# ewrfcas/LeftRefill

Measured on AMD Instinct MI355X. Metric: 512x1024 stitched images/sec @ 50 DDIM steps, cfg=2.5; per-UNet-step ms, higher is better.
Workload: dtype f16; 1 GPU; configs[1]: 1-ref inpainting, 512x1024 canvas (latent 64x128), B=4 per GPU (UNet batch 8 under CFG), 50 DDIM steps, cfg=2.5, eta=1.0, fp16; global_batch=4, per_gpu_batch=4, ddim_steps=50, parallelism=dp1 (sample-sharded, no data-path collective), ranks=1

## Files before the change

### include/leftrefill_hip.h

```cpp
#ifndef LEFTREFILL_HIP_H
#define LEFTREFILL_HIP_H

#include <stdint.h>

#ifdef __cplusplus
extern "C" {
#endif

#define LR_E_ARG (-1)
#define LR_E_ALIGN (-2)
#define LR_E_UNSUPPORTED (-3)

typedef void* lr_stream_t;
typedef uint16_t lr_half;
#define LR_DTYPE_F16 0
#define LR_DTYPE_BF16 1
#define LR_PIPE_DEFAULT 0
#define LR_PIPE_W8_DEEP 4
#define LR_PIPE_HALO 8

int lr_abi_version(void);

int lr_nchw_f32_to_nhwc_f16(const float* x1, int C1, const float* x2, int C2, lr_half* y, int Cpad, int N, int H,
                            int W, lr_stream_t s);
int lr_nhwc_f16_to_nchw(const lr_half* y, int Cstride, int C, void* out_nchw, int out_is_f32, int N, int H, int W,
                        lr_stream_t s);

#define LR_GN_CHUNKS 256
int lr_groupnorm_stats(const lr_half* x1, int C1, const lr_half* x2, int C2, int N, int HW, float* partials,
                       lr_stream_t s);
int lr_groupnorm_apply(const lr_half* x1, int C1, const lr_half* x2, int C2, int N, int HW, const float* partials,
                       const float* gamma, const float* beta, float eps, int silu, lr_half* y, lr_stream_t s);
int lr_groupnorm_finalize(const float* p1, int C1, int R1, const float* p2, int C2, int R2, int N, int HW, float* partials,
                          lr_stream_t s);

int lr_gn_conv_out_f16(const lr_half* x, int B, int H, int W, int C, const float* gpart, int chunks, const float* gamma, const float* beta,
                       float eps, const lr_half* w, int ldw, const float* bias, int Cout, lr_half* y, lr_stream_t s);
int lr_groupnorm_apply_n(const lr_half* x1, int C1, const lr_half* x2, int C2, int N, int HW, const float* partials,
                         int nchunks, const float* gamma, const float* beta, float eps, int silu, lr_half* y, lr_stream_t s);

int lr_layernorm(const lr_half* x, const float* gamma, const float* beta, float eps, lr_half* y, int M, int C,
                 lr_stream_t s);

int lr_timestep_embedding(const int64_t* t, int N, int dim, lr_half* out, lr_stream_t s);
int lr_timestep_embedding_f32(const float* t, int N, int dim, lr_half* out, lr_stream_t s);
int lr_linear_small_m(const lr_half* a, int lda, const lr_half* w, const float* bias, lr_half* out, int ldo, int M,
                      int N, int K, int act_in, int act_out, lr_stream_t s);

typedef struct lr_gemm_args {
  const lr_half* p1; int32_t C1;
  const lr_half* p2; int32_t C2;
  int32_t B, H, W;
  int32_t Hs, Ws;
  int32_t taps, stride, up;
  int32_t asym;
  const lr_half* wt; int32_t N;
  const float* bias;
  const lr_half* rowvec; int32_t ld_rowvec;
  const lr_half* resid; int32_t ld_resid;
  lr_half* out; int32_t ld_out;
  int32_t geglu;
  int32_t tile_n;
  int32_t tile_m;
  int32_t splits;
  float* workspace; int64_t workspace_bytes;
  const float* ln_stats; int32_t ln_parts; float ln_eps;
  const float* ln_colsum;
  float* stats_out;
  float* gn_stats_out;
  int32_t dtype;
  int32_t pipe;
  float* gn_group_out; int32_t gn_hw;
  int32_t wt_bstride, bias_bstride;
  int32_t wt_pm;
  const lr_half* skip1; const lr_half* skip2; int32_t Cs1, Cs2;
  int32_t splitk_mode;
} lr_gemm_args;
int lr_gemm_gn_group_chunks(const lr_gemm_args* args);
int lr_gemm_gn_rows(const lr_gemm_args* args);
int lr_gemm_plan(const lr_gemm_args* args, int32_t* plan);
int lr_gemm_stats_parts(const lr_gemm_args* args);
int64_t lr_gemm_workspace_bytes(const lr_gemm_args* args);
int lr_gemm_conv_f16(const lr_gemm_args* args, lr_stream_t s);
int lr_gemm_splitk_timeouts(void);

int lr_attention_f16(const lr_half* q, int ldq, const lr_half* k, int ldk, const lr_half* v, int ldv, lr_half* o,
                     int ldo, int B, int heads, int Nq, int Nkv, float scale, lr_stream_t s);

int lr_attention_causal_f16(const lr_half* q, int ldq, const lr_half* k, int ldk, const lr_half* v, int ldv, lr_half* o,
                            int ldo, int B, int heads, int N, float scale, lr_stream_t s);
int lr_attention_vt_f16(const lr_half* q, int ldq, const lr_half* k, int ldk, const lr_half* vt, int ld_vt, lr_half* o,
                        int ldo, int B, int heads, int Nq, int Nkv, float scale, lr_stream_t s);
int lr_transpose_v_f16(const lr_half* v, int ldv, lr_half* vt, int ld_vt, int B, int heads, int Nkv, lr_stream_t s);

typedef struct lr_xattn_args {
  const lr_half* x; lr_half* out;
  const lr_half* wq; const float* bq;
  const lr_half* k; int32_t ldk;
  const lr_half* vt;
  const lr_half* wo; const float* bo;
  float* stats_out;
  int32_t M, HW, C, heads, Lc;
  float ln_eps, scale;
  const lr_half* pre_a; const lr_half* pre_w; const float* pre_b;
} lr_xattn_args;
int lr_xattn_block_f16(const lr_xattn_args* args, lr_stream_t s);
int lr_xattn_pack_vt_f16(const lr_half* v, int ldv, lr_half* vt, int B, int heads, int Lc, lr_stream_t s);

typedef struct lr_stin_args {
  const lr_half* x; const lr_half* wp; const float* bp; const lr_half* wqkv; const float* bqkv;
  lr_half* x1; lr_half* qkv;
  int32_t M, C, NQ, ld_qkv;
  float ln_eps;
  const float* gn_part; const float* gn_gamma; const float* gn_beta;
  int32_t gn_chunks, gn_hw;
  float gn_eps;
} lr_stin_args;
int lr_stin_block_f16(const lr_stin_args* args, lr_stream_t s);

typedef struct lr_rowlin_args {
  const lr_half* x; const lr_half* w; const float* bias; lr_half* out;
  int32_t M, C, N, ld_out, geglu;
  float ln_eps;
  int32_t ln;
  const float* gn_part; const float* gn_gamma; const float* gn_beta;
  int32_t gn_chunks, gn_hw;
  float gn_eps;
} lr_rowlin_args;
int lr_rowlin_f16(const lr_rowlin_args* args, lr_stream_t s);

typedef struct lr_ffn_args {
  const lr_half* x; lr_half* out;
  const lr_half* w1; const float* b1;
  const lr_half* w2; const float* b2;
  float* stats_out;
  int32_t M, C, H;
  float ln_eps;
  const lr_half* post_w; const float* post_b; const lr_half* post_resid; float* gn_stats_out;
  float* gn_group_out; int32_t gn_hw;
} lr_ffn_args;
int lr_ffn_block_f16(const lr_ffn_args* args, lr_stream_t s);

int lr_softmax_rows_f16(const lr_half* s, lr_half* p, int M, int N, float scale, lr_stream_t st);

int lr_mv_gather(const lr_half* x, lr_half* seq, int b, int v, int s, int C, lr_stream_t st);
typedef struct lr_row_copy_job {
  const void* src; int64_t src_pitch, src_off;
  void* dst; int64_t dst_pitch, dst_off;
  int32_t row_bytes, n_rows;
  const int32_t* src_idx; const int32_t* dst_idx;
} lr_row_copy_job;
int lr_row_copy(const lr_row_copy_job* jobs, int n_jobs, lr_stream_t s);
int lr_mv_scatter(const lr_half* seq, lr_half* x, int b, int v, int s, int C, lr_stream_t st);

int lr_ddim_cfg_step(const float* x, const void* eps, int eps_is_f32, const float* noise, float* x_prev,
                     float* pred_x0, int64_t numel, float cfg_scale, float a_t, float a_prev, float sigma_t,
                     float sqrt_one_minus_at, lr_stream_t s);

int lr_plms_cfg_step(const float* x, const void* eps, int eps_is_f32, const float* const* hist, int n_hist, const float* weights,
                     float divisor, float* e_out, float* x_prev, float* pred_x0, int64_t numel, float cfg_scale, float a_t,
                     float a_prev, float sqrt_one_minus_at, lr_stream_t s);

int lr_dpmpp_cfg_step(const float* x, const void* eps, int eps_is_f32, const float* x0_prev, float* x0_out, float* x_next,
                      int64_t numel, float cfg_scale, float sigma_s, float alpha_s, float ratio, float c, float c_half,
                      float inv_r0, lr_stream_t s);

int lr_ddim_inv_cfg_step(const float* x, const void* eps, int eps_is_f32, float* x_next, int64_t numel, float cfg_scale,
                         float c1, float c2, lr_stream_t s);

int lr_ddim_cfg3_step(const float* x, const void* eps, int eps_is_f32, const float* noise, float* x_prev, float* pred_x0,
                      int64_t numel, float cfg_scale, float cond_weight, float one_minus_cond_weight, float a_t, float a_prev,
                      float sigma_t, float sqrt_one_minus_at, lr_stream_t s);

#define LR_Q_SAMPLE_MAX_B 32
int lr_ddim_q_sample(const float* x0, const float* noise, float* out, int B, int64_t per_sample, const float* sa,
                     const float* s1ma, lr_stream_t s);


int lr_layernorm_bwd(const lr_half* x, const lr_half* dy, const float* gamma, float eps, lr_half* dx, int M, int C,
                     lr_stream_t s);
int lr_groupnorm_bwd(const lr_half* x1, int C1, const lr_half* x2, int C2, const lr_half* dy, int N, int HW,
                     const float* fwd_partials, const float* gamma, const float* beta, float eps, int silu,
                     float* bwd_partials, lr_half* dx1, lr_half* dx2, lr_stream_t s);
int lr_layernorm_bwd_res(const lr_half* x, const lr_half* dy, const lr_half* dres, const float* gamma, float eps, lr_half* dx,
                         int M, int C, lr_stream_t s);
int lr_groupnorm_bwd_res(const lr_half* x1, int C1, const lr_half* x2, int C2, const lr_half* dy, const lr_half* dres1,
                         const lr_half* dres2, int N, int HW, const float* fwd_partials, int fwd_chunks, const float* gamma,
                         const float* beta, float eps, int silu, float* bwd_partials, lr_half* dx1, lr_half* dx2, lr_stream_t s);
int lr_geglu_bwd(const lr_half* pre, const lr_half* dy, lr_half* dpre, int M, int H, lr_stream_t s);
int lr_geglu_fwd(const lr_half* pre, lr_half* out, int M, int H, lr_stream_t s);
int lr_attention_lse_f16(const lr_half* q, int ldq, const lr_half* k, int ldk, const lr_half* v, int ldv, lr_half* o,
                         int ldo, float* lse, int B, int heads, int Nq, int Nkv, float scale, lr_stream_t s);
typedef struct lr_attn_bwd_args {
  const lr_half* q; const lr_half* k; const lr_half* v; const lr_half* o; const lr_half* dout;
  const lr_half* qt; const lr_half* kt; const lr_half* dot;
  const float* lse; float* dsum;
  lr_half* dq; lr_half* dk; lr_half* dv;
  int32_t ldq, ldk, ldv, ldo, lddo, ld_qt, ld_kt, lddq, lddk, lddv;
  int32_t B, heads, Nq, Nkv;
  float scale;
} lr_attn_bwd_args;
int lr_attention_bwd_f16(const lr_attn_bwd_args* args, lr_stream_t s);
int lr_attention_causal_lse_f16(const lr_half* q, int ldq, const lr_half* k, int ldk, const lr_half* v, int ldv, lr_half* o,
                                int ldo, float* lse, int B, int heads, int N, float scale, lr_stream_t s);
int lr_attention_causal_bwd_f16(const lr_attn_bwd_args* args, lr_stream_t s);
int lr_gelu_fwd_f16(const lr_half* pre, lr_half* y, int64_t n, lr_stream_t s);
int lr_gelu_bwd_f16(const lr_half* pre, const lr_half* dy, lr_half* dpre, int64_t n, lr_stream_t s);

int lr_mv_gather_bwd(const lr_half* dseq, lr_half* dx, int b, int v, int s, int C, lr_stream_t st);
int lr_mv_scatter_bwd(const lr_half* dx, lr_half* dseq, int b, int v, int s, int C, lr_stream_t st);
int lr_sumpool2x2(const lr_half* x, lr_half* y, int N, int H, int W, int C, lr_stream_t s);

int lr_groupnorm_stats_bf16(const lr_half* x1, int C1, const lr_half* x2, int C2, int N, int HW, float* partials,
    lr_stream_t s);
int lr_groupnorm_apply_bf16(const lr_half* x1, int C1, const lr_half* x2, int C2, int N, int HW, const float*
    partials, const float* gamma, const float* beta, float eps, int silu, lr_half* y, lr_stream_t s);
int lr_groupnorm_apply_n_bf16(const lr_half* x1, int C1, const lr_half* x2, int C2, int N, int HW, const float*
    partials, int nchunks, const float* gamma, const float* beta, float eps, int silu, lr_half* y, lr_stream_t s);
int lr_layernorm_bf16(const lr_half* x, const float* gamma, const float* beta, float eps, lr_half* y, int M, int C,
    lr_stream_t s);
int lr_layernorm_bwd_bf16(const lr_half* x, const lr_half* dy, const float* gamma, float eps, lr_half* dx, int M, int
    C, lr_stream_t s);
int lr_groupnorm_bwd_bf16(const lr_half* x1, int C1, const lr_half* x2, int C2, const lr_half* dy, int N, int HW,
    const float* fwd_partials, const float* gamma, const float* beta, float eps, int silu, float* bwd_partials,
    lr_half* dx1, lr_half* dx2, lr_stream_t s);
int lr_layernorm_bwd_res_bf16(const lr_half* x, const lr_half* dy, const lr_half* dres, const float* gamma, float eps, lr_half*
    dx, int M, int C, lr_stream_t s);
int lr_groupnorm_bwd_res_bf16(const lr_half* x1, int C1, const lr_half* x2, int C2, const lr_half* dy, const lr_half* dres1,
    const lr_half* dres2, int N, int HW, const float* fwd_partials, int fwd_chunks, const float* gamma, const float* beta,
// ... 66 lines not shown
```

### leftrefill_amd/_lib.py

```python
import ctypes
import os

HERE = os.path.dirname(os.path.abspath(__file__))
LIB_PATH = os.environ.get("LEFTREFILL_LIB_PATH") or os.path.join(HERE, "lib", "libleftrefill_hip.so")
ABI_VERSION = 29

c_void_p, c_int, c_float, c_int64 = ctypes.c_void_p, ctypes.c_int, ctypes.c_float, ctypes.c_int64


class GemmArgs(ctypes.Structure):
    _fields_ = [
        ("p1", c_void_p), ("C1", ctypes.c_int32),
        ("p2", c_void_p), ("C2", ctypes.c_int32),
        ("B", ctypes.c_int32), ("H", ctypes.c_int32), ("W", ctypes.c_int32),
        ("Hs", ctypes.c_int32), ("Ws", ctypes.c_int32),
        ("taps", ctypes.c_int32), ("stride", ctypes.c_int32), ("up", ctypes.c_int32),
        ("asym", ctypes.c_int32),
        ("wt", c_void_p), ("N", ctypes.c_int32),
        ("bias", c_void_p),
        ("rowvec", c_void_p), ("ld_rowvec", ctypes.c_int32),
        ("resid", c_void_p), ("ld_resid", ctypes.c_int32),
        ("out", c_void_p), ("ld_out", ctypes.c_int32),
        ("geglu", ctypes.c_int32),
        ("tile_n", ctypes.c_int32),
        ("tile_m", ctypes.c_int32),
        ("splits", ctypes.c_int32),
        ("workspace", c_void_p), ("workspace_bytes", ctypes.c_int64),
        ("ln_stats", c_void_p), ("ln_parts", ctypes.c_int32), ("ln_eps", ctypes.c_float),
        ("ln_colsum", c_void_p),
        ("stats_out", c_void_p),
        ("gn_stats_out", c_void_p),
        ("dtype", ctypes.c_int32),
        ("pipe", ctypes.c_int32),
        ("gn_group_out", c_void_p), ("gn_hw", ctypes.c_int32),
        ("wt_bstride", ctypes.c_int32), ("bias_bstride", ctypes.c_int32),
        ("wt_pm", ctypes.c_int32),
        ("skip1", c_void_p), ("skip2", c_void_p), ("Cs1", ctypes.c_int32), ("Cs2", ctypes.c_int32),
        ("splitk_mode", ctypes.c_int32),
    ]


class AttnBwdArgs(ctypes.Structure):
    _fields_ = ([(n, c_void_p) for n in ("q", "k", "v", "o", "dout", "qt", "kt", "dot", "lse", "dsum", "dq", "dk", "dv")] +
                [(n, ctypes.c_int32) for n in ("ldq", "ldk", "ldv", "ldo", "lddo", "ld_qt", "ld_kt", "lddq", "lddk", "lddv",
                                               "B", "heads", "Nq", "Nkv")] + [("scale", ctypes.c_float)])


class XattnArgs(ctypes.Structure):
    _fields_ = [("x", c_void_p), ("out", c_void_p), ("wq", c_void_p), ("bq", c_void_p), ("k", c_void_p), ("ldk", ctypes.c_int32),
                ("vt", c_void_p), ("wo", c_void_p), ("bo", c_void_p), ("stats_out", c_void_p),
                ("M", ctypes.c_int32), ("HW", ctypes.c_int32), ("C", ctypes.c_int32), ("heads", ctypes.c_int32),
                ("Lc", ctypes.c_int32), ("ln_eps", ctypes.c_float), ("scale", ctypes.c_float),
                ("pre_a", c_void_p), ("pre_w", c_void_p), ("pre_b", c_void_p)]


class RowCopyJob(ctypes.Structure):
    _fields_ = [("src", c_void_p), ("src_pitch", ctypes.c_int64), ("src_off", ctypes.c_int64),
                ("dst", c_void_p), ("dst_pitch", ctypes.c_int64), ("dst_off", ctypes.c_int64),
                ("row_bytes", ctypes.c_int32), ("n_rows", ctypes.c_int32), ("src_idx", c_void_p), ("dst_idx", c_void_p)]


class StinArgs(ctypes.Structure):
    _fields_ = [("x", c_void_p), ("wp", c_void_p), ("bp", c_void_p), ("wqkv", c_void_p), ("bqkv", c_void_p), ("x1", c_void_p),
                ("qkv", c_void_p), ("M", ctypes.c_int32), ("C", ctypes.c_int32), ("NQ", ctypes.c_int32), ("ld_qkv", ctypes.c_int32),
                ("ln_eps", ctypes.c_float), ("gn_part", c_void_p), ("gn_gamma", c_void_p), ("gn_beta", c_void_p),
                ("gn_chunks", ctypes.c_int32), ("gn_hw", ctypes.c_int32), ("gn_eps", ctypes.c_float)]


class RowlinArgs(ctypes.Structure):
    _fields_ = [("x", c_void_p), ("w", c_void_p), ("bias", c_void_p), ("out", c_void_p), ("M", ctypes.c_int32), ("C", ctypes.c_int32),
                ("N", ctypes.c_int32), ("ld_out", ctypes.c_int32), ("geglu", ctypes.c_int32), ("ln_eps", ctypes.c_float), ("ln", ctypes.c_int32),
                ("gn_part", c_void_p), ("gn_gamma", c_void_p), ("gn_beta", c_void_p), ("gn_chunks", ctypes.c_int32), ("gn_hw", ctypes.c_int32),
                ("gn_eps", ctypes.c_float)]


class FfnArgs(ctypes.Structure):
    _fields_ = [("x", c_void_p), ("out", c_void_p), ("w1", c_void_p), ("b1", c_void_p), ("w2", c_void_p), ("b2", c_void_p),
                ("stats_out", c_void_p), ("M", ctypes.c_int32), ("C", ctypes.c_int32), ("H", ctypes.c_int32), ("ln_eps", ctypes.c_float),
                ("post_w", c_void_p), ("post_b", c_void_p), ("post_resid", c_void_p), ("gn_stats_out", c_void_p),
                ("gn_group_out", c_void_p), ("gn_hw", ctypes.c_int32)]


SIGNATURES = {
    "lr_abi_version": [],
    "lr_nchw_f32_to_nhwc_f16": [c_void_p, c_int, c_void_p, c_int, c_void_p, c_int, c_int, c_int, c_int, c_void_p],
    "lr_nhwc_f16_to_nchw": [c_void_p, c_int, c_int, c_void_p, c_int, c_int, c_int, c_int, c_void_p],
    "lr_groupnorm_stats": [c_void_p, c_int, c_void_p, c_int, c_int, c_int, c_void_p, c_void_p],
    "lr_groupnorm_apply": [c_void_p, c_int, c_void_p, c_int, c_int, c_int, c_void_p, c_void_p, c_void_p, c_float,
                           c_int, c_void_p, c_void_p],
    "lr_layernorm_bwd": [c_void_p, c_void_p, c_void_p, c_float, c_void_p, c_int, c_int, c_void_p],
    "lr_groupnorm_bwd": [c_void_p, c_int, c_void_p, c_int, c_void_p, c_int, c_int, c_void_p, c_void_p, c_void_p, c_float,
                         c_int, c_void_p, c_void_p, c_void_p, c_void_p],
    "lr_layernorm_bwd_res": [c_void_p, c_void_p, c_void_p, c_void_p, c_float, c_void_p, c_int, c_int, c_void_p],
    "lr_groupnorm_bwd_res": [c_void_p, c_int, c_void_p, c_int, c_void_p, c_void_p, c_void_p, c_int, c_int, c_void_p, c_int, c_void_p,
                             c_void_p, c_float, c_int, c_void_p, c_void_p, c_void_p, c_void_p],
    "lr_mv_gather_bwd": [c_void_p, c_void_p, c_int, c_int, c_int, c_int, c_void_p],
    "lr_mv_scatter_bwd": [c_void_p, c_void_p, c_int, c_int, c_int, c_int, c_void_p],
    "lr_geglu_fwd": [c_void_p, c_void_p, c_int, c_int, c_void_p],
    "lr_geglu_bwd": [c_void_p, c_void_p, c_void_p, c_int, c_int, c_void_p],
    "lr_sumpool2x2": [c_void_p, c_void_p, c_int, c_int, c_int, c_int, c_void_p],
    "lr_softmax_rows_f16": [c_void_p, c_void_p, c_int, c_int, c_float, c_void_p],
    "lr_layernorm": [c_void_p, c_void_p, c_void_p, c_float, c_void_p, c_int, c_int, c_void_p],
    "lr_timestep_embedding": [c_void_p, c_int, c_int, c_void_p, c_void_p],
    "lr_linear_small_m": [c_void_p, c_int, c_void_p, c_void_p, c_void_p, c_int, c_int, c_int, c_int, c_int, c_int,
                          c_void_p],
    "lr_gemm_workspace_bytes": [ctypes.POINTER(GemmArgs)],
    "lr_gemm_stats_parts": [ctypes.POINTER(GemmArgs)],
    "lr_gemm_gn_rows": [ctypes.POINTER(GemmArgs)],
    "lr_gemm_gn_group_chunks": [ctypes.POINTER(GemmArgs)],
    "lr_gn_conv_out_f16": [c_void_p, c_int, c_int, c_int, c_int, c_void_p, c_int, c_void_p, c_void_p, c_float, c_void_p, c_int, c_void_p,
                           c_int, c_void_p, c_void_p],
    "lr_groupnorm_finalize": [c_void_p, c_int, c_int, c_void_p, c_int, c_int, c_int, c_int, c_void_p, c_void_p],
    "lr_groupnorm_apply_n": [c_void_p, c_int, c_void_p, c_int, c_int, c_int, c_void_p, c_int, c_void_p, c_void_p, c_float,
                             c_int, c_void_p, c_void_p],
    "lr_gemm_plan": [ctypes.POINTER(GemmArgs), ctypes.POINTER(ctypes.c_int32)],
    "lr_gemm_conv_f16": [ctypes.POINTER(GemmArgs), c_void_p],
    "lr_attention_f16": [c_void_p, c_int, c_void_p, c_int, c_void_p, c_int, c_void_p, c_int, c_int, c_int, c_int,
                         c_int, c_float, c_void_p],
    "lr_attention_vt_f16": [c_void_p, c_int, c_void_p, c_int, c_void_p, c_int, c_void_p, c_int, c_int, c_int, c_int,
                         c_int, c_float, c_void_p],
    "lr_attention_causal_f16": [c_void_p, c_int, c_void_p, c_int, c_void_p, c_int, c_void_p, c_int, c_int, c_int, c_int, c_float,
                                c_void_p],
    "lr_attention_lse_f16": [c_void_p, c_int, c_void_p, c_int, c_void_p, c_int, c_void_p, c_int, c_void_p, c_int, c_int, c_int,
                             c_int, c_float, c_void_p],
    "lr_attention_bwd_f16": [ctypes.POINTER(AttnBwdArgs), c_void_p],
    "lr_attention_causal_lse_f16": [c_void_p, c_int, c_void_p, c_int, c_void_p, c_int, c_void_p, c_int, c_void_p, c_int, c_int, c_int,
                                    c_float, c_void_p],
    "lr_attention_causal_bwd_f16": [ctypes.POINTER(AttnBwdArgs), c_void_p],
    "lr_gelu_fwd_f16": [c_void_p, c_void_p, c_int64, c_void_p],
    "lr_gelu_bwd_f16": [c_void_p, c_void_p, c_void_p, c_int64, c_void_p],
    "lr_transpose_v_f16": [c_void_p, c_int, c_void_p, c_int, c_int, c_int, c_int, c_void_p],
    "lr_xattn_block_f16": [ctypes.POINTER(XattnArgs), c_void_p],
    "lr_xattn_pack_vt_f16": [c_void_p, c_int, c_void_p, c_int, c_int, c_int, c_void_p],
    "lr_ffn_block_f16": [ctypes.POINTER(FfnArgs), c_void_p],
    "lr_stin_block_f16": [ctypes.POINTER(StinArgs), c_void_p],
    "lr_rowlin_f16": [ctypes.POINTER(RowlinArgs), c_void_p],
    "lr_mv_gather": [c_void_p, c_void_p, c_int, c_int, c_int, c_int, c_void_p],
    "lr_row_copy": [c_void_p, c_int, c_void_p],
    "lr_gemm_splitk_timeouts": [],
    "lr_mv_scatter": [c_void_p, c_void_p, c_int, c_int, c_int, c_int, c_void_p],
    "lr_ddim_cfg_step": [c_void_p, c_void_p, c_int, c_void_p, c_void_p, c_void_p, c_int64, c_float, c_float, c_float,
                         c_float, c_float, c_void_p],
    "lr_timestep_embedding_f32": [c_void_p, c_int, c_int, c_void_p, c_void_p],
    "lr_plms_cfg_step": [c_void_p, c_void_p, c_int, c_void_p, c_int, c_void_p, c_float, c_void_p, c_void_p, c_void_p, c_int64,
                         c_float, c_float, c_float, c_float, c_void_p],
    "lr_dpmpp_cfg_step": [c_void_p, c_void_p, c_int, c_void_p, c_void_p, c_void_p, c_int64, c_float, c_float, c_float, c_float,
                          c_float, c_float, c_float, c_void_p],
    "lr_ddim_inv_cfg_step": [c_void_p, c_void_p, c_int, c_void_p, c_int64, c_float, c_float, c_float, c_void_p],
    "lr_ddim_cfg3_step": [c_void_p, c_void_p, c_int, c_void_p, c_void_p, c_void_p, c_int64, c_float, c_float, c_float, c_float,
                          c_float, c_float, c_float, c_void_p],
    "lr_ddim_q_sample": [c_void_p, c_void_p, c_void_p, c_int, c_int64, c_void_p, c_void_p, c_void_p],
}

BF16_TWINS = ["lr_groupnorm_stats", "lr_groupnorm_apply", "lr_groupnorm_apply_n", "lr_layernorm", "lr_layernorm_bwd",
              "lr_groupnorm_bwd", "lr_layernorm_bwd_res", "lr_groupnorm_bwd_res", "lr_nchw_f32_to_nhwc_f16", "lr_nhwc_f16_to_nchw", "lr_timestep_embedding", "lr_linear_small_m",
              "lr_mv_gather", "lr_mv_scatter", "lr_ddim_cfg_step", "lr_timestep_embedding_f32", "lr_plms_cfg_step",
              "lr_dpmpp_cfg_step", "lr_ddim_inv_cfg_step", "lr_ddim_cfg3_step", "lr_geglu_fwd", "lr_geglu_bwd", "lr_sumpool2x2",
              "lr_mv_gather_bwd", "lr_mv_scatter_bwd", "lr_attention_f16", "lr_attention_causal_f16", "lr_attention_lse_f16",
              "lr_attention_vt_f16", "lr_transpose_v_f16", "lr_attention_bwd_f16", "lr_xattn_block_f16",
              "lr_xattn_pack_vt_f16", "lr_ffn_block_f16", "lr_stin_block_f16", "lr_rowlin_f16", "lr_gn_conv_out_f16",
              "lr_attention_causal_lse_f16", "lr_attention_causal_bwd_f16", "lr_gelu_fwd_f16", "lr_gelu_bwd_f16"]


def twin(name):
    return (name[:-4] if name.endswith("_f16") else name) + "_bf16"


for _n in BF16_TWINS:
    SIGNATURES[twin(_n)] = SIGNATURES[_n]

_FOLD_SIG = [c_void_p, c_int, c_int, c_int, c_int, c_void_p, c_void_p, c_float, c_void_p, c_void_p, c_int, c_void_p, c_void_p, c_void_p]
DEV_SIGNATURES = {"lr_dev_set": [ctypes.c_char_p, c_int], "lr_dev_unset": [ctypes.c_char_p],
                  "lr_gn_fold_weights_f16": _FOLD_SIG, "lr_gn_fold_weights_bf16": _FOLD_SIG}

_lib = None


def fn(lib, name, dtype):
    import torch
    if dtype == torch.bfloat16:
        return getattr(lib, twin(name))
    assert dtype == torch.float16, dtype
    return getattr(lib, name)


def load():
    global _lib
    if _lib is not None:
        return _lib
    import torch
    if not os.path.exists(LIB_PATH):
# ... 42 lines not shown
```

### leftrefill_amd/build.py

```python
import os
import shutil
import subprocess
import sys
from concurrent.futures import ThreadPoolExecutor

HERE = os.path.dirname(os.path.abspath(__file__))
CSRC = os.path.join(HERE, "csrc")
LIBDIR = os.path.join(HERE, "lib")
LIB = os.path.join(LIBDIR, "libleftrefill_hip.so")
SOURCES = ["norm.hip", "elementwise.hip", "gemm_conv.hip", "conv_halo.hip", "attention.hip", "attention_bwd.hip", "xattn_block.hip", "xattn_block640.hip", "stin_block.hip", "rowlin.hip", "ffn_block.hip", "conv_out.hip"]
FLAGS = ["--offload-arch=gfx950", "-O3", "-std=c++17", "-fPIC", "-Wno-unused-value"]
EXTRA = {"attention.hip": ["-mllvm", "-amdgpu-mfma-vgpr-form"], "xattn_block.hip": ["-mllvm", "-amdgpu-mfma-vgpr-form"], "ffn_block.hip": ["-mllvm", "-amdgpu-mfma-vgpr-form"], "stin_block.hip": ["-mllvm", "-amdgpu-mfma-vgpr-form"], "rowlin.hip": ["-mllvm", "-amdgpu-mfma-vgpr-form"], "attention_bwd.hip": ["-mllvm", "-amdgpu-mfma-vgpr-form"]}


def hipcc():
    for c in (os.environ.get("HIPCC"), shutil.which("hipcc"), "/opt/rocm/bin/hipcc"):
        if c and os.path.exists(c):
            return c
    raise RuntimeError("hipcc not found")


def _stale(out, deps):
    if not os.path.exists(out):
        return True
    t = os.path.getmtime(out)
    return any(os.path.getmtime(d) > t for d in deps)


def build(force=False, verbose=True):
    os.makedirs(LIBDIR, exist_ok=True)
    objdir = os.path.join(HERE, "build")
    os.makedirs(objdir, exist_ok=True)
    cc = hipcc()
    headers = [os.path.join(CSRC, "common.h"), os.path.join(CSRC, "chain_common.h"), os.path.join(CSRC, "gemm_common.h"), os.path.join(HERE, "..", "include", "leftrefill_hip.h")]
    jobs = []
    for s in SOURCES:
        src = os.path.join(CSRC, s)
        obj = os.path.join(objdir, s.replace(".hip", ".o"))
        if force or _stale(obj, [src] + headers):
            jobs.append([cc] + FLAGS + EXTRA.get(s, []) + ["-c", src, "-o", obj])
    if jobs:
        def run(cmd):
            if verbose:
                print(" ".join(cmd), flush=True)
            subprocess.run(cmd, check=True)
        with ThreadPoolExecutor(max_workers=4) as ex:
            list(ex.map(run, jobs))
    objs = [os.path.join(objdir, s.replace(".hip", ".o")) for s in SOURCES]
    if force or jobs or _stale(LIB, objs):
        cmd = [cc, "--offload-arch=gfx950", "-shared", "-fPIC", "-o", LIB] + objs
        if verbose:
            print(" ".join(cmd), flush=True)
        subprocess.run(cmd, check=True)
    return LIB


if __name__ == "__main__":
    print(build(force="--force" in sys.argv))
```

### leftrefill_amd/csrc/chain_common.h

```cpp
#pragma once
#include "common.h"

typedef __attribute__((address_space(3))) void* lptr_t;

template <int N> __device__ __forceinline__ void xa_wait_vmcnt() { asm volatile("s_waitcnt vmcnt(%0)" ::"n"(N) : "memory"); }

__device__ __forceinline__ float xa_row4_sum(float v) {
#if defined(__HIP_DEVICE_COMPILE__)
  const unsigned u = __builtin_bit_cast(unsigned, v);
  const auto a = __builtin_amdgcn_permlane16_swap(u, u, false, false);
  v = __builtin_bit_cast(float, (unsigned)a[0]) + __builtin_bit_cast(float, (unsigned)a[1]);
  const unsigned u2 = __builtin_bit_cast(unsigned, v);
  const auto b = __builtin_amdgcn_permlane32_swap(u2, u2, false, false);
  v = __builtin_bit_cast(float, (unsigned)b[0]) + __builtin_bit_cast(float, (unsigned)b[1]);
#endif
  return v;
}
__device__ __forceinline__ float xa_row4_max(float v) {
#if defined(__HIP_DEVICE_COMPILE__)
  const unsigned u = __builtin_bit_cast(unsigned, v);
  const auto a = __builtin_amdgcn_permlane16_swap(u, u, false, false);
  v = fmaxf(__builtin_bit_cast(float, (unsigned)a[0]), __builtin_bit_cast(float, (unsigned)a[1]));
  const unsigned u2 = __builtin_bit_cast(unsigned, v);
  const auto b = __builtin_amdgcn_permlane32_swap(u2, u2, false, false);
  v = fmaxf(__builtin_bit_cast(float, (unsigned)b[0]), __builtin_bit_cast(float, (unsigned)b[1]));
#endif
  return v;
}

template <typename T>
__device__ __forceinline__ vec8<T> xa_pack(const f32x4& a, const f32x4& b) {
  vec8<T> r;
#pragma unroll
  for (int i = 0; i < 4; ++i) { r[i] = (T)a[i]; r[4 + i] = (T)b[i]; }
  return r;
}
int lr_xattn640_launch(const lr_xattn_args* a, int bf16_, lr_stream_t s);

__device__ __forceinline__ void xa_swap_rows16(f32x4& a, f32x4& b) {
#if defined(__HIP_DEVICE_COMPILE__)
#pragma unroll
  for (int r = 0; r < 4; ++r) {
    const float ar = a[r], br = b[r];
    const auto s = __builtin_amdgcn_permlane16_swap(__builtin_bit_cast(unsigned, ar), __builtin_bit_cast(unsigned, br), false, false);
    a[r] = __builtin_bit_cast(float, (unsigned)s[0]);
    b[r] = __builtin_bit_cast(float, (unsigned)s[1]);
  }
#endif
}

__device__ __forceinline__ void xa_gn_tables(const float* gp, int nchunks, int n, int HW, int C, const float* gamma, const float* beta,
                                             float eps, float* tabA, float* tabB, float* s_mr , int t, int nthreads) {
#if defined(__HIP_DEVICE_COMPILE__)
  const int Cg = C / 32;
  if (t < 128) {
    const int g = t >> 2, sub = t & 3;
    double s = 0.0, q = 0.0;
    const float* ps = gp + ((size_t)n * nchunks * 32 + g) * 2;
#pragma unroll 4
    for (int c = sub; c < nchunks; c += 4) { s += (double)ps[c * 64]; q += (double)ps[c * 64 + 1]; }
#pragma unroll
    for (int sh = 2; sh > 0; sh >>= 1) { s += __shfl_xor(s, sh, 64); q += __shfl_xor(q, sh, 64); }
    if (sub == 0) {
      const double cnt = (double)HW * (double)Cg;
      const double mean = s / cnt;
      double var = q / cnt - mean * mean;
      if (var < 0.0) var = 0.0;
      s_mr[g] = (float)mean;
      s_mr[32 + g] = (float)(1.0 / sqrt(var + (double)eps));
    }
  }
  __syncthreads();
  for (int c = t; c < C; c += nthreads) {
    const int g = c / Cg;
    const float a = s_mr[32 + g] * gamma[c];
    tabA[c] = a;
    tabB[c] = beta[c] - s_mr[g] * a;
  }
  __syncthreads();
#endif
}
```

### leftrefill_amd/csrc/conv_halo.hip

```cpp
#include "gemm_common.h"

#ifndef HALO_EXP
#define HALO_EXP 0
#endif
#define HALO_PW 18
#define HALO_NQ 45

template <int BN, int WMW, int NSTAGE, typename T>
__global__ __launch_bounds__(512) void conv_halo_kernel(const GemmParams P) {
#if defined(__HIP_DEVICE_COMPILE__)
  constexpr int NW = 8, WNW = NW / WMW, TM = 16 / WMW, TN = BN / WNW / 16;
  constexpr int PATCH_BYTES = HALO_NQ * 1024;
  constexpr int B_BYTES = BN * 128;
  constexpr int NB_FULL = BN / (NW * 8);
  constexpr bool B_TAIL = (BN % (NW * 8)) != 0;
  constexpr int TAIL_WAVES = (BN % (NW * 8)) / 8;
  constexpr int PAR_LD = ((BN + 63) / 64) * 64;
  static_assert(NSTAGE == 2 || NSTAGE == 3, "weight ring depth");
  extern __shared__ __attribute__((aligned(16))) char smem[];
  char* const patch = smem;
  char* const wring = smem + PATCH_BYTES;
  float* const par = reinterpret_cast<float*>(wring + NSTAGE * B_BYTES);

  const int t = threadIdx.x;
  const int lane = t & 63;
  const int w = __builtin_amdgcn_readfirstlane(t >> 6);
  const int wm = w / WNW, wn = w % WNW;
  const int fr = lane & 15, fq = lane >> 4;
  const unsigned OOB = 0x80000000u;

  const int xcd = blockIdx.x & 7;
  const int q8 = P.nblocks >> 3, r8 = P.nblocks & 7;
  const int bid = (xcd < r8 ? xcd * (q8 + 1) : r8 * (q8 + 1) + (xcd - r8) * q8) + (blockIdx.x >> 3);
  [[maybe_unused]] const int lr_trace_tile = bid;
  int tile_n, tile;
  tile_order(P, bid, tile, tile_n);
  const bool seg = P.H == 8;
  const int Hv = seg ? 16 : P.H;
  const int npx = seg ? 2 * 10 * HALO_PW : HALO_PW * HALO_PW, nq = (npx + 7) >> 3;
  const int tiles_x = P.W >> 4, tps = (Hv >> 4) * tiles_x;
  const int smp = tile / tps, trem = tile - smp * tps;
  const int tyi = trem / tiles_x, txi = trem - tyi * tiles_x;
  const int y0 = tyi * 16, x0 = txi * 16;
  const int n0 = tile_n * BN;
  const int m_org = (smp * Hv + y0) * P.W + x0;

  int pix[6];
#pragma unroll
  for (int k = 0; k < 6; ++k) {
    const int px = (w + 8 * k) * 8 + (lane >> 3);
    const int pl = (px * 3641) >> 16, pc = px - pl * HALO_PW;
    const int sg = seg ? (pl * 26) >> 8 : 0;
    const int y = (seg ? pl - 10 * sg : y0 + pl) - 1, x = x0 - 1 + pc;
    const bool ok = px < npx && (unsigned)y < (unsigned)P.H && (unsigned)x < (unsigned)P.W;
    const int c = (lane & 7) ^ (pc & 6);
    pix[k] = ok ? (((((seg ? 2 * smp + sg : smp) * P.H + y) * P.W + x)) | (c << 28)) : -1;
  }
  const int Ctot = P.C1 + P.C2;
  const int cpt1 = P.C1 >> 6, ncm = Ctot >> 6, cpt3 = P.C3 >> 6;
  const int nch_all = ncm + ((P.C3 + P.C4) >> 6);
  const int c_per = (nch_all + P.splits - 1) / P.splits;
  const int c_begin = min((int)blockIdx.y * c_per, nch_all);
  const int nch = min(nch_all, c_begin + c_per);
  const int nsteps = (min(nch, ncm) - min(c_begin, ncm)) * 9 + (max(nch, ncm) - max(c_begin, ncm));
  auto issue_patch = [&](const int ci) __attribute__((always_inline)) {
    const f16* src; int cs, ch;
    if (ci < cpt1) { src = P.p1; cs = P.C1; ch = ci; }
    else if (ci < ncm) { src = P.p2; cs = P.C2; ch = ci - cpt1; }
    else if (ci < ncm + cpt3) { src = P.p3; cs = P.C3; ch = ci - ncm; }
    else { src = P.p4; cs = P.C4; ch = ci - ncm - cpt3; }
    const __amdgpu_buffer_rsrc_t rsA = uniform_rsrc((const void*)src, (size_t)P.M * cs * 2);
    const unsigned coff = (unsigned)ch * 128u;
#pragma unroll
    for (int k = 0; k < 6; ++k) {
      const int q = w + 8 * k;
      if (q < nq) {
        const unsigned vo = pix[k] >= 0 ? (unsigned)((pix[k] & 0x0FFFFFFF) * cs + (pix[k] >> 28) * 8) * 2u : OOB;
        __builtin_amdgcn_raw_ptr_buffer_load_lds(rsA, (lptr_t)(patch + q * 1024), 16, vo, coff, 0, 0);
      }
    }
  };

  const __amdgpu_buffer_rsrc_t rsB = uniform_rsrc((const void*)P.wt, (size_t)P.N * P.K * 2);
  const __amdgpu_buffer_rsrc_t rsZ = uniform_rsrc((const void*)P.wt, 0);
  __amdgpu_buffer_rsrc_t rsW = rsB;
  unsigned wvo[NB_FULL + 1];
#pragma unroll
  for (int i = 0; i < NB_FULL + 1; ++i) {
    const int row = (i * NW + w) * 8 + (lane >> 3);
    const int n = n0 + row;
    const int chunk = (lane & 7) ^ ((row >> 1) & 7);
    wvo[i] = (row < BN && n < P.N) ? (unsigned)(((size_t)n * (P.wt_pm ? 64 : P.K) + chunk * 8) * 2) : OOB;
  }
  auto wkoff = [&](const int ci, const int tap) -> unsigned {
    if (P.wt_pm) return (unsigned)(ci < ncm ? tap * ncm + ci : 9 * ncm + (ci - ncm)) * (unsigned)P.N * 128u;
    return (unsigned)((ci < ncm ? tap * Ctot + ci * 64 : 9 * Ctot + (ci - ncm) * 64) * 2);
  };
  auto issue_weights = [&](const int slot, const unsigned koff) __attribute__((always_inline)) {
    char* Bs = wring + slot * B_BYTES;
    if (B_TAIL && w < TAIL_WAVES)
      __builtin_amdgcn_raw_ptr_buffer_load_lds(rsW, (lptr_t)(Bs + ((NB_FULL * NW + w) * 8) * 128), 16, wvo[NB_FULL], koff, 0, 0);
#pragma unroll
    for (int i = 0; i < NB_FULL; ++i)
      __builtin_amdgcn_raw_ptr_buffer_load_lds(rsW, (lptr_t)(Bs + ((i * NW + w) * 8) * 128), 16, wvo[i], koff, 0, 0);
  };
  auto advance = [&](int& ci, int& tap) __attribute__((always_inline)) {
    const int nt = ci < ncm ? 9 : 1;
    if (++tap == nt) { tap = 0; ++ci; }
  };

  const int pb0 = (wm * TM + (seg ? 2 * ((wm * TM) >> 3) : 0)) * HALO_PW + fr;
  auto read_frags = [&](vec8<T> (&xf)[TM], vec8<T> (&wf)[TN], const int slot, const int ks, const int ky, const int kx) {
    const char* Bs = wring + slot * B_BYTES;
    const int kc = ks * 4 + fq;
    const int col = fr + kx;
    const char* xs = patch + (pb0 + kx) * 128 + ((kc ^ (col & 6)) << 4) + ky * (HALO_PW * 128);
#pragma unroll
    for (int i = 0; i < TM; ++i) xf[i] = *reinterpret_cast<const vec8<T>*>(xs + i * (HALO_PW * 128));
#pragma unroll
    for (int j = 0; j < TN; ++j) {
      const int row = weight_tile<TN, WNW, false>(wn, j) * 16 + fr;
      wf[j] = *reinterpret_cast<const vec8<T>*>(Bs + row * 128 + ((kc ^ ((row >> 1) & 7)) << 4));
    }
  };
  f32x4 acc[TN][TM];
  auto mma = [&](const vec8<T> (&xf)[TM], const vec8<T> (&wf)[TN]) {
#pragma unroll
    for (int j = 0; j < TN; ++j)
#pragma unroll
      for (int i = 0; i < TM; ++i)
        acc[j][i] = lr_mfma16(wf[j], xf[i], acc[j][i]);
  };
  auto spread = [&](auto ndma) __attribute__((always_inline)) {
    constexpr int ND = decltype(ndma)::value;
    constexpr int PER = (TM * TN) / ND > 0 ? (TM * TN) / ND : 1;
#pragma unroll
    for (int g = 0; g < ND; ++g) {
      __builtin_amdgcn_sched_group_barrier(0x8, PER, 0);
      __builtin_amdgcn_sched_group_barrier(0x10, 1, 0);
    }
  };
  using std::integral_constant;

  LR_STAMP(0);
  stage_params<BN, PAR_LD>(P, par, n0, w, lane, 0);
  if (nsteps > 0) issue_patch(c_begin);
  int wci = c_begin, wtap = 0;
#pragma unroll
  for (int sidx = 0; sidx < NSTAGE - 1; ++sidx) {
    if (sidx < nsteps) { issue_weights(sidx, wkoff(wci, wtap)); advance(wci, wtap); }
  }
  LR_STAMP(1);
#pragma unroll
  for (int j = 0; j < TN; ++j)
#pragma unroll
    for (int i = 0; i < TM; ++i) acc[j][i] = (f32x4){0.f, 0.f, 0.f, 0.f};
  if (NSTAGE == 3 && nsteps > 1) {
    if (B_TAIL && w < TAIL_WAVES) wait_vmcnt<NB_FULL + 1>(); else wait_vmcnt<NB_FULL>();
  } else {
    wait_vmcnt<0>();
  }
  __builtin_amdgcn_s_barrier();
  LR_STAMP(2);

  int ci = c_begin, tap = 0, cur = 0;
  vec8<T> xa[TM], wa[TN];
  for (int s = 0; s < nsteps; ++s) {
    const bool main_part = ci < ncm;
    const int ky = main_part ? (tap * 11) >> 5 : 1, kx = main_part ? tap - 3 * ky : 1;
    const bool last_tap = !main_part || tap == 8;
    const bool pf_w = s + NSTAGE - 1 < nsteps;
    const bool pf_p = last_tap && ci + 1 < nch;
    int wslot = cur + NSTAGE - 1; if (wslot >= NSTAGE) wslot -= NSTAGE;
    read_frags(xa, wa, cur, 0, ky, kx);
    __builtin_amdgcn_sched_barrier(0);
    rsW = (pf_w && HALO_EXP != 3) ? rsB : rsZ;
    issue_weights(wslot, wkoff(wci, wtap));
    advance(wci, wtap);
    mma(xa, wa);
    spread(integral_constant<int, NB_FULL>{});
    __builtin_amdgcn_sched_barrier(0);
    read_frags(xa, wa, cur, 1, ky, kx);
    if (pf_p && HALO_EXP != 1) {
      asm volatile("s_waitcnt lgkmcnt(0)" ::: "memory");
      __builtin_amdgcn_s_barrier();
      issue_patch(ci + 1);
    }
    mma(xa, wa);
    if (NSTAGE == 3 && !pf_p) {
      if (B_TAIL && w < TAIL_WAVES) wait_vmcnt<NB_FULL + 1>(); else wait_vmcnt<NB_FULL>();
    } else {
      wait_vmcnt<0>();
    }
    __builtin_amdgcn_s_barrier();
    cur = cur + 1 == NSTAGE ? 0 : cur + 1;
    advance(ci, tap);
  }
  LR_STAMP(3);
  LR_STAMP(4);

  float* gsl = reinterpret_cast<float*>(smem);
  const bool gp = P.gp_out != nullptr && P.splits == 1;
  epilogue_units<TM, TN, 0, PAR_LD, WNW, T, true>(P, acc, m_org + wm * TM * P.W, n0, wn, lane, par, par, tile_n * WNW + wn,
                                                  gsl + wm * (BN * 2), tile * WMW + wm);
  if (gp) {
    asm volatile("s_waitcnt lgkmcnt(0)" ::: "memory");
    __builtin_amdgcn_s_barrier();
    gn_group_reduce<BN, WMW, 256>(P, gsl, tile * 256, n0, t);
  }
#ifdef LR_DEV_VARIANTS
  if (P.sk_cnt != nullptr && P.splits > 1)
    sk_fused_tail<T, BN>(P, tile * P.ntiles_n + tile_n, 8,
                         [&](const int j, const int r) { return m_org + (2 * j + (r >> 4)) * P.W + (r & 15); },
                         [&](const int j) { return tile * 8 + j; }, [&](const int j) { return tile * 256 + 32 * j; }, n0,
                         reinterpret_cast<float*>(smem), t);
#endif
  LR_STAMP(5);
#ifdef LR_GEMM_TRACE
  asm volatile("s_waitcnt vmcnt(0)" ::: "memory");
  LR_STAMP(6);
#endif
#endif
}

template <int BN, int WMW, int NSTAGE, typename T>
static int launch_halo_t(const GemmParams& P0, hipStream_t st) {
  GemmParams P = P0;
  P.ntiles_n = (P.N + BN - 1) / BN;
  P.ntiles_m = P.M / 256;
  P.m_fastest = 0;
  if (LR_DEV("LR_HALO_MFASTEST", 0) && P.splits > 1) P.m_fastest = 1;
  P.nblocks = P.ntiles_n * P.ntiles_m;
  const size_t smem = (size_t)HALO_NQ * 1024 + NSTAGE * (size_t)BN * 128 + 2 * (((BN + 63) / 64) * 64) * sizeof(float);
  static unsigned long long attr_done = 0;
  if (lr_attr_needed(&attr_done)) {
    hipFuncSetAttribute(reinterpret_cast<const void*>(conv_halo_kernel<BN, WMW, NSTAGE, T>), hipFuncAttributeMaxDynamicSharedMemorySize,
                        (int)smem);
  }
  hipLaunchKernelGGL((conv_halo_kernel<BN, WMW, NSTAGE, T>), dim3(P.nblocks, P.splits), dim3(512), smem, st, P);
  return lr_launch_status();
}

int lr_launch_conv_halo(const GemmParams& P, int tile_n, hipStream_t st) {
  if (P.taps != 9 || P.stride != 1 || P.up || P.zins || P.pad != 1 || P.c16 || P.splits < 1 || P.geglu || P.gelu || P.ln_part ||
      P.wt_bstride || P.st_out || ((P.H & 15) && !(P.H == 8 && P.M % 256 == 0)) || (P.W & 15) || P.Hs != P.H || P.Ws != P.W)
    return LR_E_UNSUPPORTED;
  if ((long long)P.M >= (1ll << 28)) return LR_E_UNSUPPORTED;
  if (tile_n == 320) return P.bf16 ? launch_halo_t<320, 2, 2, bf16>(P, st) : launch_halo_t<320, 2, 2, f16>(P, st);
  if (tile_n == 160) return P.bf16 ? launch_halo_t<160, 4, 3, bf16>(P, st) : launch_halo_t<160, 4, 3, f16>(P, st);
  return LR_E_UNSUPPORTED;
}

unsigned lr_halo_sk_timeouts() {
  unsigned v = 0;
  if (hipMemcpyFromSymbol(&v, HIP_SYMBOL(lr_sk_error), sizeof(v)) != hipSuccess) return 0xFFFFFFFFu;
  return v;
}
```

### leftrefill_amd/csrc/elementwise.hip

```cpp
#include "common.h"

template <typename T>
__global__ void nchw_to_nhwc_kernel(const float* __restrict__ x1, int C1, const float* __restrict__ x2, int C2,
                                    T* __restrict__ y, int Cpad, int HW, long long total) {
  const int nOct = Cpad >> 3;
  for (long long idx = blockIdx.x * (long long)blockDim.x + threadIdx.x; idx < total;
       idx += (long long)gridDim.x * blockDim.x) {
    const int p = (int)(idx % HW);
    const long long q = idx / HW;
    const int o = (int)(q % nOct);
    const long long n = q / nOct;
    float f[8];
#pragma unroll
    for (int i = 0; i < 8; ++i) {
      const int c = o * 8 + i;
      float v = 0.f;
      if (c < C1) v = x1[((size_t)n * C1 + c) * HW + p];
      else if (c < C1 + C2) v = x2[((size_t)n * C2 + (c - C1)) * HW + p];
      f[i] = v;
    }
    *reinterpret_cast<uint4*>(y + ((size_t)n * HW + p) * Cpad + o * 8) = lr_pack8<T>(f);
  }
}

// ... 228 lines not shown
    ld_eps<V, EpsT>(eps, i, eu);
    ld_eps<V, EpsT>(eps, numel + i, ec);
    ld_f32<V>(x, i, xv);
    if (n_hist > 0) ld_f32<V>(h1, i, a);
    if (n_hist > 1) ld_f32<V>(h2, i, b);
    if (n_hist > 2) ld_f32<V>(h3, i, c);
#pragma unroll
    for (int k = 0; k < V; ++k) {
      e[k] = cfg_combine<EpsT, T>(eu[k], ec[k], scale);
      float acc = w0 * e[k];
      if (n_hist > 0) acc = acc + w1 * a[k];
      if (n_hist > 1) acc = acc + w2 * b[k];
      if (n_hist > 2) acc = acc + w3 * c[k];
      const float ep = acc / div;
      p0[k] = (xv[k] - sqrt_1m_at * ep) / sqrt_at;
      xp[k] = sqrt_aprev * p0[k] + dir_coef * ep;
    }
    if (e_out) st_f32<V>(e_out, i, e);
    st_f32<V>(pred_x0, i, p0);
    st_f32<V>(x_prev, i, xp);
  }
}

template <int V, typename EpsT, typename T>
__global__ void dpmpp_cfg_step_kernel(const float* __restrict__ x, const EpsT* __restrict__ eps, const float* __restrict__ x0_prev,
                                      float* __restrict__ x0_out, float* __restrict__ x_next, long long numel, float scale,
                                      float sigma_s, float alpha_s, float ratio, float c, float c_half, float inv_r0) {
#pragma clang fp contract(off)
  const long long groups = numel / V;
  for (long long g = blockIdx.x * (long long)blockDim.x + threadIdx.x; g < groups; g += (long long)gridDim.x * blockDim.x) {
    const long long i = g * V;
    float eu[V], ec[V], xv[V], m1[V], m0[V], xt[V];
    ld_eps<V, EpsT>(eps, i, eu);
    ld_eps<V, EpsT>(eps, numel + i, ec);
    ld_f32<V>(x, i, xv);
    if (x0_prev) ld_f32<V>(x0_prev, i, m1);
#pragma unroll
    for (int k = 0; k < V; ++k) {
      const float e = cfg_combine<EpsT, T>(eu[k], ec[k], scale);
      m0[k] = (xv[k] - sigma_s * e) / alpha_s;
      float v = ratio * xv[k] - c * m0[k];
      if (x0_prev) {
        const float D = inv_r0 * (m0[k] - m1[k]);
        v = v - c_half * D;
      }
      xt[k] = v;
    }
    st_f32<V>(x0_out, i, m0);
    st_f32<V>(x_next, i, xt);
  }
}

template <int V, typename EpsT, typename T>
__global__ void ddim_inv_cfg_step_kernel(const float* __restrict__ x, const EpsT* __restrict__ eps, float* __restrict__ x_next,
                                         long long numel, float scale, float c1, float c2) {
#pragma clang fp contract(off)
  const long long groups = numel / V;
  for (long long g = blockIdx.x * (long long)blockDim.x + threadIdx.x; g < groups; g += (long long)gridDim.x * blockDim.x) {
    const long long i = g * V;
    float eu[V], ec[V], xv[V], xn[V];
    ld_eps<V, EpsT>(eps, i, eu);
    ld_eps<V, EpsT>(eps, numel + i, ec);
    ld_f32<V>(x, i, xv);
#pragma unroll
    for (int k = 0; k < V; ++k) {
      const float e = cfg_combine<EpsT, T>(eu[k], ec[k], scale);
      const float a = c1 * xv[k];
      float b;
      if constexpr (sizeof(EpsT) == 2) b = (float)(T)((float)(T)c2 * e);
      else b = c2 * e;
      xn[k] = a + b;
    }
    st_f32<V>(x_next, i, xn);
  }
}

__device__ __forceinline__ float f32_rounded(float v) {
  asm volatile("" : "+v"(v));
  return v;
}

template <typename EpsT, typename T>
__device__ __forceinline__ float cfg3_combine(float eu, float ec, float es, float scale, float w, float w1m) {
#pragma clang fp contract(off)
  if constexpr (sizeof(EpsT) == 2) {
    const T a = (T)f32_rounded(w * ec);
    const T b = (T)f32_rounded(w1m * es);
    const T m = (T)((float)a + (float)b);
    const T d = (T)((float)m - eu);
    const T sd = (T)f32_rounded(scale * (float)d);
    return (float)(T)(eu + (float)sd);
  } else {
    return eu + scale * ((w * ec + w1m * es) - eu);
  }
}

template <int V, typename EpsT, typename T>
__global__ void ddim_cfg3_step_kernel(const float* __restrict__ x, const EpsT* __restrict__ eps, const float* __restrict__ noise,
                                      float* __restrict__ x_prev, float* __restrict__ pred_x0, long long numel, float scale,
                                      float w, float w1m, float sqrt_at, float sqrt_1m_at, float sqrt_aprev, float dir_coef,
                                      float sigma) {
#pragma clang fp contract(off)
  const long long groups = numel / V;
  for (long long g = blockIdx.x * (long long)blockDim.x + threadIdx.x; g < groups; g += (long long)gridDim.x * blockDim.x) {
    const long long i = g * V;
    float eu[V], ec[V], es[V], xv[V], nz[V], p0[V], xp[V];
    ld_eps<V, EpsT>(eps, i, eu);
    ld_eps<V, EpsT>(eps, numel + i, ec);
    ld_eps<V, EpsT>(eps, 2 * numel + i, es);
    ld_f32<V>(x, i, xv);
    if (noise) ld_f32<V>(noise, i, nz);
#pragma unroll
    for (int k = 0; k < V; ++k) {
      const float e = cfg3_combine<EpsT, T>(eu[k], ec[k], es[k], scale, w, w1m);
      p0[k] = (xv[k] - sqrt_1m_at * e) / sqrt_at;
      float v = sqrt_aprev * p0[k] + dir_coef * e;
      if (noise) v = v + sigma * nz[k];
      xp[k] = v;
    }
    st_f32<V>(pred_x0, i, p0);
    st_f32<V>(x_prev, i, xp);
  }
}

struct QSampleCoefs { float sa[LR_Q_SAMPLE_MAX_B]; float s1ma[LR_Q_SAMPLE_MAX_B]; };

template <int V>
__global__ void ddim_q_sample_kernel(const float* __restrict__ x0, const float* __restrict__ noise, float* __restrict__ out,
                                     long long per_sample, const QSampleCoefs C) {
#pragma clang fp contract(off)
  const long long base = (long long)blockIdx.y * per_sample;
  const float sa = C.sa[blockIdx.y], s1ma = C.s1ma[blockIdx.y];
  const long long groups = per_sample / V;
  for (long long g = blockIdx.x * (long long)blockDim.x + threadIdx.x; g < groups; g += (long long)gridDim.x * blockDim.x) {
    const long long i = base + g * V;
    float xv[V], nv[V], o[V];
    ld_f32<V>(x0, i, xv);
    ld_f32<V>(noise, i, nv);
#pragma unroll
    for (int k = 0; k < V; ++k) o[k] = sa * xv[k] + s1ma * nv[k];
    st_f32<V>(out, i, o);
  }
}

static inline bool aligned16(const void* p) { return p == nullptr || ((uintptr_t)p & 15) == 0; }

static inline int grid_for(long long total, int block, int cap = 4096) {
  long long g = (total + block - 1) / block;
  if (g > cap) g = cap;
  if (g < 1) g = 1;
  return (int)g;
}

extern "C" int lr_abi_version(void) { return 29; }

#ifdef LR_DEV_VARIANTS
#include <map>
#include <mutex>
#include <string>
static std::map<std::string, int>& lr_dev_table() { static std::map<std::string, int> t; return t; }
static std::mutex lr_dev_mutex;
extern "C" int lr_dev_set(const char* name, int value) {
  if (!name) return LR_E_ARG;
  std::lock_guard<std::mutex> g(lr_dev_mutex);
  lr_dev_table()[name] = value;
  return 0;
}
extern "C" int lr_dev_unset(const char* name) {
  if (!name) return LR_E_ARG;
  std::lock_guard<std::mutex> g(lr_dev_mutex);
  lr_dev_table().erase(name);
  return 0;
}
int lr_dev_get(const char* name, int dflt) {
  std::lock_guard<std::mutex> g(lr_dev_mutex);
  const auto it = lr_dev_table().find(name);
  return it == lr_dev_table().end() ? dflt : it->second;
}
#endif

template <typename T>
static int lr_nchw_f32_to_nhwc_t(const float* x1, int C1, const float* x2, int C2, lr_half* y, int Cpad, int N,
                                       int H, int W, lr_stream_t s) {
  if (!x1 || !y || N <= 0 || H <= 0 || W <= 0 || C1 <= 0) return LR_E_ARG;
  if (!x2) C2 = 0;
  if (Cpad % 8 || Cpad < C1 + C2) return LR_E_ALIGN;
  const long long total = (long long)N * (Cpad / 8) * H * W;
  hipLaunchKernelGGL(nchw_to_nhwc_kernel<T>, dim3(grid_for(total, 256)), dim3(256), 0, (hipStream_t)s, x1, C1, x2, C2,
                     (T*)y, Cpad, H * W, total);
  return lr_launch_status();
}

template <typename T>
static int lr_nhwc_f16_to_nchw_t(const lr_half* y, int Cstride, int C, void* out, int out_is_f32, int N, int H, int W,
                                   lr_stream_t s) {
  if (!y || !out || N <= 0 || C <= 0 || C > Cstride) return LR_E_ARG;
  const long long total = (long long)N * C * H * W;
  if (out_is_f32)
    hipLaunchKernelGGL((nhwc_to_nchw_kernel<float, T>), dim3(grid_for(total, 256)), dim3(256), 0, (hipStream_t)s,
                       (const T*)y, Cstride, C, (float*)out, H * W, total);
  else
    hipLaunchKernelGGL((nhwc_to_nchw_kernel<T, T>), dim3(grid_for(total, 256)), dim3(256), 0, (hipStream_t)s,
                       (const T*)y, Cstride, C, (T*)out, H * W, total);
  return lr_launch_status();
}

template <typename TT, typename T>
static int lr_timestep_embedding_t(const TT* t, int N, int dim, lr_half* out, lr_stream_t s) {
  if (!t || !out || N <= 0 || dim < 2) return LR_E_ARG;
  const int total = N * (dim / 2);
  hipLaunchKernelGGL((timestep_embedding_kernel<TT, T>), dim3((total + 255) / 256), dim3(256), 0, (hipStream_t)s, t, N, dim,
                     (T*)out);
  return lr_launch_status();
}

template <typename T>
static int lr_linear_small_m_t(const lr_half* a, int lda, const lr_half* w, const float* bias, lr_half* out, int ldo,
                                 int M, int N, int K, int act_in, int act_out, lr_stream_t s) {
  if (!a || !w || !out || M <= 0 || N <= 0 || K <= 0) return LR_E_ARG;
  if (M > 16) return LR_E_UNSUPPORTED;
  if (K % 8) return LR_E_ALIGN;
  const int waves = 4;
  int cpw = (N + waves * 512 - 1) / (waves * 512);
  if (cpw < 4) cpw = 4;
  if (cpw > 32) cpw = 32;
  dim3 grid((N + cpw * waves - 1) / (cpw * waves)), block(64 * waves);
  hipStream_t st = (hipStream_t)s;
  if (M <= 4)
    hipLaunchKernelGGL((linear_small_m_kernel<4, T>), grid, block, 4 * K * sizeof(T), st, (const T*)a, lda,
                       (const T*)w, bias, (T*)out, ldo, M, N, K, act_in, act_out, cpw);
  else if (M <= 8)
    hipLaunchKernelGGL((linear_small_m_kernel<8, T>), grid, block, 8 * K * sizeof(T), st, (const T*)a, lda,
                       (const T*)w, bias, (T*)out, ldo, M, N, K, act_in, act_out, cpw);
  else
    hipLaunchKernelGGL((linear_small_m_kernel<16, T>), grid, block, 16 * K * sizeof(T), st, (const T*)a, lda,
                       (const T*)w, bias, (T*)out, ldo, M, N, K, act_in, act_out, cpw);
  return lr_launch_status();
}

template <typename T>
static int lr_mv_gather_t(const lr_half* x, lr_half* seq, int b, int v, int s, int C, lr_stream_t st) {
  if (!x || !seq || b <= 0 || v <= 0 || s <= 0) return LR_E_ARG;
  if (C % 8) return LR_E_ALIGN;
  const long long total = (long long)b * (v + 1) * s * s * (C / 8);
  hipLaunchKernelGGL((mv_gather_kernel<false, T>), dim3(grid_for(total, 256)), dim3(256), 0, (hipStream_t)st, (const uint4*)x,
                     (uint4*)seq, b, v, s, C / 8, total);
  return lr_launch_status();
}

template <typename T>
static int lr_mv_scatter_t(const lr_half* seq, lr_half* x, int b, int v, int s, int C, lr_stream_t st) {
  if (!x || !seq || b <= 0 || v <= 0 || s <= 0) return LR_E_ARG;
  if (C % 8) return LR_E_ALIGN;
  const long long total = (long long)b * v * s * 2 * s * (C / 8);
  hipLaunchKernelGGL(mv_scatter_kernel<false>, dim3(grid_for(total, 256)), dim3(256), 0, (hipStream_t)st, (const uint4*)seq,
                     (uint4*)x, b, v, s, C / 8, total);
  return lr_launch_status();
}

template <typename T>
static int lr_ddim_cfg_step_t(const float* x, const void* eps, int eps_is_f32, const float* noise, float* x_prev,
                                float* pred_x0, int64_t numel, float cfg_scale, float a_t, float a_prev, float sigma_t,
                                float sqrt_one_minus_at, lr_stream_t s) {
  if (!x || !eps || !x_prev || !pred_x0 || numel <= 0) return LR_E_ARG;
  const float sqrt_at = sqrtf(a_t);
  const float sqrt_aprev = sqrtf(a_prev);
  const float dir_coef = sqrtf(1.0f - a_prev - sigma_t * sigma_t);
  dim3 grid(grid_for(numel, 256)), block(256);
  if (eps_is_f32)
    hipLaunchKernelGGL((ddim_cfg_step_kernel<float, T>), grid, block, 0, (hipStream_t)s, x, (const float*)eps, noise, x_prev,
                       pred_x0, (long long)numel, cfg_scale, sqrt_at, sqrt_one_minus_at, sqrt_aprev, dir_coef,
                       sigma_t);
  else
    hipLaunchKernelGGL((ddim_cfg_step_kernel<T, T>), grid, block, 0, (hipStream_t)s, x, (const T*)eps, noise, x_prev,
                       pred_x0, (long long)numel, cfg_scale, sqrt_at, sqrt_one_minus_at, sqrt_aprev, dir_coef,
                       sigma_t);
  return lr_launch_status();
}

template <int V, typename EpsT, typename T>
static void launch_plms(const float* x, const void* eps, const float* h1, const float* h2, const float* h3, float* e_out,
                        float* x_prev, float* pred_x0, long long numel, int n_hist, float scale, const float* w, float div,
                        float sqrt_at, float sqrt_1m_at, float sqrt_aprev, float dir_coef, hipStream_t s) {
  hipLaunchKernelGGL((plms_cfg_step_kernel<V, EpsT, T>), dim3(grid_for(numel / V, 256)), dim3(256), 0, s, x, (const EpsT*)eps,
                     h1, h2, h3, e_out, x_prev, pred_x0, numel, n_hist, scale, w[0], w[1], w[2], w[3], div, sqrt_at, sqrt_1m_at,
                     sqrt_aprev, dir_coef);
}

template <typename T>
static int lr_plms_cfg_step_t(const float* x, const void* eps, int eps_is_f32, const float* const* hist, int n_hist,
                              const float* weights, float divisor, float* e_out, float* x_prev, float* pred_x0, int64_t numel,
                              float cfg_scale, float a_t, float a_prev, float sqrt_one_minus_at, lr_stream_t s) {
  if (!x || !eps || !x_prev || !pred_x0 || !weights || numel <= 0 || n_hist < 0 || n_hist > 3 || divisor == 0.f) return LR_E_ARG;
  if (n_hist > 0 && !hist) return LR_E_ARG;
  const float* h[3] = {nullptr, nullptr, nullptr};
  for (int k = 0; k < n_hist; ++k) {
    if (!hist[k]) return LR_E_ARG;
    h[k] = hist[k];
  }
  float w[4] = {weights[0], 0.f, 0.f, 0.f};
  for (int k = 0; k < n_hist; ++k) w[k + 1] = weights[k + 1];
  const float sqrt_at = sqrtf(a_t);
  const float sqrt_aprev = sqrtf(a_prev);
  const float dir_coef = sqrtf(1.0f - a_prev - 0.0f);
  const bool vec = numel % 4 == 0 && aligned16(x) && aligned16(h[0]) && aligned16(h[1]) && aligned16(h[2]) && aligned16(e_out) &&
                   aligned16(x_prev) && aligned16(pred_x0) && ((uintptr_t)eps & (eps_is_f32 ? 15 : 7)) == 0;
  hipStream_t st = (hipStream_t)s;
// ... 326 lines not shown
```

### leftrefill_amd/csrc/gemm_common.h

```cpp
#pragma once
#include "common.h"
#include <type_traits>

#define BK 64
#define GEMM_THREADS 256
#define BM 128

struct GemmParams {
  const f16* p1; const f16* p2; const f16* wt; const float* bias; const f16* rowvec; const f16* resid; f16* out;
  int C1, C2, H, W, Hs, Ws, taps, stride, up, pad, zins, N, M, K, ld_rowvec, ld_resid, ld_out, geglu, gelu, rows_per_batch;
  int ntiles_n, nblocks;
  int splits; float* ws;
  int ntiles_m, m_fastest;
  unsigned hw_mul, hw_sh, w_mul, w_sh;
  const float* ln_part; const float* ln_cs; int ln_parts; float ln_eps, ln_invc;
  float* st_out; int st_parts;
  float* gs_out;
  float* gp_out; int gp_cg, gp_chunks, gp_hw;
  int gs_store;
  int wt_bstride, bias_bstride;
  int wt_pm;
  int c16;
  const f16* p3; const f16* p4; int C3, C4;
  int bf16;
  unsigned* sk_cnt;
#ifdef LR_GEMM_STAGGER
  int stagger;
#endif
#ifdef LR_GEMM_TRACE
  unsigned long long* trace;
#endif
};

#ifdef LR_GEMM_TRACE
#define LR_STAMP(k) do { if (P.trace && threadIdx.x == 0) P.trace[(size_t)(blockIdx.y * P.nblocks + lr_trace_tile) * 8 + (k)] = __builtin_readcyclecounter(); } while (0)
#else
#define LR_STAMP(k) do { } while (0)
#endif

__device__ __forceinline__ void tile_order(const GemmParams& P, int bid, int& tile_m, int& tile_n) {
  if (P.m_fastest > 1) {
    const int G = P.m_fastest, per = G * P.ntiles_n;
    const int grp = bid / per, first = grp * G;
    const int gsz = min(G, P.ntiles_m - first), r = bid - grp * per;
    tile_m = first + r % gsz; tile_n = r / gsz;
  } else if (P.m_fastest) { tile_m = bid % P.ntiles_m; tile_n = bid / P.ntiles_m; }
  else { tile_n = bid % P.ntiles_n; tile_m = bid / P.ntiles_n; }
}

typedef __attribute__((address_space(3))) void* lptr_t;


__device__ __forceinline__ void swap_rows16(f32x4& a, f32x4& b) {
#if defined(__HIP_DEVICE_COMPILE__)
#pragma unroll
  for (int r = 0; r < 4; ++r) {
    const float ar = a[r], br = b[r];
    const auto s = __builtin_amdgcn_permlane16_swap(__builtin_bit_cast(unsigned, ar), __builtin_bit_cast(unsigned, br),
                                                    false, false);
    a[r] = __builtin_bit_cast(float, (unsigned)s[0]);
    b[r] = __builtin_bit_cast(float, (unsigned)s[1]);
  }
#endif
}

typedef unsigned u32x4 __attribute__((ext_vector_type(4)));
#ifndef LR_OUT_AUX
#define LR_OUT_AUX 16
#endif

template <int TE, int WNW>
__device__ __forceinline__ constexpr int emit_tile(const int wn, const int je) {
  return TE == 5 ? (je < 4 ? 4 * wn + je : 4 * WNW + wn) : wn * TE + je;
}
template <int TN, int WNW, bool GEGLU>
__device__ __forceinline__ constexpr int weight_tile(const int wn, const int j) {
  return GEGLU ? 2 * emit_tile<TN / 2, WNW>(wn, j >> 1) + (j & 1) : emit_tile<TN, WNW>(wn, j);
}

template <int TM, int TN, int MODE, int PAR_LD, int WNW, typename T, bool HALO = false>
__device__ __forceinline__ void epilogue_units(const GemmParams& P, f32x4 (&acc)[TN][TM], const int m_w0, const int n0,
                                               const int wn, const int lane, const float* rs, const float* par,
                                               const int part, float* gsl = nullptr, const int rb_halo = 0) {
#if defined(__HIP_DEVICE_COMPILE__)
  constexpr bool GEGLU = MODE == 1;
  constexpr int TE = GEGLU ? TN / 2 : TN;
  constexpr int NPJ = TE / 2;
  constexpr int NUJ = TM * NPJ;
  constexpr int NU = NUJ + (TE & 1) * (TM / 2);
  constexpr int G = TM * TN >= 40 ? 8 : (NU < 16 ? NU : 16);
  const int fr = lane & 15, fq = lane >> 4;
  const int odd = fq & 1, ch8 = (fq >> 1) * 8;
  const int N_out = GEGLU ? P.N >> 1 : P.N;
  const int no0 = GEGLU ? n0 >> 1 : n0;
  const bool ln = P.ln_part != nullptr;
  const bool fin = P.splits == 1;
  const unsigned OOB = 0x80000000u;
  const int mstep = HALO ? P.W : 16;
  const __amdgpu_buffer_rsrc_t rsR = uniform_rsrc(P.resid ? (const void*)P.resid : (const void*)P.out,
                                                  (P.resid && fin) ? ((size_t)(P.M - 1) * P.ld_resid + N_out) * 2 : 0);
  const __amdgpu_buffer_rsrc_t rsV = uniform_rsrc(P.rowvec ? (const void*)P.rowvec : (const void*)P.out,
                                                  (P.rowvec && fin) ? ((size_t)((P.M - 1) / P.rows_per_batch) * P.ld_rowvec + N_out) * 2 : 0);
  const __amdgpu_buffer_rsrc_t rsO = uniform_rsrc(P.out, fin ? ((size_t)(P.M - 1) * P.ld_out + N_out) * 2 : 0);
  const __amdgpu_buffer_rsrc_t rsWS = uniform_rsrc(P.sk_cnt ? (const void*)P.ws : (const void*)P.out,
                                                   P.sk_cnt ? (size_t)P.splits * P.M * P.N * 4 : 0);
  constexpr int SGH = TM > 8 ? TM : 8;
  float sg[2 * SGH];
#pragma unroll
  for (int i = 0; i < 2 * SGH; ++i) sg[i] = 0.f;
#define s1(i) sg[(i)]
#define s2(i) sg[SGH + (i)]
#define g1(q) sg[(q)]
#define g2(q) sg[SGH + (q)]
  const bool gstat = !GEGLU && fin && (P.gs_out != nullptr || P.gp_out != nullptr) && P.st_out == nullptr;
  auto row16_sum = [&](float v) -> float {
    v += __builtin_bit_cast(float, __builtin_amdgcn_mov_dpp(__builtin_bit_cast(int, v), 0xB1, 0xF, 0xF, true));
    v += __builtin_bit_cast(float, __builtin_amdgcn_mov_dpp(__builtin_bit_cast(int, v), 0x4E, 0xF, 0xF, true));
    v += __builtin_bit_cast(float, __builtin_amdgcn_mov_dpp(__builtin_bit_cast(int, v), 0x141, 0xF, 0xF, true));
    v += __builtin_bit_cast(float, __builtin_amdgcn_mov_dpp(__builtin_bit_cast(int, v), 0x140, 0xF, 0xF, true));
    return v;
  };
  auto flush_group = [&](const int n_lane, const bool pair_fq) {
    const int rb = HALO ? rb_halo : m_w0 / (TM * 16);
#pragma unroll
    for (int q = 0; q < 8; ++q) {
      float a = row16_sum(g1(q)), b = row16_sum(g2(q));
      if (pair_fq) {
        const auto sa = __builtin_amdgcn_permlane16_swap(__builtin_bit_cast(unsigned, a), __builtin_bit_cast(unsigned, a), false, false);
        a = __builtin_bit_cast(float, (unsigned)sa[0]) + __builtin_bit_cast(float, (unsigned)sa[1]);
        const auto sb = __builtin_amdgcn_permlane16_swap(__builtin_bit_cast(unsigned, b), __builtin_bit_cast(unsigned, b), false, false);
        b = __builtin_bit_cast(float, (unsigned)sb[0]) + __builtin_bit_cast(float, (unsigned)sb[1]);
      }
      g1(q) = a; g2(q) = b;
    }
    if (fr == 0 && (!pair_fq || !odd) && n_lane < N_out) {
      if (P.gs_out != nullptr && m_w0 < P.M) {
        float* dst = P.gs_out + ((size_t)rb * N_out + n_lane) * 2;
#pragma unroll
        for (int q = 0; q < 8; q += 2) {
          const f32x4 o = {g1(q), g2(q), g1(q + 1), g2(q + 1)};
          *reinterpret_cast<f32x4*>(dst + 2 * q) = o;
        }
      }
      if (P.gp_out != nullptr) {
        float* dst = gsl + (n_lane - no0) * 2;
#pragma unroll
        for (int q = 0; q < 8; q += 2) {
          const f32x4 o = {g1(q), g2(q), g1(q + 1), g2(q + 1)};
          *reinterpret_cast<f32x4*>(dst + 2 * q) = o;
        }
      }
    }
#pragma unroll
    for (int q = 0; q < 8; ++q) { g1(q) = 0.f; g2(q) = 0.f; }
  };
  auto rowstat = [&](const int i) -> float2 { return *reinterpret_cast<const float2*>(rs + 2 * (i * 16 + fr)); };
  auto par4 = [&](const int which, const int col) -> f32x4 { return *reinterpret_cast<const f32x4*>(par + which * PAR_LD + col); };
  auto tile = [&](const int i, const int je) -> f32x4 {
    if constexpr (!GEGLU) {
      const int c = weight_tile<TN, WNW, false>(wn, je) * 16 + fq * 4;
      f32x4 r = acc[je][i];
      if (ln) { const float2 mr = rowstat(i); r = (r - par4(1, c) * mr.x) * mr.y; }
      if (fin) r += par4(0, c);
      return r;
    } else {
      const int c = weight_tile<TN, WNW, true>(wn, 2 * je) * 16 + fq * 4;
      f32x4 u = acc[2 * je][i], g = acc[2 * je + 1][i];
      if (ln) {
        const float2 mr = rowstat(i);
        u = (u - par4(1, c) * mr.x) * mr.y;
        g = (g - par4(1, c + 16) * mr.x) * mr.y;
      }
      u += par4(0, c); g += par4(0, c + 16);
      const f32x2_t g01 = lr_gelu_erf2((f32x2_t){g[0], g[1]}), g23 = lr_gelu_erf2((f32x2_t){g[2], g[3]});
      const f32x4 o = {u[0] * g01[0], u[1] * g01[1], u[2] * g23[0], u[3] * g23[1]};
      return o;
    }
  };
// ... 338 lines not shown
```

### leftrefill_amd/csrc/gemm_conv.hip

```cpp
#include "gemm_common.h"
#include <atomic>

#ifdef LR_GEMM_TRACE
static unsigned long long* g_trace = nullptr;
extern "C" void lr_gemm_set_trace(void* p) { g_trace = (unsigned long long*)p; }
#endif


template <int BN, int MODE, typename T>
__global__ __launch_bounds__(GEMM_THREADS, BN == 64 ? 4 : BN == 128 ? 3 : 2) void gemm_conv_kernel(const GemmParams P) {
#if defined(__HIP_DEVICE_COMPILE__)
  constexpr int TM = 4;
  constexpr int TN = BN / 32;
  constexpr int A_BYTES = BM * 128;
  constexpr int B_BYTES = BN * 128;
  constexpr int STAGE = A_BYTES + B_BYTES;
  extern __shared__ __attribute__((aligned(16))) char smem[];

  const int t = threadIdx.x;
  const int lane = t & 63;
  const int w = __builtin_amdgcn_readfirstlane(t >> 6);
  const int wm = w >> 1, wn = w & 1;
#ifdef LR_GEMM_STAGGER
  if (P.stagger) {
// ... 771 lines not shown
  const int splits = a->splits ? a->splits : choose_splits(M, a->N, K, tm, tn, a->geglu == 1, a->pipe);
  return gn_group_chunks(a, tm, tn, splits);
}

extern "C" int lr_gemm_stats_parts(const lr_gemm_args* a) {
  if (!a) return 0;
  int tn = a->tile_n, tm = a->tile_m;
  choose_tile(a->B * a->H * a->W, a->N, a->geglu != 0, &tm, &tn);
  return ((a->N + tn - 1) / tn) * tile_wnw(tm, tn, a->geglu == 1);
}

extern "C" int64_t lr_gemm_workspace_bytes(const lr_gemm_args* a) {
  if (!a) return 0;
  const int M = a->B * a->H * a->W;
  const int K = a->taps * (a->C1 + (a->p2 ? a->C2 : 0)) + (a->skip1 ? a->Cs1 + (a->skip2 ? a->Cs2 : 0) : 0);
  int tn = a->tile_n, tm = a->tile_m;
  choose_tile(M, a->N, a->geglu != 0, &tm, &tn);
  int splits = a->splits ? a->splits : choose_splits(M, a->N, K, tm, tn, a->geglu == 1, a->pipe);
  return splits > 1 ? (int64_t)splits * M * a->N * (int64_t)sizeof(float) : 0;
}

static __device__ unsigned lr_sk_counters[16][2048];
static unsigned* sk_counter_slot() {
  static unsigned* base[64] = {nullptr};
  static std::atomic<unsigned> next{0};
  int dev = 0;
  if (hipGetDevice(&dev) != hipSuccess) return nullptr;
  dev &= 63;
  if (!base[dev]) {
    void* p = nullptr;
    if (hipGetSymbolAddress(&p, HIP_SYMBOL(lr_sk_counters)) != hipSuccess) return nullptr;
    base[dev] = (unsigned*)p;
  }
  return base[dev] + (size_t)(next.fetch_add(1, std::memory_order_relaxed) & 15) * 2048;
}

extern "C" int lr_gemm_splitk_timeouts(void) {
  unsigned v = 0;
  if (hipMemcpyFromSymbol(&v, HIP_SYMBOL(lr_sk_error), sizeof(v)) != hipSuccess) return -1;
  const unsigned h = lr_halo_sk_timeouts();
  return h == 0xFFFFFFFFu ? -1 : (int)(v + h);
}

extern "C" int lr_gemm_conv_f16(const lr_gemm_args* a, lr_stream_t s) {
  if (!a || !a->p1 || !a->wt || !a->out) return LR_E_ARG;
  GemmParams P;
  P.p1 = (const f16*)a->p1; P.C1 = a->C1;
  P.p2 = (const f16*)a->p2; P.C2 = a->p2 ? a->C2 : 0;
  P.c16 = (P.C1 == 16 && P.C2 == 0 && a->taps == 9 && a->stride == 1 && a->up == 0 && !a->asym) ? 1 : 0;
  if (P.C1 <= 0 || (!P.c16 && P.C1 % 64) || P.C2 % 64) return LR_E_ALIGN;
  if (a->taps != 1 && a->taps != 9) return LR_E_UNSUPPORTED;
  if (a->stride != 1 && a->stride != 2) return LR_E_UNSUPPORTED;
  if (a->up < 0 || a->up > 2) return LR_E_UNSUPPORTED;
  if (a->B <= 0 || a->H <= 0 || a->W <= 0 || a->Hs <= 0 || a->Ws <= 0 || a->N <= 0) return LR_E_ARG;
  P.H = a->H; P.W = a->W; P.Hs = a->Hs; P.Ws = a->Ws;
  P.taps = a->taps; P.stride = a->stride; P.up = a->up;
  P.zins = (a->up == 2) ? 1 : 0;
  if (P.zins) P.up = 1;
  P.pad = a->asym ? 0 : 1;
  P.wt = (const f16*)a->wt; P.N = a->N; P.bias = a->bias;
  P.M = a->B * a->H * a->W;
  P.p3 = (const f16*)a->skip1; P.C3 = a->skip1 ? a->Cs1 : 0;
  P.p4 = a->skip1 ? (const f16*)a->skip2 : nullptr; P.C4 = P.p4 ? a->Cs2 : 0;
  if (P.p3) {
    if (P.c16 || a->stride != 1 || a->up != 0 || a->asym || a->geglu || a->ln_stats || a->wt_bstride ||
        a->Hs != a->H || a->Ws != a->W)
      return LR_E_UNSUPPORTED;
    if (P.C3 <= 0 || P.C3 % 64 || P.C4 % 64 || (((uintptr_t)P.p3 | (uintptr_t)P.p4) & 15)) return LR_E_ALIGN;
  }
  P.K = P.c16 ? 192 : a->taps * (P.C1 + P.C2) + P.C3 + P.C4;
  const int64_t lim = (int64_t)1 << 31;
  const int64_t src_rows = (int64_t)a->B * a->Hs * a->Ws;
  if (src_rows * P.C1 * 2 >= lim || src_rows * P.C2 * 2 >= lim || src_rows * P.C3 * 2 >= lim || src_rows * P.C4 * 2 >= lim ||
      (int64_t)P.N * P.K * 2 >= lim ||
      (int64_t)a->B * a->H * a->W >= lim / 2)
    return LR_E_UNSUPPORTED;
  P.rowvec = (const f16*)a->rowvec; P.ld_rowvec = a->ld_rowvec;
  P.resid = (const f16*)a->resid; P.ld_resid = a->ld_resid;
  P.out = (f16*)a->out; P.ld_out = a->ld_out;
  if ((int64_t)P.M * a->ld_out * 2 >= lim || (a->resid && (int64_t)P.M * a->ld_resid * 2 >= lim) ||
      (a->rowvec && (int64_t)a->B * a->ld_rowvec * 2 >= lim))
    return LR_E_UNSUPPORTED;
  if (a->geglu < 0 || a->geglu > 2) return LR_E_ARG;
  P.geglu = a->geglu == 1 ? 1 : 0;
  P.gelu = a->geglu == 2 ? 1 : 0;
  P.rows_per_batch = a->H * a->W;
  lr_udiv_magic((unsigned)(a->H * a->W), &P.hw_mul, &P.hw_sh);
  lr_udiv_magic((unsigned)a->W, &P.w_mul, &P.w_sh);
  const int N_out = P.geglu ? P.N / 2 : P.N;
  if (P.N % 8 || N_out % 8 || P.ld_out % 8 || (P.resid && P.ld_resid % 8) || (P.rowvec && P.ld_rowvec % 8))
    return LR_E_ALIGN;
  if (P.geglu && P.N % 32) return LR_E_ALIGN;
  if (((uintptr_t)P.p1 | (uintptr_t)P.p2 | (uintptr_t)P.wt | (uintptr_t)P.out | (uintptr_t)P.resid |
       (uintptr_t)P.rowvec | (uintptr_t)P.bias) & 15)
    return LR_E_ALIGN;
  int tn = a->tile_n, tm = a->tile_m;
  choose_tile(P.M, P.N, P.geglu || P.gelu, &tm, &tn);
  int splits = a->splits;
  if (P.c16) {
    if (tm != 256 || (a->splits > 1) || P.geglu || P.gelu || a->wt_bstride) return LR_E_UNSUPPORTED;
    splits = 1;
  }
  if (splits == 0) splits = choose_splits(P.M, P.N, P.K, tm, tn, P.geglu, a->pipe);
  if (splits > 1 && P.geglu) return LR_E_UNSUPPORTED;
  if (splits > 1) {
    const int64_t need = (int64_t)splits * P.M * P.N * (int64_t)sizeof(float);
    if (!a->workspace || a->workspace_bytes < need) {
      if (a->splits > 1) return LR_E_ARG;
      splits = 1;
    }
  }
  P.splits = splits;
  P.ws = a->workspace;
  P.sk_cnt = nullptr;
  if (a->splitk_mode != 0 && a->splitk_mode != 1) return LR_E_ARG;
#ifndef LR_DEV_VARIANTS
  if (a->splitk_mode == 1) return LR_E_UNSUPPORTED;
#endif
  P.ln_part = a->ln_stats; P.ln_cs = a->ln_colsum; P.ln_parts = a->ln_parts; P.ln_eps = a->ln_eps;
  P.ln_invc = 1.0f / (float)P.K;
  if (P.ln_part) {
    if (!P.ln_cs || P.ln_parts <= 0 || P.taps != 1 || P.C2 || splits > 1) return LR_E_ARG;
    if (((uintptr_t)P.ln_part & 7) || ((uintptr_t)P.ln_cs & 15)) return LR_E_ALIGN;
  }
#ifdef LR_GEMM_TRACE
  P.trace = g_trace;
#endif
  if (a->dtype != LR_DTYPE_F16 && a->dtype != LR_DTYPE_BF16) return LR_E_ARG;
  P.bf16 = a->dtype == LR_DTYPE_BF16;
#ifdef LR_GEMM_STAGGER
  P.stagger = LR_DEV("LR_GEMM_STAGGER", 0);
#endif
  if (P.bf16 && P.gelu) return LR_E_UNSUPPORTED;
  P.gs_out = a->gn_stats_out;
  if (P.gs_out && (P.geglu || ((uintptr_t)P.gs_out & 15))) return LR_E_ARG;
  P.gs_store = P.gs_out != nullptr;
  P.gp_out = a->gn_group_out; P.gp_cg = 1; P.gp_chunks = 0; P.gp_hw = 1;
  if (P.gp_out) {
    P.gp_chunks = gn_group_chunks(a, tm, tn, splits);
    if (P.gp_chunks <= 0 || ((uintptr_t)P.gp_out & 7) || a->stats_out) return LR_E_ARG;
    P.gp_cg = P.N / 32;
    P.gp_hw = a->gn_hw > 0 ? a->gn_hw : a->H * a->W;
  }
  P.wt_pm = a->wt_pm ? 1 : 0;
  if (P.wt_pm && (a->wt_bstride || P.K % 64)) return LR_E_ARG;
  P.wt_bstride = a->wt_bstride; P.bias_bstride = a->bias_bstride;
  if (P.wt_bstride) {
    if (a->taps != 1 || splits > 1 || P.rows_per_batch % tm || P.wt_bstride < 0 || P.bias_bstride < 0 || (P.wt_bstride & 7)) return LR_E_ARG;
    if ((int64_t)a->B * P.wt_bstride * 2 >= lim) return LR_E_UNSUPPORTED;
  }
  P.st_out = a->stats_out;
  P.st_parts = ((P.N + tn - 1) / tn) * tile_wnw(tm, tn, P.geglu);
  if (P.st_out && (splits > 1 || ((uintptr_t)P.st_out & 7))) return LR_E_ARG;
  hipStream_t st = (hipStream_t)s;
  int rc;
  const int mode = P.geglu ? 1 : P.gelu ? 2 : 0;
  if (a->pipe != 0 && a->pipe != choose_stages(tm, tn, a->pipe)) return LR_E_UNSUPPORTED;
  const bool deep = tm == 128 && choose_stages(tm, tn, a->pipe) == 4;
#ifdef LR_DEV_VARIANTS
  if (P.splits > 1 && a->splitk_mode == 1 && mode != 1 && (tn == 160 || tn == 320) && (tm == 256 || deep || a->pipe == LR_PIPE_HALO)) {
    const int64_t tiles = (int64_t)((P.M + tm - 1) / tm) * ((P.N + tn - 1) / tn);
    if (tiles * P.splits <= 256 && tiles <= 2048 && (int64_t)P.splits * P.M * P.N * 4 < lim && P.N % 8 == 0)
      P.sk_cnt = sk_counter_slot();
  }
#endif
  if (a->pipe == LR_PIPE_HALO) {
    if (mode != 0 || a->asym) return LR_E_UNSUPPORTED;
    rc = lr_launch_conv_halo(P, tn, st);
    if (rc || P.splits == 1 || P.sk_cnt) return rc;
    return launch_reduce(P, st);
  }
  if (mode == 0) {
    if (deep && tn == 128) rc = launch_pipe<128, 8, 128, 4, 4, 0>(P, st);
    else if (deep && tn == 160) rc = launch_pipe<128, 8, 160, 4, 4, 0>(P, st);

    else if (tm == 128 && tn == 128) rc = launch_gemm<128, 0>(P, st);
    else if (tm == 128 && tn == 64) rc = launch_gemm<64, 0>(P, st);
    else if (tm == 128 && tn == 160) rc = launch_gemm<160, 0>(P, st);
    else if (tm == 256 && tn == 128) rc = launch_gemm256<128, 4, 3, 0>(P, st);
    else if (tm == 256 && tn == 160) rc = launch_gemm256<160, 4, 3, 0>(P, st);
    else if (tm == 256 && tn == 256) rc = launch_gemm256<256, 2, 2, 0>(P, st);
    else if (tm == 256 && tn == 320) rc = launch_gemm256<320, 2, 2, 0>(P, st);
    else return LR_E_UNSUPPORTED;
  } else if (mode == 1) {
    if (deep && tn == 128) rc = launch_pipe<128, 8, 128, 4, 4, 1>(P, st);
    else if (deep) return LR_E_UNSUPPORTED;
    else if (tm == 128 && tn == 128) rc = launch_gemm<128, 1>(P, st);
    else if (tm == 128 && tn == 64) rc = launch_gemm<64, 1>(P, st);
    else if (tm == 256 && tn == 128) rc = launch_gemm256<128, 4, 3, 1>(P, st);
    else if (tm == 256 && tn == 256) rc = launch_gemm256<256, 2, 2, 1>(P, st);
    else if (tm == 256 && tn == 320) rc = launch_gemm256<320, 4, 2, 1>(P, st);
    else return LR_E_UNSUPPORTED;
  } else {
    if (deep) return LR_E_UNSUPPORTED;
    if (tm == 128 && tn == 128) rc = launch_gemm<128, 2>(P, st);
    else if (tm == 128 && tn == 64) rc = launch_gemm<64, 2>(P, st);
    else if (tm == 256 && tn == 128) rc = launch_gemm256<128, 4, 3, 2>(P, st);
    else return LR_E_UNSUPPORTED;
  }
  if (rc || P.splits == 1 || P.sk_cnt) return rc;
  return launch_reduce(P, st);
}
```

### leftrefill_amd/csrc/norm.hip

```cpp
#include "common.h"

#include <stdlib.h>

template <typename T>
__global__ void gn_stats_kernel(const T* __restrict__ x1, int C1, const T* __restrict__ x2, int C2, int HW,
                                float* __restrict__ partials, int nOct, int R, int nchunks) {
  extern __shared__ float s_part[];
  const int C = C1 + C2;
  const int Cg = C / 32;
  const int n = blockIdx.y, chunk = blockIdx.x;
  const int t = threadIdx.x;
  const int o = t % nOct, r = t / nOct;
  const int per = (HW + nchunks - 1) / nchunks;
  const int p0 = chunk * per, p1 = min(HW, p0 + per);
  const int c0 = o * 8;
  const T* src;
  int cs, coff;
  if (c0 < C1) { src = x1; cs = C1; coff = c0; } else { src = x2; cs = C2; coff = c0 - C1; }
  float sm[8], sq[8];
#pragma unroll
  for (int i = 0; i < 8; ++i) { sm[i] = 0.f; sq[i] = 0.f; }
  const T* base = src + ((size_t)n * HW) * cs + coff;
  int p = p0 + r;
  for (; p + 3 * R < p1; p += 4 * R) {
    uint4 u[4];
#pragma unroll
    for (int k = 0; k < 4; ++k) u[k] = *reinterpret_cast<const uint4*>(base + (size_t)(p + k * R) * cs);
#pragma unroll
    for (int k = 0; k < 4; ++k) {
      float f[8];
      lr_unpack8<T>(u[k], f);
#pragma unroll
      for (int i = 0; i < 8; ++i) { sm[i] += f[i]; sq[i] = fmaf(f[i], f[i], sq[i]); }
    }
  }
  for (; p < p1; p += R) {
    const uint4 u0 = *reinterpret_cast<const uint4*>(base + (size_t)p * cs);
    float f[8];
    lr_unpack8<T>(u0, f);
#pragma unroll
    for (int i = 0; i < 8; ++i) { sm[i] += f[i]; sq[i] = fmaf(f[i], f[i], sq[i]); }
  }
#pragma unroll
  for (int i = 0; i < 8; ++i) {
    s_part[((size_t)r * C + c0 + i) * 2 + 0] = sm[i];
    s_part[((size_t)r * C + c0 + i) * 2 + 1] = sq[i];
  }
  __syncthreads();
  if (t < 32) {
    float s = 0.f, q = 0.f;
    for (int c = t * Cg; c < (t + 1) * Cg; ++c)
      for (int rr = 0; rr < R; ++rr) { s += s_part[((size_t)rr * C + c) * 2]; q += s_part[((size_t)rr * C + c) * 2 + 1]; }
    float* dst = partials + (((size_t)n * nchunks + chunk) * 32 + t) * 2;
    dst[0] = s;
    dst[1] = q;
  }
}

template <typename T>
__global__ void gn_apply_kernel(const T* __restrict__ x1, int C1, const T* __restrict__ x2, int C2, int HW,
                                const float* __restrict__ partials, const float* __restrict__ gamma,
                                const float* __restrict__ beta, float eps, int silu, T* __restrict__ y,
                                int pix_per_block, int nOct, int R, int nchunks) {
  __shared__ float s_mean[32], s_rstd[32];
  const int C = C1 + C2;
  const int Cg = C / 32;
  const int n = blockIdx.y;
  const int t = threadIdx.x;
  const int o = t % nOct, r = t / nOct;
  const int c0 = o * 8;
  const int p0 = blockIdx.x * pix_per_block;
  const int p1 = min(HW, p0 + pix_per_block);
  const T* src;
  int cs;
  if (c0 < C1) { src = x1 + ((size_t)n * HW) * C1 + c0; cs = C1; }
  else { src = x2 + ((size_t)n * HW) * C2 + (c0 - C1); cs = C2; }
  T* dst = y + ((size_t)n * HW) * C + c0;

  int p = p0 + r;
  uint4 u[4];
  const bool first = p + 3 * R < p1;
  if (first) {
#pragma unroll
    for (int k = 0; k < 4; ++k) u[k] = *reinterpret_cast<const uint4*>(src + (size_t)(p + k * R) * cs);
  }
  float ga[8], be[8];
#pragma unroll
  for (int i = 0; i < 8; ++i) { ga[i] = gamma[c0 + i]; be[i] = beta[c0 + i]; }
  if (t < 128) {
    const int g = t >> 2, sub = t & 3;
    double s = 0.0, q = 0.0;
    const float* ps = partials + ((size_t)n * nchunks * 32 + g) * 2;
#pragma unroll 4
    for (int c = sub; c < nchunks; c += 4) { s += (double)ps[c * 64]; q += (double)ps[c * 64 + 1]; }
#pragma unroll
    for (int sh = 2; sh > 0; sh >>= 1) { s += __shfl_xor(s, sh, 64); q += __shfl_xor(q, sh, 64); }
    if (sub == 0) {
      const double cnt = (double)HW * (double)Cg;
      const double mean = s / cnt;
      double var = q / cnt - mean * mean;
      if (var < 0.0) var = 0.0;
      s_mean[g] = (float)mean;
      s_rstd[g] = (float)(1.0 / sqrt(var + (double)eps));
    }
  }
  __syncthreads();
  float a[8], b[8];
#pragma unroll
  for (int i = 0; i < 8; ++i) {
    const int g = (c0 + i) / Cg;
    a[i] = s_rstd[g] * ga[i];
    b[i] = be[i] - s_mean[g] * a[i];
  }
  auto emit = [&](int pp, const uint4& v) {
    float f[8];
    lr_unpack8<T>(v, f);
#pragma unroll
    for (int i = 0; i < 8; ++i) {
      const float z = fmaf(f[i], a[i], b[i]);
      f[i] = silu ? z * __builtin_amdgcn_rcpf(1.0f + __expf(-z)) : z;
    }
    *reinterpret_cast<uint4*>(dst + (size_t)pp * C) = lr_pack8<T>(f);
  };
  if (r >= R) return;
  bool have = first;
  while (have) {
    const int np = p + 4 * R;
    const bool more = np + 3 * R < p1;
    uint4 w[4];
    if (more) {
#pragma unroll
      for (int k = 0; k < 4; ++k) w[k] = *reinterpret_cast<const uint4*>(src + (size_t)(np + k * R) * cs);
    }
#pragma unroll
    for (int k = 0; k < 4; ++k) emit(p + k * R, u[k]);
    if (more) {
#pragma unroll
      for (int k = 0; k < 4; ++k) u[k] = w[k];
    }
    p = np;
    have = more;
  }
  for (; p < p1; p += R) emit(p, *reinterpret_cast<const uint4*>(src + (size_t)p * cs));
}

template <int NV, typename T>
__global__ void layernorm_kernel(const T* __restrict__ x, const float* __restrict__ gamma,
                                 const float* __restrict__ beta, float eps, T* __restrict__ y, int M, int C) {
  const int lane = threadIdx.x & 63;
  const int row = blockIdx.x * (blockDim.x >> 6) + (threadIdx.x >> 6);
  if (row >= M) return;
  const int nOct = C >> 3;
  float v[NV][8];
  float sum = 0.f;
#pragma unroll
  for (int j = 0; j < NV; ++j) {
    const int o = lane + j * 64;
    if (o < nOct) {
      const uint4 u = *reinterpret_cast<const uint4*>(x + (size_t)row * C + o * 8);
      lr_unpack8<T>(u, v[j]);
#pragma unroll
      for (int i = 0; i < 8; ++i) sum += v[j][i];
    } else {
#pragma unroll
      for (int i = 0; i < 8; ++i) v[j][i] = 0.f;
    }
  }
  const float mean = lr_wave_sum(sum) / (float)C;
  float sq = 0.f;
#pragma unroll
  for (int j = 0; j < NV; ++j) {
    const int o = lane + j * 64;
    if (o < nOct) {
#pragma unroll
      for (int i = 0; i < 8; ++i) { const float d = v[j][i] - mean; sq = fmaf(d, d, sq); }
    }
  }
  const float rstd = rsqrtf(lr_wave_sum(sq) / (float)C + eps);
#pragma unroll
  for (int j = 0; j < NV; ++j) {
    const int o = lane + j * 64;
    if (o < nOct) {
      const float4 g0 = *reinterpret_cast<const float4*>(gamma + o * 8);
      const float4 g1 = *reinterpret_cast<const float4*>(gamma + o * 8 + 4);
      const float4 b0 = *reinterpret_cast<const float4*>(beta + o * 8);
      const float4 b1 = *reinterpret_cast<const float4*>(beta + o * 8 + 4);
      const float g[8] = {g0.x, g0.y, g0.z, g0.w, g1.x, g1.y, g1.z, g1.w};
      const float b[8] = {b0.x, b0.y, b0.z, b0.w, b1.x, b1.y, b1.z, b1.w};
      float f[8];
#pragma unroll
      for (int i = 0; i < 8; ++i) f[i] = fmaf((v[j][i] - mean) * rstd, g[i], b[i]);
      *reinterpret_cast<uint4*>(y + (size_t)row * C + o * 8) = lr_pack8<T>(f);
    }
  }
}


template <int NV, typename T>
__global__ void softmax_rows_kernel(const T* __restrict__ s, T* __restrict__ p, int N, float scale) {
  __shared__ float red[8];
  const size_t row = blockIdx.x;
  const int t = threadIdx.x, lane = t & 63, w = t >> 6;
  const T* src = s + row * (size_t)N;
  T* dst = p + row * (size_t)N;
  float f[NV][8];
  float mx = -INFINITY;
#pragma unroll
  for (int v = 0; v < NV; ++v) {
    const int c = (v * 256 + t) * 8;
    if (c < N) {
      const uint4 u = *reinterpret_cast<const uint4*>(src + c);
      lr_unpack8<T>(u, f[v]);
#pragma unroll
      for (int i = 0; i < 8; ++i) { f[v][i] *= scale; mx = fmaxf(mx, f[v][i]); }
    }
  }
  mx = lr_wave_max(mx);
  if (lane == 0) red[w] = mx;
  __syncthreads();
  mx = fmaxf(fmaxf(red[0], red[1]), fmaxf(red[2], red[3]));
  float sum = 0.f;
#pragma unroll
  for (int v = 0; v < NV; ++v) {
    const int c = (v * 256 + t) * 8;
    if (c < N) {
#pragma unroll
      for (int i = 0; i < 8; ++i) { f[v][i] = __expf(f[v][i] - mx); sum += f[v][i]; }
    }
  }
  sum = lr_wave_sum(sum);
  if (lane == 0) red[4 + w] = sum;
  __syncthreads();
  const float inv = 1.f / ((red[4] + red[5]) + (red[6] + red[7]));
#pragma unroll
  for (int v = 0; v < NV; ++v) {
    const int c = (v * 256 + t) * 8;
    if (c < N) {
#pragma unroll
      for (int i = 0; i < 8; ++i) f[v][i] *= inv;
      *reinterpret_cast<uint4*>(dst + c) = lr_pack8<T>(f[v]);
    }
  }
}

static int gn_nchunks(int N, int HW, int C) {
  const int base_blocks = LR_DEV("LR_GN_STAT_BLOCKS", 256);
  const long long want = ((long long)N * HW * C * 2) >> 19;
  const int target_blocks = want > base_blocks ? (int)want : base_blocks;
  int c = (target_blocks + N - 1) / N;
  if (c > LR_GN_CHUNKS) c = LR_GN_CHUNKS;
  if (c > HW / 8) c = HW / 8;
  if (c < 1) c = 1;
  return c;
}

template <typename T>
static int lr_groupnorm_stats_t(const lr_half* x1, int C1, const lr_half* x2, int C2, int N, int HW, float* partials,
                                  lr_stream_t s) {
  if (!x1 || !partials || N <= 0 || HW <= 0) return LR_E_ARG;
  if (!x2) C2 = 0;
  const int C = C1 + C2;
  if (C % 32 || C1 % 8 || C2 % 8) return LR_E_ALIGN;
  const int nOct = C / 8;
  int R = 256 / nOct;
  if (R < 1) R = 1;
  const int threads = nOct * R;
  if (threads > 1024) return LR_E_UNSUPPORTED;
  const int nchunks = gn_nchunks(N, HW, C);
  dim3 grid(nchunks, N);
  hipLaunchKernelGGL(gn_stats_kernel<T>, grid, dim3(threads), (size_t)R * C * 2 * sizeof(float), (hipStream_t)s,
                     (const T*)x1, C1, (const T*)x2, C2, HW, partials, nOct, R, nchunks);
  return lr_launch_status();
}

__global__ __launch_bounds__(256) void gn_finalize_kernel(const float* __restrict__ p1, int C1, int R1,
                                                          const float* __restrict__ p2, int C2, int R2, int HW,
// ... 130 lines not shown
  if (nchunks <= 0) return LR_E_ARG;
  return groupnorm_apply_impl<T>(x1, C1, x2, C2, N, HW, partials, nchunks, gamma, beta, eps, silu, y, s);
}

template <typename T>
static int groupnorm_apply_impl(const lr_half* x1, int C1, const lr_half* x2, int C2, int N, int HW, const float* partials,
                                int nchunks_in, const float* gamma, const float* beta, float eps, int silu, lr_half* y,
                                lr_stream_t s) {
  if (!x1 || !partials || !gamma || !beta || !y || N <= 0 || HW <= 0) return LR_E_ARG;
  if (!x2) C2 = 0;
  const int C = C1 + C2;
  if (C % 32 || C1 % 8 || C2 % 8) return LR_E_ALIGN;
  int ppb = (int)(((long long)N * HW + 1023) / 1024);
  if (ppb < 16) ppb = 16;
  if (ppb > HW) ppb = HW;
  const int nOct = C / 8;
  int R = 256 / nOct;
  if (R < 1) R = 1;
  const int threads = nOct * R;
  const int base_apply_blocks = LR_DEV("LR_GN_APPLY_BLOCKS", 2048);
  const long long want_blocks = ((long long)N * HW * C * 2) >> 18;
  const long long apply_blocks = want_blocks > base_apply_blocks ? want_blocks : base_apply_blocks;
  ppb = (int)(((long long)N * HW + apply_blocks - 1) / apply_blocks);
  if (ppb < 16) ppb = 16;
  if (ppb > HW) ppb = HW;
  ppb = ((ppb + 4 * R - 1) / (4 * R)) * (4 * R);
  dim3 grid((HW + ppb - 1) / ppb, N);
  if (threads > 1024 || threads < 128) return LR_E_UNSUPPORTED;
  hipLaunchKernelGGL(gn_apply_kernel<T>, grid, dim3(threads), 0, (hipStream_t)s, (const T*)x1, C1, (const T*)x2, C2,
                     HW, partials, gamma, beta, eps, silu, (T*)y, ppb, nOct, R, nchunks_in > 0 ? nchunks_in : gn_nchunks(N, HW, C));
  return lr_launch_status();
}

template <typename T>
static int lr_layernorm_t(const lr_half* x, const float* gamma, const float* beta, float eps, lr_half* y, int M, int C,
                            lr_stream_t s) {
  if (!x || !gamma || !beta || !y || M <= 0) return LR_E_ARG;
  if (C % 8 || C > 2048) return LR_E_ALIGN;
  const int nv = (C / 8 + 63) / 64;
  dim3 grid((M + 3) / 4), block(256);
  hipStream_t st = (hipStream_t)s;
  switch (nv) {
    case 1: hipLaunchKernelGGL((layernorm_kernel<1, T>), grid, block, 0, st, (const T*)x, gamma, beta, eps, (T*)y, M, C); break;
    case 2: hipLaunchKernelGGL((layernorm_kernel<2, T>), grid, block, 0, st, (const T*)x, gamma, beta, eps, (T*)y, M, C); break;
    case 3: hipLaunchKernelGGL((layernorm_kernel<3, T>), grid, block, 0, st, (const T*)x, gamma, beta, eps, (T*)y, M, C); break;
    default: hipLaunchKernelGGL((layernorm_kernel<4, T>), grid, block, 0, st, (const T*)x, gamma, beta, eps, (T*)y, M, C); break;
  }
  return lr_launch_status();
}

extern "C" int lr_softmax_rows_f16(const lr_half* s, lr_half* p, int M, int N, float scale, lr_stream_t st) {
  if (!s || !p || M <= 0 || N <= 0) return LR_E_ARG;
  if (N % 8) return LR_E_ALIGN;
  if (N > 8 * 2048) return LR_E_UNSUPPORTED;
  const int nv = (N + 2047) / 2048;
  dim3 grid(M), block(256);
  hipStream_t hs = (hipStream_t)st;
  if (nv <= 1) hipLaunchKernelGGL((softmax_rows_kernel<1, f16>), grid, block, 0, hs, (const f16*)s, (f16*)p, N, scale);
  else if (nv <= 2) hipLaunchKernelGGL((softmax_rows_kernel<2, f16>), grid, block, 0, hs, (const f16*)s, (f16*)p, N, scale);
  else if (nv <= 4) hipLaunchKernelGGL((softmax_rows_kernel<4, f16>), grid, block, 0, hs, (const f16*)s, (f16*)p, N, scale);
  else hipLaunchKernelGGL((softmax_rows_kernel<8, f16>), grid, block, 0, hs, (const f16*)s, (f16*)p, N, scale);
  return lr_launch_status();
}


template <int NV, typename T>
__global__ void layernorm_bwd_kernel(const T* __restrict__ x, const T* __restrict__ dy, const float* __restrict__ gamma,
                                     float eps, T* __restrict__ dx, int M, int C, const T* __restrict__ dres) {
  const int lane = threadIdx.x & 63;
  const int row = blockIdx.x * (blockDim.x >> 6) + (threadIdx.x >> 6);
  if (row >= M) return;
  const int nOct = C >> 3;
  float v[NV][8], g[NV][8];
  float sum = 0.f;
#pragma unroll
  for (int j = 0; j < NV; ++j) {
    const int o = lane + j * 64;
    if (o < nOct) {
      lr_unpack8<T>(*reinterpret_cast<const uint4*>(x + (size_t)row * C + o * 8), v[j]);
      lr_unpack8<T>(*reinterpret_cast<const uint4*>(dy + (size_t)row * C + o * 8), g[j]);
      const float4 g0 = *reinterpret_cast<const float4*>(gamma + o * 8);
      const float4 g1 = *reinterpret_cast<const float4*>(gamma + o * 8 + 4);
      const float gm[8] = {g0.x, g0.y, g0.z, g0.w, g1.x, g1.y, g1.z, g1.w};
#pragma unroll
      for (int i = 0; i < 8; ++i) { sum += v[j][i]; g[j][i] *= gm[i]; }
    } else {
#pragma unroll
      for (int i = 0; i < 8; ++i) { v[j][i] = 0.f; g[j][i] = 0.f; }
    }
  }
  const float mean = lr_wave_sum(sum) / (float)C;
  float sq = 0.f;
#pragma unroll
  for (int j = 0; j < NV; ++j) {
    const int o = lane + j * 64;
    if (o < nOct) {
#pragma unroll
      for (int i = 0; i < 8; ++i) { const float d = v[j][i] - mean; sq = fmaf(d, d, sq); }
    }
  }
  const float rstd = rsqrtf(lr_wave_sum(sq) / (float)C + eps);
  float s1 = 0.f, s2 = 0.f;
#pragma unroll
  for (int j = 0; j < NV; ++j) {
    const int o = lane + j * 64;
    if (o < nOct) {
#pragma unroll
      for (int i = 0; i < 8; ++i) {
        v[j][i] = (v[j][i] - mean) * rstd;
        s1 += g[j][i];
        s2 = fmaf(g[j][i], v[j][i], s2);
      }
    }
  }
  s1 = lr_wave_sum(s1) / (float)C;
  s2 = lr_wave_sum(s2) / (float)C;
#pragma unroll
  for (int j = 0; j < NV; ++j) {
    const int o = lane + j * 64;
    if (o < nOct) {
      float f[8];
#pragma unroll
      for (int i = 0; i < 8; ++i) f[i] = rstd * (g[j][i] - s1 - v[j][i] * s2);
      if (dres) {
        float e[8];
        lr_unpack8<T>(*reinterpret_cast<const uint4*>(dres + (size_t)row * C + o * 8), e);
#pragma unroll
        for (int i = 0; i < 8; ++i) f[i] += e[i];
      }
      *reinterpret_cast<uint4*>(dx + (size_t)row * C + o * 8) = lr_pack8<T>(f);
    }
  }
}

template <typename T>
static int lr_layernorm_bwd_t(const lr_half* x, const lr_half* dy, const float* gamma, float eps, lr_half* dx, int M,
                                int C, lr_stream_t s, const lr_half* dres = nullptr) {
  if (!x || !dy || !gamma || !dx || M <= 0) return LR_E_ARG;
  if (C % 8 || C > 2048) return LR_E_ALIGN;
  const int nv = (C / 8 + 63) / 64;
  dim3 grid((M + 3) / 4), block(256);
  hipStream_t st = (hipStream_t)s;
  switch (nv) {
    case 1: hipLaunchKernelGGL((layernorm_bwd_kernel<1, T>), grid, block, 0, st, (const T*)x, (const T*)dy, gamma, eps, (T*)dx, M, C, (const T*)dres); break;
    case 2: hipLaunchKernelGGL((layernorm_bwd_kernel<2, T>), grid, block, 0, st, (const T*)x, (const T*)dy, gamma, eps, (T*)dx, M, C, (const T*)dres); break;
    case 3: hipLaunchKernelGGL((layernorm_bwd_kernel<3, T>), grid, block, 0, st, (const T*)x, (const T*)dy, gamma, eps, (T*)dx, M, C, (const T*)dres); break;
    default: hipLaunchKernelGGL((layernorm_bwd_kernel<4, T>), grid, block, 0, st, (const T*)x, (const T*)dy, gamma, eps, (T*)dx, M, C, (const T*)dres); break;
  }
  return lr_launch_status();
}

__device__ __forceinline__ void gn_finalize_stats(const float* __restrict__ partials, int n, int nchunks, int HW, int Cg,
                                                  float eps, float* s_mean, float* s_rstd) {
  const int t = threadIdx.x;
  if (t < 128) {
    const int g = t >> 2, sub = t & 3;
    double s = 0.0, q = 0.0;
    const float* ps = partials + ((size_t)n * nchunks * 32 + g) * 2;
    for (int c = sub; c < nchunks; c += 4) { s += (double)ps[c * 64]; q += (double)ps[c * 64 + 1]; }
#pragma unroll
    for (int sh = 2; sh > 0; sh >>= 1) { s += __shfl_xor(s, sh, 64); q += __shfl_xor(q, sh, 64); }
    if (sub == 0) {
      const double cnt = (double)HW * (double)Cg;
      const double mean = s / cnt;
      double var = q / cnt - mean * mean;
      if (var < 0.0) var = 0.0;
      s_mean[g] = (float)mean;
      s_rstd[g] = (float)(1.0 / sqrt(var + (double)eps));
    }
  }
}

__device__ __forceinline__ float gn_act_grad(float z, int silu) {
  if (!silu) return 1.0f;
  const float sg = __builtin_amdgcn_rcpf(1.0f + __expf(-z));
  return sg * fmaf(z, 1.0f - sg, 1.0f);
}

template <typename T>
__global__ void gn_bwd_stats_kernel(const T* __restrict__ x1, int C1, const T* __restrict__ x2, int C2, int HW,
                                    const T* __restrict__ dy, const float* __restrict__ fwd, const float* __restrict__ gamma,
                                    const float* __restrict__ beta, float eps, int silu, float* __restrict__ out, int nOct,
                                    int R, int nchunks, int fwd_chunks) {
  extern __shared__ float s_part[];
  __shared__ float s_mean[32], s_rstd[32];
  const int C = C1 + C2, Cg = C / 32;
  const int n = blockIdx.y, chunk = blockIdx.x, t = threadIdx.x;
  const int o = t % nOct, r = t / nOct;
  const int per = (HW + nchunks - 1) / nchunks;
  const int p0 = chunk * per, p1 = min(HW, p0 + per);
  const int c0 = o * 8;
  gn_finalize_stats(fwd, n, fwd_chunks, HW, Cg, eps, s_mean, s_rstd);
  __syncthreads();
  const T* src;
  int cs;
  if (c0 < C1) { src = x1 + ((size_t)n * HW) * C1 + c0; cs = C1; } else { src = x2 + ((size_t)n * HW) * C2 + (c0 - C1); cs = C2; }
  const T* gsrc = dy + ((size_t)n * HW) * C + c0;
  float mu[8], rs[8], ga[8], be[8], s1[8], s2[8];
#pragma unroll
  for (int i = 0; i < 8; ++i) {
    const int g = (c0 + i) / Cg;
    mu[i] = s_mean[g]; rs[i] = s_rstd[g]; ga[i] = gamma[c0 + i]; be[i] = beta[c0 + i];
    s1[i] = 0.f; s2[i] = 0.f;
  }
  auto accum = [&](const uint4& ux, const uint4& ug) {
    float xv[8], gv[8];
    lr_unpack8<T>(ux, xv);
    lr_unpack8<T>(ug, gv);
#pragma unroll
    for (int i = 0; i < 8; ++i) {
      const float xh = (xv[i] - mu[i]) * rs[i];
      const float z = fmaf(xh, ga[i], be[i]);
      const float g = gv[i] * gn_act_grad(z, silu) * ga[i];
      s1[i] += g;
      s2[i] = fmaf(g, xh, s2[i]);
    }
  };
  int p = p0 + r;
  for (; p + 3 * R < p1; p += 4 * R) {
    uint4 ux[4], ug[4];
#pragma unroll
    for (int k = 0; k < 4; ++k) {
      ux[k] = *reinterpret_cast<const uint4*>(src + (size_t)(p + k * R) * cs);
      ug[k] = *reinterpret_cast<const uint4*>(gsrc + (size_t)(p + k * R) * C);
    }
#pragma unroll
    for (int k = 0; k < 4; ++k) accum(ux[k], ug[k]);
  }
  for (; p < p1; p += R)
    accum(*reinterpret_cast<const uint4*>(src + (size_t)p * cs), *reinterpret_cast<const uint4*>(gsrc + (size_t)p * C));
#pragma unroll
  for (int i = 0; i < 8; ++i) {
    s_part[((size_t)r * C + c0 + i) * 2 + 0] = s1[i];
    s_part[((size_t)r * C + c0 + i) * 2 + 1] = s2[i];
  }
  __syncthreads();
  if (t < 32) {
    float a = 0.f, b = 0.f;
    for (int c = t * Cg; c < (t + 1) * Cg; ++c)
      for (int rr = 0; rr < R; ++rr) { a += s_part[((size_t)rr * C + c) * 2]; b += s_part[((size_t)rr * C + c) * 2 + 1]; }
    float* dst = out + (((size_t)n * nchunks + chunk) * 32 + t) * 2;
    dst[0] = a;
    dst[1] = b;
  }
}

template <typename T>
__global__ void gn_bwd_apply_kernel(const T* __restrict__ x1, int C1, const T* __restrict__ x2, int C2, int HW,
                                    const T* __restrict__ dy, const float* __restrict__ fwd, const float* __restrict__ bwd,
                                    const float* __restrict__ gamma, const float* __restrict__ beta, float eps, int silu,
                                    T* __restrict__ dx1, T* __restrict__ dx2, int pix_per_block, int nOct, int R,
                                    int nchunks, int fwd_chunks, const T* __restrict__ dres1, const T* __restrict__ dres2) {
  __shared__ float s_mean[32], s_rstd[32], s_c1[32], s_c2[32];
  const int C = C1 + C2, Cg = C / 32;
  const int n = blockIdx.y, t = threadIdx.x;
  const int o = t % nOct, r = t / nOct;
  const int c0 = o * 8;
  const int p0 = blockIdx.x * pix_per_block, p1 = min(HW, p0 + pix_per_block);
  gn_finalize_stats(fwd, n, fwd_chunks, HW, Cg, eps, s_mean, s_rstd);
  __syncthreads();
  if (t < 128) {
    const int g = t >> 2, sub = t & 3;
    double a = 0.0, b = 0.0;
    const float* ps = bwd + ((size_t)n * nchunks * 32 + g) * 2;
    for (int c = sub; c < nchunks; c += 4) { a += (double)ps[c * 64]; b += (double)ps[c * 64 + 1]; }
#pragma unroll
    for (int sh = 2; sh > 0; sh >>= 1) { a += __shfl_xor(a, sh, 64); b += __shfl_xor(b, sh, 64); }
    if (sub == 0) {
      const double m = (double)HW * (double)Cg;
      s_c1[g] = (float)(a / m);
      s_c2[g] = (float)(b / m);
    }
  }
  __syncthreads();
  if (r >= R) return;
  const T* src;
  const T* rsrc;
  T* dst;
  int cs;
  if (c0 < C1) { src = x1 + ((size_t)n * HW) * C1 + c0; dst = dx1 + ((size_t)n * HW) * C1 + c0; cs = C1; rsrc = dres1 ? dres1 + ((size_t)n * HW) * C1 + c0 : nullptr; }
  else { src = x2 + ((size_t)n * HW) * C2 + (c0 - C1); dst = dx2 + ((size_t)n * HW) * C2 + (c0 - C1); cs = C2; rsrc = dres2 ? dres2 + ((size_t)n * HW) * C2 + (c0 - C1) : nullptr; }
  const T* gsrc = dy + ((size_t)n * HW) * C + c0;
  float mu[8], rs[8], ga[8], be[8], k1[8], k2[8];
#pragma unroll
  for (int i = 0; i < 8; ++i) {
    const int g = (c0 + i) / Cg;
    mu[i] = s_mean[g]; rs[i] = s_rstd[g]; ga[i] = gamma[c0 + i]; be[i] = beta[c0 + i];
    k1[i] = s_c1[g]; k2[i] = s_c2[g];
  }
  auto emit = [&](int pp, const uint4& ux, const uint4& ug) {
    float xv[8], gv[8], f[8];
    lr_unpack8<T>(ux, xv);
    lr_unpack8<T>(ug, gv);
#pragma unroll
    for (int i = 0; i < 8; ++i) {
      const float xh = (xv[i] - mu[i]) * rs[i];
      const float z = fmaf(xh, ga[i], be[i]);
      const float g = gv[i] * gn_act_grad(z, silu) * ga[i];
      f[i] = rs[i] * (g - k1[i] - xh * k2[i]);
    }
    if (rsrc) {
      float e[8];
      lr_unpack8<T>(*reinterpret_cast<const uint4*>(rsrc + (size_t)pp * cs), e);
#pragma unroll
      for (int i = 0; i < 8; ++i) f[i] += e[i];
    }
    *reinterpret_cast<uint4*>(dst + (size_t)pp * cs) = lr_pack8<T>(f);
  };
  int p = p0 + r;
  for (; p + 3 * R < p1; p += 4 * R) {
    uint4 ux[4], ug[4];
#pragma unroll
    for (int k = 0; k < 4; ++k) {
      ux[k] = *reinterpret_cast<const uint4*>(src + (size_t)(p + k * R) * cs);
      ug[k] = *reinterpret_cast<const uint4*>(gsrc + (size_t)(p + k * R) * C);
    }
#pragma unroll
    for (int k = 0; k < 4; ++k) emit(p + k * R, ux[k], ug[k]);
  }
  for (; p < p1; p += R)
    emit(p, *reinterpret_cast<const uint4*>(src + (size_t)p * cs), *reinterpret_cast<const uint4*>(gsrc + (size_t)p * C));
}

// ... 58 lines not shown
```

### leftrefill_amd/engine.py

```python
import math
from dataclasses import dataclass
from typing import Optional

import torch

from . import packing
from . import train_ops as ops
from .ops import plan_batch_scale

_COMPUTE = [torch.float16]


def compute_dtype():
    return _COMPUTE[0]


class compute:

    def __init__(self, dtype):
        if dtype not in (torch.float16, torch.bfloat16):
            raise ValueError(f"compute dtype must be float16 or bfloat16, got {dtype}")
        self.dtype = dtype

    def __enter__(self):
        self.prev = _COMPUTE[0]
        _COMPUTE[0] = self.dtype

    def __exit__(self, *exc):
        _COMPUTE[0] = self.prev


@dataclass
class Act:
    tok: torch.Tensor
    N: int
    H: int
    W: int
    tok2: Optional[torch.Tensor] = None
    gs: Optional[tuple] = None
    gs2: Optional[tuple] = None

    @property
    def HW(self):
        return self.H * self.W

    def materialize(self):
        if self.tok2 is None:
            return self.tok
        return torch.cat([self.tok, self.tok2], dim=1).contiguous()


def f32(p):
    return p.detach().float().contiguous()


class PackedConv:
    def __init__(self, conv, cin_pad=None):
        w = conv.weight.detach()
        self.cout = w.shape[0]
        self.taps = w.shape[2] * w.shape[3]
        self.w = packing.pack_conv(w, cin_pad=cin_pad, dtype=compute_dtype())
        if cin_pad == 16 and self.taps == 9:
            self.w = torch.cat([self.w, self.w.new_zeros(self.w.shape[0], 192 - self.w.shape[1])], dim=1).contiguous()
        self.b = packing.pack_bias(conv.bias.detach(), self.w.shape[0]) if conv.bias is not None else None
        self.stride = conv.stride[0]


class PackedLinear:

    def __init__(self, lin=None, weight=None, bias=None, norm=None):
        if lin is not None:
            weight, bias = lin.weight, lin.bias
        w = weight.detach()
        if w.dim() == 4:
            w = w.reshape(w.shape[0], w.shape[1])
        self.w = packing.pack_linear(w, compute_dtype())
        self.b = f32(bias) if bias is not None else None
        self.wf = None
        if norm is not None:
            self.wf, self.bf, self.cs = packing.fold_layernorm(w, None if bias is None else bias.detach(),
                                                               norm.weight.detach(), norm.bias.detach(), compute_dtype())
            self.eps = float(norm.eps)


class PackedNorm:
    def __init__(self, norm):
        self.g = f32(norm.weight)
        self.b = f32(norm.bias)
        self.eps = float(norm.eps)


class PackedRes:
    def __init__(self, blk):
        self.n1 = PackedNorm(blk.in_layers[0])
        self.c1 = PackedConv(blk.in_layers[2])
        self.emb = PackedLinear(blk.emb_layers[1])
        self.n2 = PackedNorm(blk.out_layers[0])
        self.c2 = PackedConv(blk.out_layers[3])
        self.skip = None
        self._c2s = None
        self._c2s_ok = False
        sk = blk.skip_connection
        if isinstance(sk, torch.nn.Conv2d):
            self.skip = PackedConv(sk)
            self._c2s_ok = (sk.kernel_size == (1, 1) and self.c2.taps == 9 and self.c2.stride == 1
                            and self.skip.w.shape[0] == self.c2.w.shape[0])
        self.cout = self.c1.cout

    @property
    def c2s(self):
        if self._c2s is None and self._c2s_ok:
            self._c2s = FusedSkipConv(self.c2, self.skip)
        return self._c2s


class FusedSkipConv:

    def __init__(self, c2, skip):
        self.w = torch.cat([c2.w, skip.w], dim=1).contiguous()
        b2 = c2.b if c2.b is not None else torch.zeros(c2.w.shape[0], device=c2.w.device)
        self.b = (b2 + skip.b) if skip.b is not None else c2.b
        self.cout, self.taps, self.stride = c2.cout, 9, 1


class PackedAttn:

    def __init__(self, attn, is_self, norm=None):
        self.heads = attn.heads
        self.is_self = is_self
        if is_self:
            self.qkv = PackedLinear(weight=torch.cat([attn.to_q.weight, attn.to_k.weight, attn.to_v.weight], 0), norm=norm)
        else:
            self.q = PackedLinear(weight=attn.to_q.weight, norm=norm)
            self.kv = PackedLinear(weight=torch.cat([attn.to_k.weight, attn.to_v.weight], 0))
        self.out = PackedLinear(attn.to_out[0])
        self.xk = None
        if not is_self and norm is not None and attn.to_q.weight.shape[0] in ops.XATTN_WIDTHS:
            self.xk, self.xwo = packing.pack_xattn(attn.to_k.weight.detach(), attn.to_out[0].weight.detach(), compute_dtype())
            self.xq_pi = self.q.wf[:, packing.xattn_perm(self.q.wf.shape[1], self.q.wf.device)].contiguous()
        self.dim_head = attn.to_q.weight.shape[0] // attn.heads
        if self.dim_head != 64:
            raise RuntimeError(f"attention kernel is specialised for d_head=64 (got {self.dim_head})")


class PackedTBlock:
    def __init__(self, blk):
        if getattr(blk, "disable_self_attn", False):
            raise RuntimeError("disable_self_attn=True is not used by LeftRefill configs and is unsupported")
        self.attn1 = PackedAttn(blk.attn1, True, blk.norm1)
        self.attn2 = PackedAttn(blk.attn2, False, blk.norm2)
        self.n1, self.n2, self.n3 = PackedNorm(blk.norm1), PackedNorm(blk.norm2), PackedNorm(blk.norm3)
        proj = blk.ff.net[0].proj
        self.geglu_w, self.geglu_b = packing.pack_geglu(proj.weight.detach(), proj.bias.detach(), compute_dtype())
        wf, bf, cs = packing.fold_layernorm(proj.weight.detach(), proj.bias.detach(), blk.norm3.weight.detach(),
                                            blk.norm3.bias.detach(), compute_dtype())
        perm = packing.geglu_perm(proj.weight.shape[0] // 2, proj.weight.device)
        self.geglu_wf, self.geglu_bf, self.geglu_cs = wf[perm].contiguous(), bf[perm].contiguous(), cs[perm].contiguous()
        self.ff2 = PackedLinear(blk.ff.net[2])
        self.ff2_x = None
        if self.ff2.w.shape[0] == ops.FFN_C and self.ff2.w.shape[1] % 64 == 0:
            self.ff2_x = packing.pack_pieces(blk.ff.net[2].weight.detach(), compute_dtype())
        self.kv_slot = None
        self.view_num = getattr(blk, "view_num", None)
        self.concat_target = getattr(blk, "concat_target", False)
        self.no_rearrange = getattr(blk, "no_rearrange_selfattn", False)
        if self.concat_target and self.no_rearrange:
            raise NotImplementedError("no_rearrange_selfattn=True with concat_target=True is unusable in the reference and not implemented")


class PackedST:
    def __init__(self, st):
        self.norm = PackedNorm(st.norm)
        self.proj_in = PackedLinear(st.proj_in)
        self.blocks = [PackedTBlock(b) for b in st.transformer_blocks]
        self.proj_out = PackedLinear(st.proj_out)
        self.proj_out_x = None
        if self.proj_out.w.shape == (ops.FFN_C, ops.FFN_C) and self.proj_out.b is not None:
            w_ = st.proj_out.weight.detach()
            self.proj_out_x = packing.pack_pieces(w_.reshape(w_.shape[0], w_.shape[1]), compute_dtype())
        self._ff_proj = None
        self._ff_src = None
        ff2 = st.transformer_blocks[-1].ff.net[2]
        wp = st.proj_out.weight
        if wp.shape[0] == wp.shape[1] == ff2.weight.shape[0] and wp.shape[1] % 64 == 0:
            self._ff_src = (st.proj_out, ff2, compute_dtype())

    def _build_ff_proj(self):
        if self._ff_proj is None and self._ff_src is not None:
            assert not (torch.cuda.is_available() and torch.cuda.is_current_stream_capturing()), "PackedST.ff_proj_w built inside a graph capture: call UNetModel.finalize_inference() first"
            proj_out, ff2, dt = self._ff_src
            wp = proj_out.weight.detach().float()
            wp = wp.reshape(wp.shape[0], wp.shape[1])
            dev_ = wp.device
            wp64, w2_64 = wp.double().cpu(), ff2.weight.detach().double().cpu()
            w = torch.cat([(wp64 @ w2_64).float(), wp64.float()], dim=1).to(device=dev_, dtype=dt).contiguous()
            b2 = ff2.bias.detach().double().cpu() if ff2.bias is not None else torch.zeros(w2_64.shape[0], dtype=torch.float64)
            bp = proj_out.bias.detach().double().cpu() if proj_out.bias is not None else torch.zeros(wp64.shape[0], dtype=torch.float64)
            self._ff_proj = (w, (wp64 @ b2 + bp).float().to(dev_).contiguous())
        return self._ff_proj

    @property
    def ff_proj_w(self):
        p_ = self._build_ff_proj()
        return None if p_ is None else p_[0]

    @property
    def ff_proj_b(self):
        p_ = self._build_ff_proj()
        return None if p_ is None else p_[1]


def linear(x, pl: PackedLinear, resid=None, M=None, want_stats=False):
    M = x.shape[0] if M is None else M
    return ops.gemm_conv(x, pl.w, B=1, H=1, W=M, taps=1, bias=pl.b, resid=resid, want_stats=want_stats)


def fold_ok(x):
    return LN_FOLD and not (torch.is_grad_enabled() and x.requires_grad)


def ln_linear(x, st, pn: PackedNorm, pl: PackedLinear, wide=None):
    if wide and pl.wf is not None and fold_ok(x) and ops.rowlin_ok(x.shape[0], x.shape[1], pl.wf.shape[0], wide):
        return ops.rowlin(x, pl.wf, pl.bf, eps=pl.eps)
    if st is not None and pl.wf is not None and fold_ok(x):
        return ops.gemm_conv(x, pl.wf, B=1, H=1, W=x.shape[0], taps=1, bias=pl.bf, ln=(st, pl.eps, pl.cs))
    return linear(ops.layer_norm(x, pn.g, pn.b, pn.eps), pl)


GN_FUSE = __import__("os").environ.get("LEFTREFILL_GN_FUSE", "1") != "0"
SKIP_FUSED = __import__("os").environ.get("LEFTREFILL_SKIP_FUSED", "1") != "0"
FF_PROJ = __import__("os").environ.get("LEFTREFILL_FF_PROJ", "1") != "0"


def gn_fuse_ok(x):
    return GN_FUSE and not (torch.is_grad_enabled() and x.requires_grad)


TRAIN_GN_STATS = __import__("os").environ.get("LEFTREFILL_TRAIN_GN_STATS", "1") != "0"
TRAIN_FORK = __import__("os").environ.get("LEFTREFILL_TRAIN_FORK", "1") != "0"


TRAIN_SKIP_FUSED = __import__("os").environ.get("LEFTREFILL_TRAIN_SKIP_FUSED", "1") != "0"


def gn_stats_ok(x):
    return GN_FUSE and (TRAIN_GN_STATS or not torch.is_grad_enabled())


def training(x):
    return torch.is_grad_enabled() and x.requires_grad


def forking(x):
    return TRAIN_FORK and training(x)


def conv(act: Act, pc: PackedConv, rowvec=None, resid=None, up=0, asym=False, gn_stats=False, skip=None, skip_parts=None):
    if pc.taps == 9:
        if up:
            H, W = act.H * 2, act.W * 2
        elif pc.stride == 2:
            H, W = act.H // 2, act.W // 2
        else:
            H, W = act.H, act.W
    else:
        H, W = act.H, act.W
    want = gn_stats and gn_stats_ok(act.tok) and pc.cout == pc.w.shape[0]
    extra = {} if skip_parts is None else {"skip_parts": skip_parts}
    y = ops.gemm_conv(act.tok, pc.w, B=act.N, H=H, W=W, Hs=act.H, Ws=act.W, taps=pc.taps, stride=pc.stride, up=up,
                      asym=asym, x2=act.tok2, bias=pc.b, rowvec=rowvec, resid=resid, want_gn_stats=want, skip=skip, **extra)
    y, gs = y if want else (y, None)
    return Act(y, act.N, H, W, gs=gs)


def _gn_train_stats(act: Act):
    HW = act.HW
    if not (act.gs is not None and HW % act.gs[1] == 0 and gn_stats_ok(act.tok)
            and (act.tok2 is None or (act.gs2 is not None and HW % act.gs2[1] == 0))):
        return None
    if act.tok2 is None and act.gs[2] is not None:
        return ("groups", act.gs[2], act.gs[3])
    return ("channels", act.gs, act.gs2)


def gn(act: Act, pn: PackedNorm, silu):
    HW = act.HW
    if training(act.tok) or (act.tok2 is not None and training(act.tok2)):
        return Act(ops.group_norm(act.tok, act.N, HW, pn.g, pn.b, pn.eps, silu, act.tok2, stats=_gn_train_stats(act)), act.N, act.H, act.W)
    fused = (act.gs is not None and HW % act.gs[1] == 0 and gn_fuse_ok(act.tok)
             and (act.tok2 is None or (act.gs2 is not None and HW % act.gs2[1] == 0)))
    if fused and act.tok2 is None and act.gs[2] is not None:
        y = ops.group_norm_groups(act.tok, act.N, HW, pn.g, pn.b, pn.eps, silu, act.gs[2], act.gs[3])
    elif fused:
        y = ops.group_norm_fused(act.tok, act.N, HW, pn.g, pn.b, pn.eps, silu, act.gs, act.tok2, act.gs2)
    else:
        y = ops.group_norm(act.tok, act.N, HW, pn.g, pn.b, pn.eps, silu, act.tok2)
    return Act(y, act.N, act.H, act.W)


def gn_fork(act: Act, pn: PackedNorm, silu):
    y, t1, t2 = ops.group_norm_fork(act.tok, act.N, act.HW, pn.g, pn.b, pn.eps, silu, act.tok2, stats=_gn_train_stats(act))
    return Act(y, act.N, act.H, act.W), Act(t1, act.N, act.H, act.W, tok2=t2)


def resblock(act: Act, pr: PackedRes, emb_out):
    if forking(act.tok) or (act.tok2 is not None and forking(act.tok2)):
        h, act = gn_fork(act, pr.n1, True)
    else:
        h = gn(act, pr.n1, True)
    h = conv(h, pr.c1, rowvec=emb_out, gn_stats=True)
    h = gn(h, pr.n2, True)
    if pr.c2s is not None and SKIP_FUSED and gn_fuse_ok(act.tok) and gn_fuse_ok(h.tok) and (act.tok2 is None or gn_fuse_ok(act.tok2)):
        return conv(h, pr.c2s, gn_stats=True, skip=(act.tok, act.tok2))
    if (pr.c2s is not None and SKIP_FUSED and TRAIN_SKIP_FUSED and (training(h.tok) or training(act.tok) or (act.tok2 is not None and training(act.tok2)))
            and h.tok2 is None):
        return conv(h, pr.c2s, gn_stats=True, skip=(act.tok, act.tok2), skip_parts=(pr.c2.w, pr.skip.w))
    if pr.skip is not None:
        resid = conv(act, pr.skip).tok
    else:
        resid = act.materialize()
    return conv(h, pr.c2, resid=resid, gn_stats=True)


def attention_plain(x, ctx, pa: PackedAttn, B, L, Lc=None):
    if pa.is_self:
        a = ops.attention_qkv(linear(x, pa.qkv), B, pa.heads, L, pa.dim_head ** -0.5)
    else:
        a = ops.attention_q_kv(linear(x, pa.q), linear(ctx, pa.kv), B, pa.heads, L, Lc, pa.dim_head ** -0.5)
    return linear(a, pa.out)


def self_attention(x, st, pn, pa: PackedAttn, B, L, want_stats=False, qkv=None, wide=None):
    if qkv is None and forking(x):
        n, x = ops.layer_norm_fork(x, pn.g, pn.b, pn.eps)
        qkv = linear(n, pa.qkv)
    qkv = ln_linear(x, st, pn, pa.qkv, wide=wide) if qkv is None else qkv
    a = ops.attention_qkv(qkv, B, pa.heads, L, pa.dim_head ** -0.5)
    return linear(a, pa.out, resid=x, want_stats=want_stats)


def dup2(t):
    return torch.cat([t, t], dim=0)


def xattn_fused(x, pa: PackedAttn, B, L, Lc, kv):
    return (XATTN and kv is not None and len(kv) > 2 and fold_ok(x) and ops.xattn_ok(B * L, L, x.shape[1], pa.heads, Lc))


def ffn_fused(x, pt, rows=None, ctx=None):
    rows = x.shape[0] if rows is None else rows
    if ctx is not None and torch.is_grad_enabled() and ctx.requires_grad:
        return False
    return FFN_FUSED and pt.ff2_x is not None and fold_ok(x) and ops.ffn_ok(rows, x.shape[1], pt.ff2_x.shape[0] * 64)


XATTN_PRE = __import__("os").environ.get("LEFTREFILL_XATTN_PRE", "1") != "0"


def self_then_cross_attention(x, st, pt, N, L, Lc, kv, want_stats, dup=False, qkv0=None):
    pa1, pa2 = pt.attn1, pt.attn2
    if dup:
        with plan_batch_scale(2):
            qkv = ln_linear(x, st, pt.n1, pa1.qkv, wide="qkv") if qkv0 is None else qkv0
        a = dup2(ops.attention_qkv(qkv, N // 2, pa1.heads, L, pa1.dim_head ** -0.5))
        x = dup2(x)
    else:
        qkv = ln_linear(x, st, pt.n1, pa1.qkv, wide="qkv") if qkv0 is None else qkv0
        a = ops.attention_qkv(qkv, N, pa1.heads, L, pa1.dim_head ** -0.5)
    return ops.xattn_block(x, pa2.xq_pi, pa2.q.bf, kv[2], kv[3], pa2.xwo, pa2.out.b, HW=L, heads=pa2.heads, Lc=Lc, eps=pa2.q.eps,
                           scale=pa2.dim_head ** -0.5, want_stats=want_stats, pre=(a, pa1.out.w, pa1.out.b))


def cross_attention(x, st, pn, ctx, pa: PackedAttn, B, L, Lc, kv=None, want_stats=False, dup=False, fused=None):
    if xattn_fused(x, pa, B, L, Lc, kv) if fused is None else fused:
        if dup:
            x = dup2(x)
        return ops.xattn_block(x, pa.q.wf, pa.q.bf, kv[2], kv[3], pa.xwo, pa.out.b, HW=L, heads=pa.heads, Lc=Lc, eps=pa.q.eps,
                               scale=pa.dim_head ** -0.5, want_stats=want_stats)
    if dup:
        with plan_batch_scale(2):
            q = ln_linear(x, st, pn, pa.q, wide="q")
        q, x = dup2(q), dup2(x)
    elif forking(x):
        n, x = ops.layer_norm_fork(x, pn.g, pn.b, pn.eps)
        q = linear(n, pa.q)
    else:
        q = ln_linear(x, st, pn, pa.q, wide="q")
    vt = None
    if kv is None:
        kv = linear(ctx, pa.kv)
    else:
        kv, vt = kv[0], kv[1]
    a = ops.attention_q_kv(q, kv, B, pa.heads, L, Lc, pa.dim_head ** -0.5, vt=vt)
    return linear(a, pa.out, resid=x, want_stats=want_stats)


def transformer_block(x, ctx, pt: PackedTBlock, N, L, Lc, kv=None, st=None, want_stats=False, dup=False, post=None, qkv0=None, ffn_split=False):
    use_xattn = xattn_fused(x, pt.attn2, N, L, Lc, kv)
    use_ffn = ffn_fused(x, pt, rows=N * L, ctx=ctx) and not ffn_split
    ws = fold_ok(x) and not use_xattn
    if pt.view_num is None and XATTN_PRE and use_xattn and pt.attn1.out.b is not None:
        ws = fold_ok(x) and not use_ffn
        x = self_then_cross_attention(x, st, pt, N, L, Lc, kv, ws, dup=dup, qkv0=qkv0)
        x, st = x if ws else (x, None)
        return _ffn(x, st, pt, want_stats, post, use_ffn)
    if pt.view_num is None and dup:
        with plan_batch_scale(2):
            x = self_attention(x, st, pt.n1, pt.attn1, N // 2, L, want_stats=ws, qkv=qkv0, wide="qkv")
    elif pt.view_num is None:
        x = self_attention(x, st, pt.n1, pt.attn1, N, L, want_stats=ws, qkv=qkv0, wide="qkv")
    elif pt.concat_target and not pt.no_rearrange and MV_SHARDED:
        x = _mv_sharded_self_attention(x, pt, N, L, st)
        ws = False
    elif pt.concat_target and not pt.no_rearrange:
        v = pt.view_num - 1
        b = N // v
        s = int(math.sqrt(L / 2))
        assert 2 * s * s == L and b * v == N, "concat_target needs square halves and batch = b*(view_num-1)"
        seq = ops.mv_gather(x, b, v, s)
        Ls = pt.view_num * s * s
        st_seq = None
        if st is not None and fold_ok(x) and MV_LN_FOLD:
            g = st.reshape(b, v, s, 2 * s, st.shape[1] * 2)
            st_seq = torch.cat((g[:, 0:1, :, s:], g[:, :, :, :s]), dim=1).reshape(b * Ls, st.shape[1], 2).contiguous()
        seq = self_attention(seq, st_seq, pt.n1, pt.attn1, b, Ls)
        x = ops.mv_scatter(seq, b, v, s)
        ws = False
    else:
        v = pt.view_num - 1 if pt.concat_target else pt.view_num
        b = N // v
        assert b * v == N
        x = self_attention(x, st, pt.n1, pt.attn1, b, v * L, want_stats=ws)
    x, st = x if ws else (x, None)
    ws = fold_ok(x) and not use_ffn
    x = cross_attention(x, st, pt.n2, ctx, pt.attn2, N, L, Lc, kv, want_stats=ws, dup=dup, fused=use_xattn)
    x, st = x if ws else (x, None)
    return _ffn(x, st, pt, want_stats, post, use_ffn)


FFN_POST = __import__("os").environ.get("LEFTREFILL_FFN_POST", "1") != "0"


def _ffn(x, st, pt: PackedTBlock, want_stats, post=None, fused=None):
    fused = ffn_fused(x, pt) if fused is None else fused
    compose = post is not None and post[0] == "compose"
    if compose and (fused or (torch.is_grad_enabled() and x.requires_grad)):
        compose, post = False, None
    if post is not None and not compose and FFN_POST and fused:
        pw, pb, x_in, want_gn, hw = post
        y = ops.ffn_block(x, pt.geglu_wf, pt.geglu_bf, pt.ff2_x, pt.ff2.b, eps=pt.n3.eps, post=(pw, pb, x_in), want_gn_stats=want_gn,
                          gn_hw=hw)
        return ("post",) + (y if want_gn else (y, None))
    if fused:
        ws = want_stats and fold_ok(x)
        y = ops.ffn_block(x, pt.geglu_wf, pt.geglu_bf, pt.ff2_x, pt.ff2.b, eps=pt.n3.eps, want_stats=ws)
        return y if ws else (y, None)
    if fold_ok(x) and ops.rowlin_ok(x.shape[0], x.shape[1], pt.geglu_wf.shape[0], "geglu"):
        g = ops.rowlin(x, pt.geglu_wf, pt.geglu_bf, eps=pt.n3.eps, geglu=True)
    elif st is not None:
        g = ops.gemm_conv(x, pt.geglu_wf, B=1, H=1, W=x.shape[0], taps=1, bias=pt.geglu_bf, geglu=True,
                          ln=(st, pt.n3.eps, pt.geglu_cs))
    else:
        n3, x = (ops.layer_norm_fork if TRAIN_FORK else (lambda *a_: (ops.layer_norm(*a_), x)))(x, pt.n3.g, pt.n3.b, pt.n3.eps)
        g = ops.gemm_conv(n3, pt.geglu_w, B=1, H=1, W=n3.shape[0], taps=1, bias=pt.geglu_b, geglu=True)
# ... 197 lines not shown
```

### leftrefill_amd/ops.py

```python
import ctypes
import os

import torch

from . import _lib
from ._lib import FfnArgs, GemmArgs, RowlinArgs, StinArgs, XattnArgs

GN_CHUNKS = 256
GN_GROUPS = os.environ.get("LEFTREFILL_GN_GROUPS", "1") != "0"

AUTOTUNE = os.environ.get("LEFTREFILL_AUTOTUNE", "0") == "1"
TILE_CANDIDATES = ((128, 64, 0), (128, 128, 0), (128, 160, 0), (128, 128, 4), (128, 160, 4), (256, 128, 0), (256, 160, 0),
                   (256, 256, 0), (256, 320, 0), (256, 160, 8), (256, 320, 8))
TILE_TABLE_PATH = os.environ.get("LEFTREFILL_TILE_TABLE_PATH",
                                 os.path.join(os.path.dirname(os.path.abspath(__file__)), "tile_table.json"))
_tile_cache = None
PLAN_LOG = os.environ.get("LEFTREFILL_PLAN_LOG", "0") == "1"
SPLITK_MODE = int(os.environ.get("LEFTREFILL_SPLITK_MODE", "0"))
_untabulated = set()
TABLE_HITS, TABLE_MISSES = set(), set()
PLAN_TRIAL = None
LAUNCH_HOOK = None


_PLAN_BATCH_SCALE = [1]


class plan_batch_scale:
    def __init__(self, scale):
        self.scale = int(scale)

    def __enter__(self):
        self.prev = _PLAN_BATCH_SCALE[0]
        _PLAN_BATCH_SCALE[0] = self.scale

    def __exit__(self, *exc):
        _PLAN_BATCH_SCALE[0] = self.prev


def tile_key(M, N, K, taps=1, stride=1, up=0, geglu=False, concat=False, asym=False, gelu=False, ln=False, stats=False):
    return "%d,%d,%d,%d,%d,%d,%d,%d,%d,%d,%d,%d" % (M, N, K, taps, stride, up, int(geglu), int(concat), int(asym),
                                                      int(gelu), int(ln), int(stats))


def tile_cache():
    global _tile_cache
    if _tile_cache is None:
        _tile_cache = {}
        if os.path.exists(TILE_TABLE_PATH) and os.environ.get("LEFTREFILL_TILE_TABLE", "1") != "0":
            import json
            with open(TILE_TABLE_PATH) as f:
                _tile_cache = {k: tuple(v) for k, v in json.load(f).items()}
    return _tile_cache


def _stream():
    return torch.cuda.current_stream().cuda_stream


def _p(t):
    return 0 if t is None else t.data_ptr()


HALF_TYPES = (torch.float16, torch.bfloat16)


def _chk16(t, name):
    assert t.is_cuda and t.dtype in HALF_TYPES and t.is_contiguous(), f"{name}: need contiguous cuda fp16 / bf16"


def _fn(lib, name, dtype):
    return _lib.fn(lib, name, dtype)


def nchw_to_nhwc(x1, x2=None, cpad=None, dtype=torch.float16):
    lib = _lib.load()
    N, C1, H, W = x1.shape
    C2 = 0 if x2 is None else x2.shape[1]
    cpad = cpad or ((C1 + C2 + 7) // 8) * 8
    x1 = x1.float().contiguous()
    x2 = None if x2 is None else x2.float().contiguous()
    y = torch.empty(N * H * W, cpad, device=x1.device, dtype=dtype)
    _lib.check(_fn(lib, "lr_nchw_f32_to_nhwc_f16", dtype)(_p(x1), C1, _p(x2), C2, _p(y), cpad, N, H, W, _stream()), "nchw_to_nhwc")
    return y


def nhwc_to_nchw(y, N, H, W, C, out_dtype=None):
    lib = _lib.load()
    _chk16(y, "y")
    out_dtype = y.dtype if out_dtype is None or out_dtype in HALF_TYPES else out_dtype
    out = torch.empty(N, C, H, W, device=y.device, dtype=out_dtype)
    _lib.check(_fn(lib, "lr_nhwc_f16_to_nchw", y.dtype)(_p(y), y.shape[-1], C, _p(out), int(out_dtype == torch.float32), N, H, W,
                                       _stream()), "nhwc_to_nchw")
    return out


def group_norm(x1, N, HW, gamma, beta, eps, silu, x2=None):
    lib = _lib.load()
    _chk16(x1, "x1")
    C1 = x1.shape[-1]
    C2 = 0
    if x2 is not None:
        _chk16(x2, "x2")
        C2 = x2.shape[-1]
    assert gamma.dtype == torch.float32 and beta.dtype == torch.float32 and gamma.numel() == C1 + C2
    partials = torch.empty(N * GN_CHUNKS * 64, device=x1.device, dtype=torch.float32)
    y = torch.empty(N * HW, C1 + C2, device=x1.device, dtype=x1.dtype)
    st = _stream()
    _lib.check(_fn(lib, "lr_groupnorm_stats", x1.dtype)(_p(x1), C1, _p(x2), C2, N, HW, _p(partials), st), "groupnorm_stats")
    _lib.check(_fn(lib, "lr_groupnorm_apply", x1.dtype)(_p(x1), C1, _p(x2), C2, N, HW, _p(partials), _p(gamma), _p(beta), float(eps),
                                      int(bool(silu)), _p(y), st), "groupnorm_apply")
    return y


def group_norm_fused(x1, N, HW, gamma, beta, eps, silu, gs1, x2=None, gs2=None):
    lib = _lib.load()
    _chk16(x1, "x1")
    C1 = x1.shape[-1]
    C2 = 0 if x2 is None else x2.shape[-1]
    p1, r1 = gs1[:2]
    p2, r2 = gs2[:2] if x2 is not None else (None, 1)
    assert p1.shape == (N * HW // r1, C1, 2) and HW % r1 == 0
    if x2 is not None:
        _chk16(x2, "x2")
        assert p2.shape == (N * HW // r2, C2, 2) and HW % r2 == 0
    assert gamma.dtype == torch.float32 and beta.dtype == torch.float32 and gamma.numel() == C1 + C2
    partials = torch.empty(N * 64, device=x1.device, dtype=torch.float32)
    y = torch.empty(N * HW, C1 + C2, device=x1.device, dtype=x1.dtype)
    st = _stream()
    _lib.check(lib.lr_groupnorm_finalize(_p(p1), C1, r1, _p(p2), C2, r2, N, HW, _p(partials), st), "groupnorm_finalize")
    _lib.check(_fn(lib, "lr_groupnorm_apply_n", x1.dtype)(_p(x1), C1, _p(x2), C2, N, HW, _p(partials), 1, _p(gamma), _p(beta), float(eps),
                                        int(bool(silu)), _p(y), st), "groupnorm_apply_n")
    return y


def group_norm_groups(x1, N, HW, gamma, beta, eps, silu, gp, chunks):
    lib = _lib.load()
    _chk16(x1, "x1")
    C1 = x1.shape[-1]
    assert gp.dtype == torch.float32 and gp.is_contiguous() and gp.shape == (N, chunks, 32, 2), (gp.shape, N, chunks)
    assert gamma.dtype == torch.float32 and beta.dtype == torch.float32 and gamma.numel() == C1
    y = torch.empty(N * HW, C1, device=x1.device, dtype=x1.dtype)
    _lib.check(_fn(lib, "lr_groupnorm_apply_n", x1.dtype)(_p(x1), C1, 0, 0, N, HW, _p(gp), chunks, _p(gamma), _p(beta), float(eps),
                                                          int(bool(silu)), _p(y), _stream()), "groupnorm_apply_n")
    return y


OUT_FUSED = os.environ.get("LEFTREFILL_OUT_FUSED", "1") != "0"


def gn_conv_out_ok(H, W, C, cout):
    return OUT_FUSED and 1 <= cout <= 4 and C % 64 == 0 and 64 <= C <= 704 and H % 8 == 0 and W % 16 == 0


def gn_conv_out(x, N, H, W, gamma, beta, eps, gp, chunks, w, bias, cout):
    lib = _lib.load()
    _chk16(x, "x")
    _chk16(w, "w")
    C = x.shape[1]
    assert x.shape[0] == N * H * W and gn_conv_out_ok(H, W, C, cout), (x.shape, N, H, W, cout)
    assert gp.dtype == torch.float32 and gp.is_contiguous() and gp.shape == (N, chunks, 32, 2), (gp.shape, N, chunks)
    assert gamma.dtype == torch.float32 and beta.dtype == torch.float32 and gamma.numel() == C and beta.numel() == C
    assert w.dtype == x.dtype and w.shape[0] >= cout and w.shape[1] == 9 * C and (bias is None or (bias.dtype == torch.float32 and bias.numel() >= cout))
    y = torch.empty(N, cout, H, W, device=x.device, dtype=x.dtype)
    _lib.check(_fn(lib, "lr_gn_conv_out_f16", x.dtype)(_p(x), N, H, W, C, _p(gp), chunks, _p(gamma), _p(beta), float(eps), _p(w), w.stride(0),
                                                       _p(bias), cout, _p(y), _stream()), "gn_conv_out")
    return y


def gn_fold_weights(gp, chunks, N, HW, gamma, beta, eps, w, bias):
    lib = _lib.load()
    if not _lib.dev_variants():
        raise RuntimeError("lr_gn_fold_weights_f16 is compiled in developer builds only (tools/build_variant.sh)")
    _chk16(w, "w")
    Nout, C = w.shape
    assert gp.dtype == torch.float32 and gp.is_contiguous() and gp.shape == (N, chunks, 32, 2)
    wb = torch.empty(N, Nout, C, device=w.device, dtype=w.dtype)
    bb = torch.empty(N, Nout, device=w.device, dtype=torch.float32)
    _lib.check(_fn(lib, "lr_gn_fold_weights_f16", w.dtype)(_p(gp), chunks, N, HW, C, _p(gamma), _p(beta), float(eps), _p(w), _p(bias), Nout,
                                                           _p(wb), _p(bb), _stream()), "gn_fold_weights")
    return wb, bb


def layer_norm(x, gamma, beta, eps=1e-5):
    lib = _lib.load()
    _chk16(x, "x")
    M, C = x.shape
    y = torch.empty_like(x)
    _lib.check(_fn(lib, "lr_layernorm", x.dtype)(_p(x), _p(gamma), _p(beta), float(eps), _p(y), M, C, _stream()), "layernorm")
    return y


def timestep_embedding(t, dim, dtype=torch.float16):
    lib = _lib.load()
    name = "lr_timestep_embedding_f32" if t.is_floating_point() else "lr_timestep_embedding"
    t = t.to(torch.float32 if t.is_floating_point() else torch.int64).contiguous()
    out = torch.empty(t.shape[0], dim, device=t.device, dtype=dtype)
    _lib.check(_fn(lib, name, dtype)(_p(t), t.shape[0], dim, _p(out), _stream()), "timestep_embedding")
    return out


def linear_small_m(a, w, bias, act_in=False, act_out=False):
    lib = _lib.load()
    _chk16(a, "a")
    _chk16(w, "w")
    M, K = a.shape
    N = w.shape[0]
    out = torch.empty(M, N, device=a.device, dtype=a.dtype)
    st = _stream()
    for m0 in range(0, M, 16):
        mc = min(16, M - m0)
        _lib.check(_fn(lib, "lr_linear_small_m", a.dtype)(a[m0:].data_ptr(), K, _p(w), _p(bias), out[m0:].data_ptr(), N, mc, N, K,
                                         int(act_in), int(act_out), st), "linear_small_m")
    return out


def gemm_conv(x1, wt, *, B, H, W, Hs=None, Ws=None, taps=1, stride=1, up=0, asym=False, x2=None, bias=None, rowvec=None,
              resid=None, geglu=False, gelu=False, out=None, tile_n=0, tile_m=0, splits=0, pipe=0, ln=None,
              want_stats=False, want_gn_stats=False, gn_hw=0, per_sample=False, wt_pm=False, skip=None):
    lib = _lib.load()
    _chk16(x1, "x1")
    _chk16(wt, "wt")
    Hs = H if Hs is None else Hs
    Ws = W if Ws is None else Ws
    C1 = x1.shape[-1]
    C2 = 0
    if x2 is not None:
        _chk16(x2, "x2")
        C2 = x2.shape[-1]
    if per_sample:
        assert wt.dim() == 3 and wt.shape[0] == B and taps == 1 and x2 is None and wt.is_contiguous() and not wt_pm
    if wt_pm:
        assert wt.dim() == 3 and wt.shape[2] == 64 and wt.is_contiguous()
        Nw, Kw = wt.shape[1], wt.shape[0] * 64
    else:
        Nw, Kw = wt.shape[-2], wt.shape[-1]
    c16 = C1 == 16 and C2 == 0 and taps == 9 and Kw == 192
    Cs1 = Cs2 = 0
    if skip is not None:
        s1, s2 = skip
        _chk16(s1, "skip1")
        Cs1 = s1.shape[-1]
        if s2 is not None:
            _chk16(s2, "skip2")
            Cs2 = s2.shape[-1]
        assert stride == 1 and not up and s1.shape[0] == B * H * W and (s2 is None or s2.shape[0] == s1.shape[0])
    assert c16 or Kw == taps * (C1 + C2) + Cs1 + Cs2, (wt.shape, taps, C1, C2, Cs1, Cs2)
    if c16 and tile_m == 0 and tile_n == 0:
        tile_m, tile_n, splits = 256, (320 if Nw % 320 == 0 else 160 if Nw % 160 == 0 else 128), 1
    assert x1.shape[0] == B * Hs * Ws, (x1.shape, B, Hs, Ws)
    M = B * H * W
    n_out = Nw // 2 if geglu else Nw
    if out is None:
        out = torch.empty(M, n_out, device=x1.device, dtype=x1.dtype)
    a = GemmArgs()
    a.p1, a.C1, a.p2, a.C2 = _p(x1), C1, _p(x2), C2
    a.B, a.H, a.W, a.Hs, a.Ws = B, H, W, Hs, Ws
    a.taps, a.stride, a.up, a.asym = taps, stride, up, int(bool(asym))
    a.wt, a.N = _p(wt), Nw
    a.bias = _p(bias)
    if bias is not None:
        assert bias.dtype == torch.float32 and bias.numel() == (Nw * B if per_sample else Nw)
    a.rowvec, a.ld_rowvec = _p(rowvec), (rowvec.stride(0) if rowvec is not None else 0)
    a.resid, a.ld_resid = _p(resid), (resid.stride(0) if resid is not None else 0)
    if resid is not None:
        assert resid.shape[0] == M and resid.dtype == x1.dtype
    a.out, a.ld_out = _p(out), out.stride(0)
    assert not (geglu and gelu)
    a.geglu = 2 if gelu else int(geglu)
    a.tile_n = tile_n
    a.tile_m = tile_m
    a.splits = splits
    a.pipe = pipe
    a.workspace, a.workspace_bytes = 0, 0
    a.ln_stats, a.ln_parts, a.ln_eps, a.ln_colsum, a.stats_out, a.gn_stats_out = 0, 0, 0.0, 0, 0, 0
    a.gn_group_out, a.gn_hw = 0, int(gn_hw)
    a.wt_bstride, a.bias_bstride = (Nw * Kw, Nw if bias is not None else 0) if per_sample else (0, 0)
    a.wt_pm = int(bool(wt_pm))
    a.skip1, a.skip2, a.Cs1, a.Cs2 = (_p(skip[0]), _p(skip[1]), Cs1, Cs2) if skip is not None else (0, 0, 0, 0)
    a.splitk_mode = SPLITK_MODE
    assert wt.dtype == x1.dtype, (wt.dtype, x1.dtype)
    a.dtype = int(x1.dtype == torch.bfloat16)
    if ln is not None:
        st_in, eps, colsum = ln
        assert st_in.dtype == torch.float32 and st_in.is_contiguous() and st_in.shape[0] == M and st_in.shape[2] == 2
        assert colsum.dtype == torch.float32 and colsum.numel() == Nw and taps == 1 and x2 is None
        a.ln_stats, a.ln_parts, a.ln_eps, a.ln_colsum = _p(st_in), st_in.shape[1], float(eps), _p(colsum)
    st = _stream()
    if tile_m == 0 and tile_n == 0 and splits == 0:
        scale = _PLAN_BATCH_SCALE[0]
        key = tile_key(M * scale, Nw, Kw - Cs1 - Cs2, taps, stride, up, geglu, C2 > 0, asym, gelu, ln is not None, want_stats)
        best = tile_cache().get(key)
        (TABLE_HITS if best is not None else TABLE_MISSES).add(key)
        if best is None and PLAN_LOG and key not in _untabulated:
            _untabulated.add(key)
            import sys
            print(f"[leftrefill] untabulated GEMM shape {key} (taps {taps}, H {H}, W {W}, skip {skip is not None})", file=sys.stderr, flush=True)
        if best is None and (scale != 1 or (HEURISTIC_REFINE and not AUTOTUNE and skip is None and not per_sample and not c16)):
            a.B = B * scale
            if ln is not None or want_stats:
                a.splits = 1
            best = _refine_plan(lib, a, geglu or gelu) if HEURISTIC_REFINE and skip is None and not per_sample and not c16 else _lib_plan(lib, a)
            a.B, a.splits, a.tile_m, a.tile_n, a.pipe = B, 0, 0, 0, 0
        if best is None and AUTOTUNE and not torch.cuda.is_current_stream_capturing():
            best = _tune_tiles(lib, a, x1.device, geglu, ln is not None or want_stats, want_stats)
            tile_cache()[key] = best
        if best is not None and PLAN_TRIAL is not None and PLAN_TRIAL.get(key) is not None:
            best = PLAN_TRIAL[key]
        if best is not None:
            a.tile_m, a.tile_n, a.splits = best[:3]
            a.pipe = best[3] if len(best) > 3 else 0
            if a.pipe == 8 and (W % 16 or (H % 16 and not (H == 8 and M % 256 == 0 and (M * scale) % 256 == 0))):
                a.pipe = 0
        if skip is not None and best is None:
            plan = (ctypes.c_int32 * 4)()
            lib.lr_gemm_plan(a, plan)
            a.tile_m, a.tile_n, a.splits, a.pipe = plan[0], plan[1], plan[2], plan[3]
    stats = None
    if want_stats:
        if a.splits == 0:
            a.splits = 1
        parts = lib.lr_gemm_stats_parts(a)
        stats = torch.empty(M, parts, 2, device=x1.device, dtype=torch.float32)
        a.stats_out = _p(stats)
    if ln is not None and a.splits == 0:
        a.splits = 1
    gstats = None
    if want_gn_stats:
        plan = (ctypes.c_int32 * 4)()
        lib.lr_gemm_plan(a, plan)
        a.splits = plan[2]
        rows = lib.lr_gemm_gn_rows(a)
        hw = gn_hw or H * W
        if hw % rows == 0:
            chunks = lib.lr_gemm_gn_group_chunks(a) if GN_GROUPS else 0
            gp = torch.empty(M // hw, chunks, 32, 2, device=x1.device, dtype=torch.float32) if chunks > 0 else None
            gstats = (torch.empty((M + rows - 1) // rows, n_out, 2, device=x1.device, dtype=torch.float32), rows, gp, chunks)
            a.gn_stats_out = _p(gstats[0])
            a.gn_group_out = _p(gp)
    ws = _workspace(lib, a, x1.device)
    if LAUNCH_HOOK is not None and tile_m == 0 and tile_n == 0 and splits == 0:
        plan = (ctypes.c_int32 * 4)()
        lib.lr_gemm_plan(a, plan)
        LAUNCH_HOOK(key, 0, tuple(plan))
        rc = lib.lr_gemm_conv_f16(a, st)
        LAUNCH_HOOK(key, 1, rc)
        if rc != 0 and PLAN_TRIAL is not None and PLAN_TRIAL.get(key) is not None:
            PLAN_TRIAL[key] = None
            return gemm_conv(x1, wt, B=B, H=H, W=W, Hs=Hs, Ws=Ws, taps=taps, stride=stride, up=up, asym=asym, x2=x2, bias=bias, rowvec=rowvec,
                             resid=resid, geglu=geglu, gelu=gelu, out=out, ln=ln, want_stats=want_stats, want_gn_stats=want_gn_stats, gn_hw=gn_hw,
                             per_sample=per_sample, wt_pm=wt_pm, skip=skip)
        _lib.check(rc, "gemm_conv")
    else:
        _lib.check(lib.lr_gemm_conv_f16(a, st), "gemm_conv")
    if want_gn_stats:
        return out, gstats
    return (out, stats) if want_stats else out


HEURISTIC_REFINE = os.environ.get("LEFTREFILL_HEURISTIC_REFINE", "1") != "0"


def _lib_plan(lib, a):
    plan = (ctypes.c_int32 * 4)()
    lib.lr_gemm_plan(a, plan)
    return tuple(plan)


def _refine_plan(lib, a, act_epilogue):
    base = _lib_plan(lib, a)
    tm, tn = base[0], base[1]
    M = a.B * a.H * a.W
    if (a.taps == 9 and a.stride == 1 and a.up == 0 and not a.asym and not act_epilogue and not a.ln_stats and not a.stats_out and a.W % 16 == 0
            and a.H % 16 == 0 and a.Hs == a.H and a.Ws == a.W and a.N % 160 == 0 and M >= 8192 and (a.C1 + a.C2) % 64 == 0 and M < (1 << 28)):
        tn = 320 if a.N % 320 == 0 and ((M + 255) // 256) * (a.N // 320) >= 200 else 160
        keep = (a.tile_m, a.tile_n, a.pipe)
        a.tile_m, a.tile_n, a.pipe = 256, tn, 8
        plan = _lib_plan(lib, a)
        a.tile_m, a.tile_n, a.pipe = keep
        return (256, tn, plan[2], 8)
    if tm != 128 or act_epilogue:
        return base
    if a.N % 160 == 0:
        tn = 160
    if tn not in (128, 160) or ((M + 127) // 128) * ((a.N + tn - 1) // tn) > 256:
        return base
    keep = (a.tile_m, a.tile_n, a.pipe)
    a.tile_m, a.tile_n, a.pipe = 128, tn, 4
    plan = _lib_plan(lib, a)
    a.tile_m, a.tile_n, a.pipe = keep
    return (128, tn, plan[2], 4)


def gemm_plan(M, N, K, **kw):
    best = tile_cache().get(tile_key(M, N, K, **kw))
    if best is not None:
        return tuple(best) if len(best) > 3 else tuple(best) + (0,)
    lib = _lib.load()
    a = GemmArgs()
    a.B, a.H, a.W, a.N, a.taps, a.C1 = 1, 1, M, N, kw.get("taps", 1), K // kw.get("taps", 1)
    a.geglu = int(kw.get("geglu", False))
    if kw.get("ln") or kw.get("stats"):
        a.splits = 1
    plan = _refine_plan(lib, a, bool(kw.get("geglu") or kw.get("gelu"))) if HEURISTIC_REFINE else _lib_plan(lib, a)
    return tuple(plan)[:3] + (plan[3] if plan[3] in (4, 8) else 0,)


def _workspace(lib, a, device):
    a.workspace, a.workspace_bytes = 0, 0
    need = lib.lr_gemm_workspace_bytes(a)
    if need <= 0:
        return None
    ws = torch.empty(need // 4, device=device, dtype=torch.float32)
    a.workspace, a.workspace_bytes = ws.data_ptr(), need
    return ws


def _time_launch(lib, a, st, reps, rounds):
    t = float("inf")
    for _ in range(rounds):
        e0, e1 = torch.cuda.Event(enable_timing=True), torch.cuda.Event(enable_timing=True)
        e0.record()
        for _ in range(reps):
            lib.lr_gemm_conv_f16(a, st)
        e1.record()
        e1.synchronize()
        t = min(t, e0.elapsed_time(e1))
    return t


def _tune_tiles(lib, a, device, geglu, no_split, want_stats, reps=4, rounds=2):
    st = _stream()
    best, best_t = None, float("inf")
    plan = (ctypes.c_int32 * 4)()
    for tm, tn, stg in TILE_CANDIDATES:
        if geglu and tn == 160:
            continue
        a.tile_m, a.tile_n, a.splits, a.pipe = tm, tn, 0, stg
        lib.lr_gemm_plan(a, plan)
        cands = {1} if no_split else {1, int(plan[2])}
        for sp in sorted(cands):
            a.splits = sp
            stats = None
            if want_stats:
                parts = lib.lr_gemm_stats_parts(a)
                stats = torch.empty(a.B * a.H * a.W, parts, 2, device=device, dtype=torch.float32)
                a.stats_out = stats.data_ptr()
            ws = _workspace(lib, a, device)
            if sp > 1 and ws is None:
                continue
            if lib.lr_gemm_conv_f16(a, st) != 0:
                continue
            t = _time_launch(lib, a, st, reps, rounds)
            del ws, stats
            if t < best_t:
                best, best_t = (tm, tn, sp, stg), t
    a.stats_out = 0
    return best


VT_MIN_KEYS = int(os.environ.get("LEFTREFILL_VT_MIN_KEYS", "1024"))
ATTN_VT = os.environ.get("LEFTREFILL_ATTN_VT", "0") != "0"


def transpose_v(v, B, heads, Nkv, out=None):
    lib = _lib.load()
    assert v.is_cuda and v.dtype in HALF_TYPES and v.stride(1) == 1
    ld = ((Nkv + 63) // 64) * 64
    vt = torch.empty(B, heads * 64, ld, device=v.device, dtype=v.dtype) if out is None else out
    assert vt.shape == (B, heads * 64, ld) and vt.is_contiguous()
    _lib.check(_fn(lib, "lr_transpose_v_f16", v.dtype)(_p(v), v.stride(0), _p(vt), ld, B, heads, Nkv, _stream()), "transpose_v")
    return vt


def attention(q, k, v, B, heads, Nq, Nkv, scale, out=None, vt=None):
    lib = _lib.load()
    for t_ in (q, k, v):
        assert t_.is_cuda and t_.dtype == q.dtype and q.dtype in HALF_TYPES and t_.stride(1) == 1
    if out is None:
        out = torch.empty(B * Nq, heads * 64, device=q.device, dtype=q.dtype)
    if vt is None and ATTN_VT and Nkv >= VT_MIN_KEYS:
        vt = transpose_v(v, B, heads, Nkv)
    if vt is not None:
        _lib.check(_fn(lib, "lr_attention_vt_f16", q.dtype)(_p(q), q.stride(0), _p(k), k.stride(0), _p(vt), vt.shape[2], _p(out),
                                           out.stride(0), B, heads, Nq, Nkv, float(scale), _stream()), "attention_vt")
        return out
    _lib.check(_fn(lib, "lr_attention_f16", q.dtype)(_p(q), q.stride(0), _p(k), k.stride(0), _p(v), v.stride(0), _p(out), out.stride(0),
                                    B, heads, Nq, Nkv, float(scale), _stream()), "attention")
    return out


def attention_causal(q, k, v, B, heads, N, scale):
    lib = _lib.load()
    for t_ in (q, k, v):
        assert t_.is_cuda and t_.dtype == q.dtype and q.dtype in HALF_TYPES and t_.stride(1) == 1
    out = torch.empty(B * N, heads * 64, device=q.device, dtype=q.dtype)
    _lib.check(_fn(lib, "lr_attention_causal_f16", q.dtype)(_p(q), q.stride(0), _p(k), k.stride(0), _p(v), v.stride(0), _p(out), out.stride(0),
                                           B, heads, N, float(scale), _stream()), "attention_causal")
    return out


def attention_qkv(qkv, B, heads, L, scale):
    C = heads * 64
    return attention(qkv[:, :C], qkv[:, C:2 * C], qkv[:, 2 * C:], B, heads, L, L, scale)
# ... 322 lines not shown
```

Measured before the change: 4.484 images/s.

## Fuse deferred GroupNorm+SiLU into halo conv prologue for ResBlock convs

ResBlock GroupNorm(+SiLU) is deferred so it no longer writes a normalized activation. Instead the halo 3x3 conv kernel computes group stats and per-channel coefficients in shared memory, then normalizes each loaded patch chunk before the MMA. This removes a full read/write pass over the activation per ResBlock norm. In exchange the conv kernel does more ALU and shared-memory work, uses more shared memory, and needs extra barriers. Shapes the halo path cannot take fall back to a separate apply kernel.

```diff
diff --git a/include/leftrefill_hip.h b/include/leftrefill_hip.h
--- a/include/leftrefill_hip.h
+++ b/include/leftrefill_hip.h
@@ -75,6 +75,8 @@
   int32_t wt_pm;
   const lr_half* skip1; const lr_half* skip2; int32_t Cs1, Cs2;
   int32_t splitk_mode;
+  const float* gn_in_part; const float* gn_in_gamma; const float* gn_in_beta;
+  int32_t gn_in_chunks; float gn_in_eps; int32_t gn_in_silu;
 } lr_gemm_args;
 int lr_gemm_gn_group_chunks(const lr_gemm_args* args);
 int lr_gemm_gn_rows(const lr_gemm_args* args);
diff --git a/leftrefill_amd/_lib.py b/leftrefill_amd/_lib.py
--- a/leftrefill_amd/_lib.py
+++ b/leftrefill_amd/_lib.py
@@ -3,7 +3,7 @@
 
 HERE = os.path.dirname(os.path.abspath(__file__))
 LIB_PATH = os.environ.get("LEFTREFILL_LIB_PATH") or os.path.join(HERE, "lib", "libleftrefill_hip.so")
-ABI_VERSION = 29
+ABI_VERSION = 30
 
 c_void_p, c_int, c_float, c_int64 = ctypes.c_void_p, ctypes.c_int, ctypes.c_float, ctypes.c_int64
 
@@ -37,6 +37,8 @@
         ("wt_pm", ctypes.c_int32),
         ("skip1", c_void_p), ("skip2", c_void_p), ("Cs1", ctypes.c_int32), ("Cs2", ctypes.c_int32),
         ("splitk_mode", ctypes.c_int32),
+        ("gn_in_part", c_void_p), ("gn_in_gamma", c_void_p), ("gn_in_beta", c_void_p),
+        ("gn_in_chunks", ctypes.c_int32), ("gn_in_eps", ctypes.c_float), ("gn_in_silu", ctypes.c_int32),
     ]
 
 
diff --git a/leftrefill_amd/build.py b/leftrefill_amd/build.py
--- a/leftrefill_amd/build.py
+++ b/leftrefill_amd/build.py
@@ -32,7 +32,7 @@
     objdir = os.path.join(HERE, "build")
     os.makedirs(objdir, exist_ok=True)
     cc = hipcc()
-    headers = [os.path.join(CSRC, "common.h"), os.path.join(CSRC, "chain_common.h"), os.path.join(CSRC, "gemm_common.h"), os.path.join(HERE, "..", "include", "leftrefill_hip.h")]
+    headers = [os.path.join(CSRC, "common.h"), os.path.join(CSRC, "chain_common.h"), os.path.join(CSRC, "gn_elem.h"), os.path.join(CSRC, "gemm_common.h"), os.path.join(HERE, "..", "include", "leftrefill_hip.h")]
     jobs = []
     for s in SOURCES:
         src = os.path.join(CSRC, s)
diff --git a/leftrefill_amd/csrc/chain_common.h b/leftrefill_amd/csrc/chain_common.h
--- a/leftrefill_amd/csrc/chain_common.h
+++ b/leftrefill_amd/csrc/chain_common.h
@@ -1,5 +1,6 @@
 #pragma once
 #include "common.h"
+#include "gn_elem.h"
 
 typedef __attribute__((address_space(3))) void* lptr_t;
 
@@ -53,29 +54,11 @@
                                              float eps, float* tabA, float* tabB, float* s_mr , int t, int nthreads) {
 #if defined(__HIP_DEVICE_COMPILE__)
   const int Cg = C / 32;
-  if (t < 128) {
-    const int g = t >> 2, sub = t & 3;
-    double s = 0.0, q = 0.0;
-    const float* ps = gp + ((size_t)n * nchunks * 32 + g) * 2;
-#pragma unroll 4
-    for (int c = sub; c < nchunks; c += 4) { s += (double)ps[c * 64]; q += (double)ps[c * 64 + 1]; }
-#pragma unroll
-    for (int sh = 2; sh > 0; sh >>= 1) { s += __shfl_xor(s, sh, 64); q += __shfl_xor(q, sh, 64); }
-    if (sub == 0) {
-      const double cnt = (double)HW * (double)Cg;
-      const double mean = s / cnt;
-      double var = q / cnt - mean * mean;
-      if (var < 0.0) var = 0.0;
-      s_mr[g] = (float)mean;
-      s_mr[32 + g] = (float)(1.0 / sqrt(var + (double)eps));
-    }
-  }
+  lr_gn_group_stats(gp, n, nchunks, HW, Cg, eps, s_mr, s_mr + 32, t);
   __syncthreads();
   for (int c = t; c < C; c += nthreads) {
     const int g = c / Cg;
-    const float a = s_mr[32 + g] * gamma[c];
-    tabA[c] = a;
-    tabB[c] = beta[c] - s_mr[g] * a;
+    lr_gn_coef(s_mr[g], s_mr[32 + g], gamma[c], beta[c], tabA[c], tabB[c]);
   }
   __syncthreads();
 #endif
diff --git a/leftrefill_amd/csrc/conv_halo.hip b/leftrefill_amd/csrc/conv_halo.hip
--- a/leftrefill_amd/csrc/conv_halo.hip
+++ b/leftrefill_amd/csrc/conv_halo.hip
@@ -1,4 +1,5 @@
 #include "gemm_common.h"
+#include "gn_elem.h"
 
 #ifndef HALO_EXP
 #define HALO_EXP 0
@@ -6,7 +7,7 @@
 #define HALO_PW 18
 #define HALO_NQ 45
 
-template <int BN, int WMW, int NSTAGE, typename T>
+template <int BN, int WMW, int NSTAGE, typename T, bool GN>
 __global__ __launch_bounds__(512) void conv_halo_kernel(const GemmParams P) {
 #if defined(__HIP_DEVICE_COMPILE__)
   constexpr int NW = 8, WNW = NW / WMW, TM = 16 / WMW, TN = BN / WNW / 16;
@@ -21,6 +22,8 @@
   char* const patch = smem;
   char* const wring = smem + PATCH_BYTES;
   float* const par = reinterpret_cast<float*>(wring + NSTAGE * B_BYTES);
+  [[maybe_unused]] float* const gn_mr = par + 2 * PAR_LD;
+  [[maybe_unused]] float* const gn_a = gn_mr + 128;
 
   const int t = threadIdx.x;
   const int lane = t & 63;
@@ -81,6 +84,34 @@
     }
   };
 
+  [[maybe_unused]] float* const gn_b = gn_a + (seg ? 2 : 1) * Ctot;
+  [[maybe_unused]] auto gn_patch = [&](const int ci, auto silu_c) __attribute__((always_inline)) {
+    constexpr int SILU = decltype(silu_c)::value;
+    int tt = t;
+    asm volatile("" : "+v"(tt));
+    char* const slot0 = patch + tt * 16;
+#pragma unroll
+    for (int k = 0; k < 6; ++k) {
+      const int q = w + 8 * k;
+      if (q < nq && pix[k] >= 0) {
+        uint4* const slot = reinterpret_cast<uint4*>(slot0 + k * 8192);
+        const int ch = ((seg && (tt >> 3) + 64 * k >= 10 * HALO_PW) ? Ctot : 0) + ci * 64 + (pix[k] >> 28) * 8;
+        float a[8], b[8];
+        *reinterpret_cast<float4*>(a) = *reinterpret_cast<const float4*>(gn_a + ch);
+        *reinterpret_cast<float4*>(a + 4) = *reinterpret_cast<const float4*>(gn_a + ch + 4);
+        *reinterpret_cast<float4*>(b) = *reinterpret_cast<const float4*>(gn_b + ch);
+        *reinterpret_cast<float4*>(b + 4) = *reinterpret_cast<const float4*>(gn_b + ch + 4);
+        *slot = lr_gn_octet<T>(*slot, a, b, SILU);
+      }
+    }
+  };
+  [[maybe_unused]] auto gn_chunk = [&](const int ci) __attribute__((always_inline)) {
+    if (ci < ncm) {
+      if (P.gi_silu) gn_patch(ci, std::integral_constant<int, 1>{}); else gn_patch(ci, std::integral_constant<int, 0>{});
+    }
+    asm volatile("s_waitcnt lgkmcnt(0)" ::: "memory");
+  };
+
   const __amdgpu_buffer_rsrc_t rsB = uniform_rsrc((const void*)P.wt, (size_t)P.N * P.K * 2);
   const __amdgpu_buffer_rsrc_t rsZ = uniform_rsrc((const void*)P.wt, 0);
   __amdgpu_buffer_rsrc_t rsW = rsB;
@@ -143,6 +174,13 @@
   using std::integral_constant;
 
   LR_STAMP(0);
+  if constexpr (GN) {
+    const int nsmp = seg ? 2 : 1;
+    if (t < 128 * nsmp)
+      lr_gn_group_stats(P.gi_part, nsmp * smp + (t >> 7), P.gi_chunks, P.H * P.W, Ctot >> 5, P.gi_eps, gn_mr + 32 * (t >> 7),
+                        gn_mr + 64 + 32 * (t >> 7), t & 127);
+    __syncthreads();
+  }
   stage_params<BN, PAR_LD>(P, par, n0, w, lane, 0);
   if (nsteps > 0) issue_patch(c_begin);
   int wci = c_begin, wtap = 0;
@@ -151,6 +189,16 @@
     if (sidx < nsteps) { issue_weights(sidx, wkoff(wci, wtap)); advance(wci, wtap); }
   }
   LR_STAMP(1);
+  if constexpr (GN) {
+    const int Cg = Ctot >> 5, nsmp = seg ? 2 : 1;
+    const int cb = min(c_begin, ncm) * 64, ce = min(nch, ncm) * 64;
+    for (int sg = 0; sg < nsmp; ++sg)
+      for (int c = cb + t; c < ce; c += 512) {
+        const int g = c / Cg;
+        lr_gn_coef(gn_mr[32 * sg + g], gn_mr[64 + 32 * sg + g], P.gi_gamma[c], P.gi_beta[c], gn_a[sg * Ctot + c], gn_b[sg * Ctot + c]);
+      }
+    __syncthreads();
+  }
 #pragma unroll
   for (int j = 0; j < TN; ++j)
 #pragma unroll
@@ -160,6 +208,7 @@
   } else {
     wait_vmcnt<0>();
   }
+  if constexpr (GN) { if (nsteps > 0) gn_chunk(c_begin); }
   __builtin_amdgcn_s_barrier();
   LR_STAMP(2);
 
@@ -192,6 +241,7 @@
     } else {
       wait_vmcnt<0>();
     }
+    if constexpr (GN) { if (pf_p) gn_chunk(ci + 1); }
     __builtin_amdgcn_s_barrier();
     cur = cur + 1 == NSTAGE ? 0 : cur + 1;
     advance(ci, tap);
@@ -223,7 +273,9 @@
 #endif
 }
 
-template <int BN, int WMW, int NSTAGE, typename T>
+#define HALO_GN_MAX_C 3072
+
+template <int BN, int WMW, int NSTAGE, typename T, bool GN>
 static int launch_halo_t(const GemmParams& P0, hipStream_t st) {
   GemmParams P = P0;
   P.ntiles_n = (P.N + BN - 1) / BN;
@@ -231,13 +283,14 @@
   P.m_fastest = 0;
   if (LR_DEV("LR_HALO_MFASTEST", 0) && P.splits > 1) P.m_fastest = 1;
   P.nblocks = P.ntiles_n * P.ntiles_m;
-  const size_t smem = (size_t)HALO_NQ * 1024 + NSTAGE * (size_t)BN * 128 + 2 * (((BN + 63) / 64) * 64) * sizeof(float);
+  const size_t base = (size_t)HALO_NQ * 1024 + NSTAGE * (size_t)BN * 128 + 2 * (((BN + 63) / 64) * 64) * sizeof(float);
+  const size_t smem = base + (GN ? (128 + 2 * (size_t)(P.H == 8 ? 2 : 1) * (P.C1 + P.C2)) * sizeof(float) : 0);
   static unsigned long long attr_done = 0;
   if (lr_attr_needed(&attr_done)) {
-    hipFuncSetAttribute(reinterpret_cast<const void*>(conv_halo_kernel<BN, WMW, NSTAGE, T>), hipFuncAttributeMaxDynamicSharedMemorySize,
-                        (int)smem);
-  }
-  hipLaunchKernelGGL((conv_halo_kernel<BN, WMW, NSTAGE, T>), dim3(P.nblocks, P.splits), dim3(512), smem, st, P);
+    hipFuncSetAttribute(reinterpret_cast<const void*>(conv_halo_kernel<BN, WMW, NSTAGE, T, GN>), hipFuncAttributeMaxDynamicSharedMemorySize,
+                        (int)(base + (GN ? (128 + 2 * HALO_GN_MAX_C) * sizeof(float) : 0)));
+  }
+  hipLaunchKernelGGL((conv_halo_kernel<BN, WMW, NSTAGE, T, GN>), dim3(P.nblocks, P.splits), dim3(512), smem, st, P);
   return lr_launch_status();
 }
 
@@ -246,8 +299,14 @@
       P.wt_bstride || P.st_out || ((P.H & 15) && !(P.H == 8 && P.M % 256 == 0)) || (P.W & 15) || P.Hs != P.H || P.Ws != P.W)
     return LR_E_UNSUPPORTED;
   if ((long long)P.M >= (1ll << 28)) return LR_E_UNSUPPORTED;
-  if (tile_n == 320) return P.bf16 ? launch_halo_t<320, 2, 2, bf16>(P, st) : launch_halo_t<320, 2, 2, f16>(P, st);
-  if (tile_n == 160) return P.bf16 ? launch_halo_t<160, 4, 3, bf16>(P, st) : launch_halo_t<160, 4, 3, f16>(P, st);
+  if (P.gi_part) {
+    if ((P.C1 + P.C2) * (P.H == 8 ? 2 : 1) > HALO_GN_MAX_C) return LR_E_UNSUPPORTED;
+    if (tile_n == 320) return P.bf16 ? launch_halo_t<320, 2, 2, bf16, true>(P, st) : launch_halo_t<320, 2, 2, f16, true>(P, st);
+    if (tile_n == 160) return P.bf16 ? launch_halo_t<160, 4, 3, bf16, true>(P, st) : launch_halo_t<160, 4, 3, f16, true>(P, st);
+    return LR_E_UNSUPPORTED;
+  }
+  if (tile_n == 320) return P.bf16 ? launch_halo_t<320, 2, 2, bf16, false>(P, st) : launch_halo_t<320, 2, 2, f16, false>(P, st);
+  if (tile_n == 160) return P.bf16 ? launch_halo_t<160, 4, 3, bf16, false>(P, st) : launch_halo_t<160, 4, 3, f16, false>(P, st);
   return LR_E_UNSUPPORTED;
 }
 
diff --git a/leftrefill_amd/csrc/elementwise.hip b/leftrefill_amd/csrc/elementwise.hip
--- a/leftrefill_amd/csrc/elementwise.hip
+++ b/leftrefill_amd/csrc/elementwise.hip
@@ -404,7 +404,7 @@
   return (int)g;
 }
 
-extern "C" int lr_abi_version(void) { return 29; }
+extern "C" int lr_abi_version(void) { return 30; }
 
 #ifdef LR_DEV_VARIANTS
 #include <map>
diff --git a/leftrefill_amd/csrc/gemm_common.h b/leftrefill_amd/csrc/gemm_common.h
--- a/leftrefill_amd/csrc/gemm_common.h
+++ b/leftrefill_amd/csrc/gemm_common.h
@@ -24,6 +24,7 @@
   const f16* p3; const f16* p4; int C3, C4;
   int bf16;
   unsigned* sk_cnt;
+  const float* gi_part; const float* gi_gamma; const float* gi_beta; int gi_chunks; float gi_eps; int gi_silu;
 #ifdef LR_GEMM_STAGGER
   int stagger;
 #endif
diff --git a/leftrefill_amd/csrc/gemm_conv.hip b/leftrefill_amd/csrc/gemm_conv.hip
--- a/leftrefill_amd/csrc/gemm_conv.hip
+++ b/leftrefill_amd/csrc/gemm_conv.hip
@@ -947,6 +947,12 @@
   P.st_out = a->stats_out;
   P.st_parts = ((P.N + tn - 1) / tn) * tile_wnw(tm, tn, P.geglu);
   if (P.st_out && (splits > 1 || ((uintptr_t)P.st_out & 7))) return LR_E_ARG;
+  P.gi_part = a->gn_in_part; P.gi_gamma = a->gn_in_gamma; P.gi_beta = a->gn_in_beta;
+  P.gi_chunks = a->gn_in_chunks; P.gi_eps = a->gn_in_eps; P.gi_silu = a->gn_in_silu ? 1 : 0;
+  if (P.gi_part) {
+    if (!P.gi_gamma || !P.gi_beta || P.gi_chunks <= 0) return LR_E_ARG;
+    if (a->pipe != LR_PIPE_HALO || (P.C1 + P.C2) % 32) return LR_E_UNSUPPORTED;
+  }
   hipStream_t st = (hipStream_t)s;
   int rc;
   const int mode = P.geglu ? 1 : P.gelu ? 2 : 0;
diff --git a/leftrefill_amd/csrc/gn_elem.h b/leftrefill_amd/csrc/gn_elem.h
--- /dev/null
+++ b/leftrefill_amd/csrc/gn_elem.h
@@ -0,0 +1,43 @@
+#pragma once
+#include "common.h"
+
+__device__ __forceinline__ void lr_gn_group_stats(const float* __restrict__ partials, int n, int nchunks, int HW, int Cg, float eps,
+                                                  float* s_mean, float* s_rstd, int t) {
+  if ((unsigned)t < 128u) {
+    const int g = t >> 2, sub = t & 3;
+    double s = 0.0, q = 0.0;
+    const float* ps = partials + ((size_t)n * nchunks * 32 + g) * 2;
+#pragma unroll 4
+    for (int c = sub; c < nchunks; c += 4) { s += (double)ps[c * 64]; q += (double)ps[c * 64 + 1]; }
+#pragma unroll
+    for (int sh = 2; sh > 0; sh >>= 1) { s += __shfl_xor(s, sh, 64); q += __shfl_xor(q, sh, 64); }
+    if (sub == 0) {
+      const double cnt = (double)HW * (double)Cg;
+      const double mean = s / cnt;
+      double var = q / cnt - mean * mean;
+      if (var < 0.0) var = 0.0;
+      s_mean[g] = (float)mean;
+      s_rstd[g] = (float)(1.0 / sqrt(var + (double)eps));
+    }
+  }
+}
+
+__device__ __forceinline__ void lr_gn_coef(float mean, float rstd, float gamma, float beta, float& a, float& b) {
+  const float sc = rstd * gamma;
+  a = sc;
+  b = beta - mean * sc;
+}
+
+__device__ __forceinline__ float lr_gn_elem(float x, float a, float b, int silu) {
+  const float z = fmaf(x, a, b);
+  return silu ? z * __builtin_amdgcn_rcpf(1.0f + __expf(-z)) : z;
+}
+
+template <typename T>
+__device__ __forceinline__ uint4 lr_gn_octet(const uint4& v, const float* a, const float* b, int silu) {
+  float f[8];
+  lr_unpack8<T>(v, f);
+#pragma unroll
+  for (int i = 0; i < 8; ++i) f[i] = lr_gn_elem(f[i], a[i], b[i], silu);
+  return lr_pack8<T>(f);
+}
diff --git a/leftrefill_amd/csrc/norm.hip b/leftrefill_amd/csrc/norm.hip
--- a/leftrefill_amd/csrc/norm.hip
+++ b/leftrefill_amd/csrc/norm.hip
@@ -1,4 +1,5 @@
 #include "common.h"
+#include "gn_elem.h"
 
 #include <stdlib.h>
 
@@ -87,41 +88,15 @@
   float ga[8], be[8];
 #pragma unroll
   for (int i = 0; i < 8; ++i) { ga[i] = gamma[c0 + i]; be[i] = beta[c0 + i]; }
-  if (t < 128) {
-    const int g = t >> 2, sub = t & 3;
-    double s = 0.0, q = 0.0;
-    const float* ps = partials + ((size_t)n * nchunks * 32 + g) * 2;
-#pragma unroll 4
-    for (int c = sub; c < nchunks; c += 4) { s += (double)ps[c * 64]; q += (double)ps[c * 64 + 1]; }
-#pragma unroll
-    for (int sh = 2; sh > 0; sh >>= 1) { s += __shfl_xor(s, sh, 64); q += __shfl_xor(q, sh, 64); }
-    if (sub == 0) {
-      const double cnt = (double)HW * (double)Cg;
-      const double mean = s / cnt;
-      double var = q / cnt - mean * mean;
-      if (var < 0.0) var = 0.0;
-      s_mean[g] = (float)mean;
-      s_rstd[g] = (float)(1.0 / sqrt(var + (double)eps));
-    }
-  }
+  lr_gn_group_stats(partials, n, nchunks, HW, Cg, eps, s_mean, s_rstd, t);
   __syncthreads();
   float a[8], b[8];
 #pragma unroll
   for (int i = 0; i < 8; ++i) {
     const int g = (c0 + i) / Cg;
-    a[i] = s_rstd[g] * ga[i];
-    b[i] = be[i] - s_mean[g] * a[i];
-  }
-  auto emit = [&](int pp, const uint4& v) {
-    float f[8];
-    lr_unpack8<T>(v, f);
-#pragma unroll
-    for (int i = 0; i < 8; ++i) {
-      const float z = fmaf(f[i], a[i], b[i]);
-      f[i] = silu ? z * __builtin_amdgcn_rcpf(1.0f + __expf(-z)) : z;
-    }
-    *reinterpret_cast<uint4*>(dst + (size_t)pp * C) = lr_pack8<T>(f);
-  };
+    lr_gn_coef(s_mean[g], s_rstd[g], ga[i], be[i], a[i], b[i]);
+  }
+  auto emit = [&](int pp, const uint4& v) { *reinterpret_cast<uint4*>(dst + (size_t)pp * C) = lr_gn_octet<T>(v, a, b, silu); };
   if (r >= R) return;
   bool have = first;
   while (have) {
@@ -558,23 +533,7 @@
 
 __device__ __forceinline__ void gn_finalize_stats(const float* __restrict__ partials, int n, int nchunks, int HW, int Cg,
                                                   float eps, float* s_mean, float* s_rstd) {
-  const int t = threadIdx.x;
-  if (t < 128) {
-    const int g = t >> 2, sub = t & 3;
-    double s = 0.0, q = 0.0;
-    const float* ps = partials + ((size_t)n * nchunks * 32 + g) * 2;
-    for (int c = sub; c < nchunks; c += 4) { s += (double)ps[c * 64]; q += (double)ps[c * 64 + 1]; }
-#pragma unroll
-    for (int sh = 2; sh > 0; sh >>= 1) { s += __shfl_xor(s, sh, 64); q += __shfl_xor(q, sh, 64); }
-    if (sub == 0) {
-      const double cnt = (double)HW * (double)Cg;
-      const double mean = s / cnt;
-      double var = q / cnt - mean * mean;
-      if (var < 0.0) var = 0.0;
-      s_mean[g] = (float)mean;
-      s_rstd[g] = (float)(1.0 / sqrt(var + (double)eps));
-    }
-  }
+  lr_gn_group_stats(partials, n, nchunks, HW, Cg, eps, s_mean, s_rstd, threadIdx.x);
 }
 
 __device__ __forceinline__ float gn_act_grad(float z, int silu) {
diff --git a/leftrefill_amd/engine.py b/leftrefill_amd/engine.py
--- a/leftrefill_amd/engine.py
+++ b/leftrefill_amd/engine.py
@@ -39,12 +39,14 @@
     tok2: Optional[torch.Tensor] = None
     gs: Optional[tuple] = None
     gs2: Optional[tuple] = None
+    pend: Optional[tuple] = None
 
     @property
     def HW(self):
         return self.H * self.W
 
     def materialize(self):
+        assert self.pend is None, "an activation with a pending GroupNorm goes to engine.conv only"
         if self.tok2 is None:
             return self.tok
         return torch.cat([self.tok, self.tok2], dim=1).contiguous()
@@ -267,6 +269,8 @@
         H, W = act.H, act.W
     want = gn_stats and gn_stats_ok(act.tok) and pc.cout == pc.w.shape[0]
     extra = {} if skip_parts is None else {"skip_parts": skip_parts}
+    if act.pend is not None:
+        extra["gn_in"] = act.pend
     y = ops.gemm_conv(act.tok, pc.w, B=act.N, H=H, W=W, Hs=act.H, Ws=act.W, taps=pc.taps, stride=pc.stride, up=up,
                       asym=asym, x2=act.tok2, bias=pc.b, rowvec=rowvec, resid=resid, want_gn_stats=want, skip=skip, **extra)
     y, gs = y if want else (y, None)
@@ -283,12 +287,17 @@
     return ("channels", act.gs, act.gs2)
 
 
-def gn(act: Act, pn: PackedNorm, silu):
+def gn(act: Act, pn: PackedNorm, silu, defer=False):
+    assert act.pend is None
     HW = act.HW
     if training(act.tok) or (act.tok2 is not None and training(act.tok2)):
         return Act(ops.group_norm(act.tok, act.N, HW, pn.g, pn.b, pn.eps, silu, act.tok2, stats=_gn_train_stats(act)), act.N, act.H, act.W)
     fused = (act.gs is not None and HW % act.gs[1] == 0 and gn_fuse_ok(act.tok)
              and (act.tok2 is None or (act.gs2 is not None and HW % act.gs2[1] == 0)))
+    if fused and defer and ops.GN_IN_CONV and (act.tok.shape[1] + (0 if act.tok2 is None else act.tok2.shape[1])) % 32 == 0:
+        single = act.tok2 is None and act.gs[2] is not None
+        gp, chunks = (act.gs[2], act.gs[3]) if single else (ops.group_norm_finalize(act.tok, act.N, HW, act.gs, act.tok2, act.gs2), 1)
+        return Act(act.tok, act.N, act.H, act.W, tok2=act.tok2, pend=(gp, chunks, pn.g, pn.b, pn.eps, silu))
     if fused and act.tok2 is None and act.gs[2] is not None:
         y = ops.group_norm_groups(act.tok, act.N, HW, pn.g, pn.b, pn.eps, silu, act.gs[2], act.gs[3])
     elif fused:
@@ -307,9 +316,9 @@
     if forking(act.tok) or (act.tok2 is not None and forking(act.tok2)):
         h, act = gn_fork(act, pr.n1, True)
     else:
-        h = gn(act, pr.n1, True)
+        h = gn(act, pr.n1, True, defer=True)
     h = conv(h, pr.c1, rowvec=emb_out, gn_stats=True)
-    h = gn(h, pr.n2, True)
+    h = gn(h, pr.n2, True, defer=True)
     if pr.c2s is not None and SKIP_FUSED and gn_fuse_ok(act.tok) and gn_fuse_ok(h.tok) and (act.tok2 is None or gn_fuse_ok(act.tok2)):
         return conv(h, pr.c2s, gn_stats=True, skip=(act.tok, act.tok2))
     if (pr.c2s is not None and SKIP_FUSED and TRAIN_SKIP_FUSED and (training(h.tok) or training(act.tok) or (act.tok2 is not None and training(act.tok2)))
diff --git a/leftrefill_amd/ops.py b/leftrefill_amd/ops.py
--- a/leftrefill_amd/ops.py
+++ b/leftrefill_amd/ops.py
@@ -146,6 +146,51 @@
     return y
 
 
+def group_norm_finalize(x1, N, HW, gs1, x2=None, gs2=None):
+    lib = _lib.load()
+    C1 = x1.shape[-1]
+    C2 = 0 if x2 is None else x2.shape[-1]
+    p1, r1 = gs1[:2]
+    p2, r2 = gs2[:2] if x2 is not None else (None, 1)
+    assert p1.shape == (N * HW // r1, C1, 2) and HW % r1 == 0
+    if x2 is not None:
+        assert p2.shape == (N * HW // r2, C2, 2) and HW % r2 == 0
+    partials = torch.empty(N, 1, 32, 2, device=x1.device, dtype=torch.float32)
+    _lib.check(lib.lr_groupnorm_finalize(_p(p1), C1, r1, _p(p2), C2, r2, N, HW, _p(partials), _stream()), "groupnorm_finalize")
+    return partials
+
+
+def group_norm_apply(x1, N, HW, gamma, beta, eps, silu, gp, chunks, x2=None):
+    lib = _lib.load()
+    _chk16(x1, "x1")
+    C1 = x1.shape[-1]
+    C2 = 0
+    if x2 is not None:
+        _chk16(x2, "x2")
+        C2 = x2.shape[-1]
+    assert gp.dtype == torch.float32 and gp.is_contiguous() and gp.shape == (N, chunks, 32, 2), (gp.shape, N, chunks)
+    assert gamma.dtype == torch.float32 and beta.dtype == torch.float32 and gamma.numel() == C1 + C2
+    y = torch.empty(N * HW, C1 + C2, device=x1.device, dtype=x1.dtype)
+    _lib.check(_fn(lib, "lr_groupnorm_apply_n", x1.dtype)(_p(x1), C1, _p(x2), C2, N, HW, _p(gp), chunks, _p(gamma), _p(beta), float(eps),
+                                                          int(bool(silu)), _p(y), _stream()), "groupnorm_apply_n")
+    return y
+
+
+GN_IN_CONV = os.environ.get("LEFTREFILL_GN_IN_CONV", "1") != "0"
+GN_IN_MAX_C = 3072
+
+
+def gn_in_conv_takes(pipe, taps, stride, up, asym, H, W, Hs, Ws, C):
+    return (pipe == 8 and taps == 9 and stride == 1 and not up and not asym and Hs == H and Ws == W and C % 64 == 0
+            and C * (2 if H == 8 else 1) <= GN_IN_MAX_C)
+
+
+def gn_in_conv_ok(pipe, taps, stride, up, asym, H, W, Hs, Ws, C, N, tile_n, enabled=None):
+    if not (GN_IN_CONV if enabled is None else enabled):
+        return False
+    return gn_in_conv_takes(pipe, taps, stride, up, asym, H, W, Hs, Ws, C) and N <= tile_n
+
+
 OUT_FUSED = os.environ.get("LEFTREFILL_OUT_FUSED", "1") != "0"
 
 
@@ -217,7 +262,7 @@
 
 def gemm_conv(x1, wt, *, B, H, W, Hs=None, Ws=None, taps=1, stride=1, up=0, asym=False, x2=None, bias=None, rowvec=None,
               resid=None, geglu=False, gelu=False, out=None, tile_n=0, tile_m=0, splits=0, pipe=0, ln=None,
-              want_stats=False, want_gn_stats=False, gn_hw=0, per_sample=False, wt_pm=False, skip=None):
+              want_stats=False, want_gn_stats=False, gn_hw=0, per_sample=False, wt_pm=False, skip=None, gn_in=None, gn_in_fuse=None):
     lib = _lib.load()
     _chk16(x1, "x1")
     _chk16(wt, "wt")
@@ -255,6 +300,9 @@
         out = torch.empty(M, n_out, device=x1.device, dtype=x1.dtype)
     a = GemmArgs()
     a.p1, a.C1, a.p2, a.C2 = _p(x1), C1, _p(x2), C2
+    if gn_in is not None:
+        assert not per_sample and not c16 and ln is None and (C1 + C2) % 32 == 0
+        a.C1, a.p2, a.C2 = C1 + C2, 0, 0
     a.B, a.H, a.W, a.Hs, a.Ws = B, H, W, Hs, Ws
     a.taps, a.stride, a.up, a.asym = taps, stride, up, int(bool(asym))
     a.wt, a.N = _p(wt), Nw
@@ -289,7 +337,7 @@
     st = _stream()
     if tile_m == 0 and tile_n == 0 and splits == 0:
         scale = _PLAN_BATCH_SCALE[0]
-        key = tile_key(M * scale, Nw, Kw - Cs1 - Cs2, taps, stride, up, geglu, C2 > 0, asym, gelu, ln is not None, want_stats)
+        key = tile_key(M * scale, Nw, Kw - Cs1 - Cs2, taps, stride, up, geglu, C2 > 0 and gn_in is None, asym, gelu, ln is not None, want_stats)
         best = tile_cache().get(key)
         (TABLE_HITS if best is not None else TABLE_MISSES).add(key)
         if best is None and PLAN_LOG and key not in _untabulated:
@@ -316,6 +364,19 @@
             plan = (ctypes.c_int32 * 4)()
             lib.lr_gemm_plan(a, plan)
             a.tile_m, a.tile_n, a.splits, a.pipe = plan[0], plan[1], plan[2], plan[3]
+    x1_raw, x2_raw = x1, x2
+    if gn_in is not None:
+        gp, chunks, gamma, beta, eps, silu = gn_in
+        takes = gn_in_conv_takes(a.pipe, taps, stride, up, asym, H, W, Hs, Ws, C1 + C2)
+        if (takes and gn_in_fuse) if gn_in_fuse is not None else gn_in_conv_ok(a.pipe, taps, stride, up, asym, H, W, Hs, Ws, C1 + C2, Nw, a.tile_n):
+            assert gp.dtype == torch.float32 and gp.is_contiguous() and gp.shape == (B, chunks, 32, 2), (gp.shape, B, chunks)
+            assert gamma.dtype == torch.float32 and beta.dtype == torch.float32 and gamma.numel() == C1 + C2 == beta.numel()
+            a.p1, a.C1, a.p2, a.C2 = _p(x1), C1, _p(x2), C2
+            a.gn_in_part, a.gn_in_gamma, a.gn_in_beta = _p(gp), _p(gamma), _p(beta)
+            a.gn_in_chunks, a.gn_in_eps, a.gn_in_silu = int(chunks), float(eps), int(bool(silu))
+        else:
+            x1, x2 = group_norm_apply(x1, B, Hs * Ws, gamma, beta, eps, silu, gp, chunks, x2=x2), None
+            a.p1 = _p(x1)
     stats = None
     if want_stats:
         if a.splits == 0:
@@ -347,9 +408,9 @@
         LAUNCH_HOOK(key, 1, rc)
         if rc != 0 and PLAN_TRIAL is not None and PLAN_TRIAL.get(key) is not None:
             PLAN_TRIAL[key] = None
-            return gemm_conv(x1, wt, B=B, H=H, W=W, Hs=Hs, Ws=Ws, taps=taps, stride=stride, up=up, asym=asym, x2=x2, bias=bias, rowvec=rowvec,
+            return gemm_conv(x1_raw, wt, B=B, H=H, W=W, Hs=Hs, Ws=Ws, taps=taps, stride=stride, up=up, asym=asym, x2=x2_raw, bias=bias, rowvec=rowvec,
                              resid=resid, geglu=geglu, gelu=gelu, out=out, ln=ln, want_stats=want_stats, want_gn_stats=want_gn_stats, gn_hw=gn_hw,
-                             per_sample=per_sample, wt_pm=wt_pm, skip=skip)
+                             per_sample=per_sample, wt_pm=wt_pm, skip=skip, gn_in=gn_in, gn_in_fuse=gn_in_fuse)
         _lib.check(rc, "gemm_conv")
     else:
         _lib.check(lib.lr_gemm_conv_f16(a, st), "gemm_conv")
```

Result: no change. 4.499 images/s, median of 6 (+0.3%).
